# jzhang-dev/FEDRANN

Hardware: AMD Instinct MI355X
Metric: read-pairs/sec (overlap candidates) (higher is better)
Workload: dtype f32 (canonical fp32 results; fp16 MFMA candidate prefilter + exact fp32 re-rank)

## Files before the change

fedrann_amd/_lib.py:

```python
import ctypes
import os

import numpy as np

HERE = os.path.dirname(os.path.abspath(__file__))
LIB_PATH = os.environ.get("FEDRANN_HIP_LIB") or os.path.join(HERE, "libfedrann_hip.so")

SYMBOLS = (
    "fdr_create", "fdr_destroy", "fdr_last_error", "fdr_device_info", "fdr_padded_dim",
    "fdr_projection_load", "fdr_embed", "fdr_knn", "fdr_embed_knn", "fdr_embed_dev",
    "fdr_normalize_dev", "fdr_knn_workspace_bytes", "fdr_knn_dev", "fdr_timing", "fdr_timing_read",
    "fdr_last_uncertified", "fdr_set_knn_mode", "fdr_set_dedup_mode", "fdr_last_unique", "fdr_kmer_output_scan",
    "fdr_kmer_output_load", "fdr_kmer_search", "fdr_kmer_search_indices", "fdr_kmer_count",
    "fdr_kmer_count_fetch", "fdr_set_kmer_count_block", "fdr_last_kmer_count_blocks", "fdr_csr_compact", "fdr_host_register", "fdr_host_unregister",
    "fdr_overlaps_write", "fdr_last_prefilter_launches", "fdr_knn_classes_dev", "fdr_knn_unique_dev",
    "fdr_knn_expand_dev", "fdr_kmer_output_scan_range", "fdr_kmer_output_load_range",
    "fdr_kmer_count_begin", "fdr_kmer_count_add", "fdr_kmer_count_finish", "fdr_reads_scan", "fdr_reads_parse",
    "fdr_kmer_output_append", "fdr_last_query_paths", "fdr_last_knn_trace", "fdr_kmer_count_export_dev",
    "fdr_kmer_count_merge_dev", "fdr_kmer_count_merge", "fdr_set_knn_capture", "fdr_last_candidates",
    "fdr_last_range_sets", "fdr_knn_sparse", "fdr_set_live_chunks", "fdr_knn_sparse_metric",
    "fdr_sparse_index_build", "fdr_sparse_index_search", "fdr_sparse_index_info", "fdr_sparse_index_free",
)
FDR_MAX_K = 128
KERNELS = ("embed_csr", "normalize_rows", "knn_tile", "knn_merge", "knn_prefilter", "knn_rerank",
           "knn_dedup", "kmer_search", "kmer_compact")
FDR_MAX_DIM = 2048
PATH_CERTIFIED, PATH_RANGE, PATH_EXACT, PATH_ZERO, PATH_RANGE_OVERFLOW, PATH_GENERIC, PATH_CLASS_MEMBER = 1, 2, 3, 4, 5, 6, 0x80
TRACE_KINDS = ("none", "exact", "prefilter", "generic", "sparse")
FALLBACKS = ("none", "chunked", "whole")
CAPTURE_CANDIDATES, CAPTURE_RANGE = 1, 2
RANGE_CAP = 1024
METRIC_COSINE, METRIC_JACCARD = 0, 1
SPARSE_METRICS = {"cosine": METRIC_COSINE, "jaccard": METRIC_JACCARD}


class KnnTrace(ctypes.Structure):
    _fields_ = [(n, ctypes.c_int32) for n in ("kind", "dp", "k", "kp")] + \
        [(n, ctypes.c_int64) for n in ("queries", "targets")] + \
        [(n, ctypes.c_int32) for n in (
            "pass_waves", "pass_wps", "pass_units", "pass_list_keys", "pass_pingpong", "pass_launches", "pass_queues",
            "pass_segments", "uncertified", "zero_queries", "range_queries", "range_chunks", "range_pp_chunks",
            "range_w8_chunks", "range_overflow", "exact_fallback", "exact_calls", "exact_queries", "exact_waves",
            "exact_qsets", "generic", "exact_segments", "pass_live", "pass_live_items_2", "pass_live_items_3",
            "pass_live_items_4", "pass_live_items_5", "pass_live_items_6", "pass_live_dense_items")]


class FedrannHipError(RuntimeError):
    pass


_lib = None


def _share_torch_hip_runtime():
    if os.environ.get("FEDRANN_HIP_SYSTEM_RUNTIME") == "1":
        return
    try:
        import importlib.util
        spec = importlib.util.find_spec("torch")
        if spec is None or not spec.submodule_search_locations:
            return
        path = os.path.join(list(spec.submodule_search_locations)[0], "lib", "libamdhip64.so")
        if os.path.exists(path):
            ctypes.CDLL(path, mode=ctypes.RTLD_GLOBAL)
    except (OSError, ImportError, ValueError):
        pass


def load_library():
    global _lib
    if _lib is not None:
        return _lib
    if not os.path.exists(LIB_PATH):
        raise FedrannHipError(
            "%s is missing: build it with `python -m fedrann_amd.build` "
            "(hipcc --offload-arch=gfx950); there is no CPU fallback" % LIB_PATH)
    _share_torch_hip_runtime()
    L = ctypes.CDLL(LIB_PATH)
    i32, i64, vp, sz = ctypes.c_int32, ctypes.c_int64, ctypes.c_void_p, ctypes.c_size_t
    L.fdr_create.argtypes = [ctypes.c_int, ctypes.POINTER(vp)]
    L.fdr_destroy.argtypes = [vp]
    L.fdr_last_error.argtypes = []
    L.fdr_last_error.restype = ctypes.c_char_p
    L.fdr_device_info.argtypes = [vp, ctypes.c_char_p, ctypes.c_int]
    L.fdr_padded_dim.argtypes = [ctypes.c_int]
    L.fdr_projection_load.argtypes = [vp, i64, i32, vp, vp, vp]
    L.fdr_embed.argtypes = [vp, i64, vp, vp, vp]
    L.fdr_knn.argtypes = [vp, vp, i64, i32, i32, vp, vp]
    L.fdr_embed_knn.argtypes = [vp, i64, vp, vp, i32, vp, vp, vp]
    L.fdr_knn_sparse.argtypes = [vp, i64, i64, vp, vp, vp, i32, vp, vp]
    L.fdr_knn_sparse_metric.argtypes = [vp, i32, i64, i64, vp, vp, vp, i32, vp, vp]
    L.fdr_sparse_index_build.argtypes = [vp, i32, i64, i64, vp, vp, vp]
    L.fdr_sparse_index_search.argtypes = [vp, i32, i64, i64, vp, vp]
    L.fdr_sparse_index_info.argtypes = [vp, ctypes.POINTER(i32), ctypes.POINTER(i64), ctypes.POINTER(i64),
                                        ctypes.POINTER(i64), ctypes.POINTER(sz)]
    L.fdr_sparse_index_free.argtypes = [vp]
    L.fdr_embed_dev.argtypes = [vp, i64, vp, vp, vp, vp]
    L.fdr_normalize_dev.argtypes = [vp, vp, i64, i32, vp, vp, vp]
    L.fdr_knn_workspace_bytes.argtypes = [vp, i64, i64, i32, i32]
    L.fdr_knn_workspace_bytes.restype = sz
    L.fdr_knn_dev.argtypes = [vp, vp, vp, i64, vp, vp, i64, i64, i32, i32, vp, vp, vp, sz, vp]
    L.fdr_knn_classes_dev.argtypes = [vp, vp, vp, i64, i32, i32, i64, vp, sz, vp, ctypes.POINTER(i32)]
    L.fdr_knn_unique_dev.argtypes = [vp, i64, i64, vp, vp, vp]
    L.fdr_knn_expand_dev.argtypes = [vp, i64, i64, i64, vp, vp, i64, vp, vp, vp]
    L.fdr_last_uncertified.argtypes = [vp]
    L.fdr_last_query_paths.argtypes = [vp, vp, i64]
    L.fdr_last_knn_trace.argtypes = [vp, ctypes.POINTER(KnnTrace)]
    L.fdr_set_knn_mode.argtypes = [vp, ctypes.c_int]
    L.fdr_set_knn_capture.argtypes = [vp, ctypes.c_int]
    L.fdr_last_candidates.argtypes = [vp, vp, i64, i32, ctypes.POINTER(i32)]
    L.fdr_last_range_sets.argtypes = [vp, i64, vp, vp, vp, vp]
    L.fdr_set_dedup_mode.argtypes = [vp, ctypes.c_int]
    L.fdr_set_live_chunks.argtypes = [vp, ctypes.c_int]
    L.fdr_last_unique.argtypes = [vp, ctypes.POINTER(ctypes.c_int), ctypes.POINTER(ctypes.c_int)]
    L.fdr_last_prefilter_launches.argtypes = [vp, ctypes.POINTER(ctypes.c_int), ctypes.POINTER(ctypes.c_int)]
    p64 = ctypes.POINTER(ctypes.c_int64)
    L.fdr_kmer_output_scan.argtypes = [ctypes.c_char_p, p64, p64, p64]
    L.fdr_kmer_output_load.argtypes = [ctypes.c_char_p, i64, i32, i64, i64, i64, vp, vp, vp, vp]
    L.fdr_kmer_output_scan_range.argtypes = [ctypes.c_char_p, i64, i64, p64, p64, p64]
    L.fdr_kmer_output_load_range.argtypes = [ctypes.c_char_p, i64, i32, i64, i64, i64, i64, i64, vp, vp, vp, vp]
    L.fdr_kmer_output_append.argtypes = [ctypes.c_char_p, i64, vp, vp, vp, vp]
    L.fdr_reads_scan.argtypes = [vp, i64, i32, i32, i32, p64, p64, p64]
    L.fdr_reads_parse.argtypes = [vp, i64, i32, i32, i64, i64, vp, vp, vp]
    L.fdr_csr_compact.argtypes = [vp, i64, vp, vp, vp, vp, i64, i32]
    L.fdr_host_register.argtypes = [vp, vp, sz]
    L.fdr_host_unregister.argtypes = [vp, vp]
    L.fdr_overlaps_write.argtypes = [ctypes.c_char_p, i32, i32, i64, i64, i64, i32, vp, vp, vp, vp, vp, i32, p64]
    L.fdr_kmer_search.argtypes = [vp, vp, vp, i64, vp, i64, i32, vp, p64]
    L.fdr_kmer_search_indices.argtypes = [vp, vp]
    L.fdr_kmer_count.argtypes = [vp, vp, vp, i64, i32, i64, p64]
    L.fdr_kmer_count_fetch.argtypes = [vp, vp, vp]
    L.fdr_kmer_count_begin.argtypes = [vp, i32]
    L.fdr_kmer_count_add.argtypes = [vp, vp, vp, i64]
    L.fdr_kmer_count_finish.argtypes = [vp, i64, p64]
    L.fdr_set_kmer_count_block.argtypes = [vp, ctypes.c_int64]
    L.fdr_last_kmer_count_blocks.argtypes = [vp]
    L.fdr_kmer_count_export_dev.argtypes = [vp, vp, i32, vp, vp, vp, vp]
    L.fdr_kmer_count_merge_dev.argtypes = [vp, i32, vp, vp, vp, i64, p64, vp]
    L.fdr_kmer_count_merge.argtypes = [vp, i32, vp, vp, vp, i64, p64]
    L.fdr_timing.argtypes = [vp, ctypes.c_int]
    L.fdr_timing_read.argtypes = [vp, ctypes.c_int, ctypes.POINTER(ctypes.c_int),
                                  ctypes.POINTER(ctypes.c_float)]
    for name in SYMBOLS:
        fn = getattr(L, name)
        if name not in ("fdr_last_error", "fdr_knn_workspace_bytes"):
            fn.restype = ctypes.c_int
    _lib = L
    return L


def _ptr(a):
    return None if a is None else ctypes.c_void_p(a.ctypes.data)


def _as(a, dtype, name):
    b = np.ascontiguousarray(a, dtype=dtype)
    if b.dtype != np.dtype(dtype):
        raise TypeError("%s must be %s" % (name, np.dtype(dtype)))
    return b


def kmer_output_load(path, n_features, n_threads=0):
    L = load_library()
    bpath = os.fsencode(path)
    R, nnz, nb = ctypes.c_int64(), ctypes.c_int64(), ctypes.c_int64()
    rc = L.fdr_kmer_output_scan(bpath, ctypes.byref(R), ctypes.byref(nnz), ctypes.byref(nb))
    if rc != 0:
        raise FedrannHipError("fdr_kmer_output_scan failed (%d): %s" % (rc, L.fdr_last_error().decode()))
    indptr = np.empty(2 * R.value + 1, dtype=np.int64)
    indices = np.empty(2 * nnz.value, dtype=np.int32)
    name_off = np.empty(R.value + 1, dtype=np.int64)
    names = np.empty(nb.value, dtype=np.uint8)
    rc = L.fdr_kmer_output_load(bpath, int(n_features), int(n_threads), R.value, nnz.value, nb.value,
                                indptr.ctypes.data, indices.ctypes.data, name_off.ctypes.data, names.ctypes.data)
    if rc != 0:
        raise FedrannHipError("fdr_kmer_output_load failed (%d): %s" % (rc, L.fdr_last_error().decode()))
    return indptr, indices, name_off, names


def kmer_output_records(path):
    import struct
    with open(path, "rb") as f:
        head = f.read(16)
    if len(head) < 16:
        raise ValueError("incomplete file header")
    magic, version, _, total = struct.unpack("<4sB3sQ", head)
    if magic != b"KMER":
        raise ValueError("invalid file format (bad magic)")
    if version != 1:
        raise ValueError("unsupported version: %d" % version)
    return int(total)


def kmer_output_load_range(path, n_features, rec_lo, rec_hi, n_threads=0, with_names=True):
    L = load_library()
    bpath = os.fsencode(path)
    R, nnz, nb = ctypes.c_int64(), ctypes.c_int64(), ctypes.c_int64()
    total = kmer_output_records(path)
    lo = max(0, min(int(rec_lo), total))
    hi = total if rec_hi is None else max(lo, min(int(rec_hi), total))
    rc = L.fdr_kmer_output_scan_range(bpath, lo, hi, ctypes.byref(R), ctypes.byref(nnz), ctypes.byref(nb))
    if rc != 0:
        raise FedrannHipError("fdr_kmer_output_scan_range failed (%d): %s" % (rc, L.fdr_last_error().decode()))
    indptr = np.empty(2 * (hi - lo) + 1, dtype=np.int64)
    indices = np.empty(2 * nnz.value, dtype=np.int32)
    name_off = np.empty(R.value + 1, dtype=np.int64) if with_names else None
    names = np.empty(nb.value, dtype=np.uint8) if with_names else None
    rc = L.fdr_kmer_output_load_range(bpath, int(n_features), int(n_threads), R.value, lo, hi, nnz.value, nb.value,
                                      indptr.ctypes.data, indices.ctypes.data,
                                      name_off.ctypes.data if with_names else None,
                                      names.ctypes.data if with_names and names.size else None)
    if rc != 0:
        raise FedrannHipError("fdr_kmer_output_load_range failed (%d): %s" % (rc, L.fdr_last_error().decode()))
    return R.value, indptr, indices, name_off, names


def reads_parse(buf, n, is_fastq, fastq_ids_as_fasta, eof, seq_buf=None):
    L = load_library()
    used, R, nb = ctypes.c_int64(), ctypes.c_int64(), ctypes.c_int64()
    base = buf.ctypes.data if n else None
    rc = L.fdr_reads_scan(base, int(n), int(bool(is_fastq)), int(bool(fastq_ids_as_fasta)), int(bool(eof)),
                          ctypes.byref(used), ctypes.byref(R), ctypes.byref(nb))
    if rc != 0:
        raise FedrannHipError("fdr_reads_scan failed (%d): %s" % (rc, L.fdr_last_error().decode()))
    seqs = np.empty(nb.value, dtype=np.uint8) if seq_buf is None else seq_buf[:nb.value]
    off = np.empty(R.value + 1, dtype=np.int64)
    span = np.empty(2 * R.value, dtype=np.int64)
    rc = L.fdr_reads_parse(base, used.value, int(bool(is_fastq)), int(bool(fastq_ids_as_fasta)), R.value, nb.value,
                           seqs.ctypes.data if nb.value else None, off.ctypes.data, span.ctypes.data if R.value else None)
    if rc != 0:
        raise FedrannHipError("fdr_reads_parse failed (%d): %s" % (rc, L.fdr_last_error().decode()))
    view = memoryview(buf)
    sp = span.tolist()
    ids = [bytes(view[sp[2 * r]:sp[2 * r + 1]]) for r in range(R.value)]
    return used.value, ids, seqs, off


def reads_consumed(buf, n, is_fastq, fastq_ids_as_fasta, eof):
    L = load_library()
    used, R, nb = ctypes.c_int64(), ctypes.c_int64(), ctypes.c_int64()
    rc = L.fdr_reads_scan(buf.ctypes.data if n else None, int(n), int(bool(is_fastq)), int(bool(fastq_ids_as_fasta)),
                          int(bool(eof)), ctypes.byref(used), ctypes.byref(R), ctypes.byref(nb))
    if rc != 0:
        raise FedrannHipError("fdr_reads_scan failed (%d): %s" % (rc, L.fdr_last_error().decode()))
    return used.value


def kmer_output_append(path, ids, indptr, indices):
    L = load_library()
    name_off, names = pack_names(ids)
    indptr = np.ascontiguousarray(indptr, dtype=np.int64)
    indices = np.ascontiguousarray(indices, dtype=np.int32)
    if indptr.size != len(ids) + 1:
        raise ValueError("indptr must have one entry per record + 1")
    rc = L.fdr_kmer_output_append(os.fsencode(path), len(ids), _ptr(name_off), _ptr(names) if names.size else None,
                                  _ptr(indptr), _ptr(indices) if indices.size else None)
    if rc != 0:
        msg = L.fdr_last_error().decode()
        if "non-ASCII" in msg or "bytes long" in msg:
            raise ValueError(msg)
        raise FedrannHipError("fdr_kmer_output_append failed (%d): %s" % (rc, msg))


def pack_names(read_names):
    enc = [n if isinstance(n, bytes) else str(n).encode("utf-8") for n in read_names]
    off = np.zeros(len(enc) + 1, dtype=np.int64)
    if enc:
        np.cumsum([len(b) for b in enc], out=off[1:])
    return off, np.frombuffer(b"".join(enc), dtype=np.uint8)


def overlaps_write(path, idx, dist, name_off, names, strands, row0=0, append=False, header=True, n_threads=0):
    L = load_library()
    idx = _as(idx, np.int32, "idx")
    dist = _as(dist, np.float32, "dist")
    if idx.ndim != 2 or dist.shape != idx.shape:
        raise ValueError("idx and dist must be [rows, k] arrays of the same shape")
    name_off = _as(name_off, np.int64, "name_off")
    names = np.ascontiguousarray(names, dtype=np.uint8)
    if strands is None:
        n_total = 2 * (name_off.size - 1)
    else:
        strands = np.ascontiguousarray(strands, dtype=np.uint8)
        n_total = name_off.size - 1
        if strands.size != n_total:
            raise ValueError("strands must have one entry per row")
    lines = ctypes.c_int64()
    rc = L.fdr_overlaps_write(os.fsencode(path), 1 if append else 0, 1 if header else 0, n_total, int(row0),
                              idx.shape[0], idx.shape[1], _ptr(idx), _ptr(dist), _ptr(name_off),
                              names.ctypes.data if names.size else None, _ptr(strands) if strands is not None else None,
                              int(n_threads),
                              ctypes.byref(lines))
    if rc != 0:
        raise FedrannHipError("fdr_overlaps_write failed (%d): %s" % (rc, L.fdr_last_error().decode()))
    return int(lines.value)


def sparse_metric_code(metric):
    if not isinstance(metric, str) or metric not in SPARSE_METRICS:
        raise ValueError("metric must be 'cosine' or 'jaccard', got %r" % (metric,))
    return SPARSE_METRICS[metric]


def check_sparse_rows(indptr, indices, values, n_features, k):
    return _check_sparse(indptr, indices, values, n_features, k)


def check_sparse_csr(indptr, indices, values, n_features):
    n, _, F = _check_sparse(indptr, indices, values, n_features, None)
    return n, F


def check_sparse_search(n, k, lo=0, hi=None):
    for name, v in (("k", k), ("lo", lo), ("hi", hi)):
        if isinstance(v, bool) or not (isinstance(v, (int, np.integer)) or (name == "hi" and v is None)):
            raise ValueError("%s must be an integer, got %r" % (name, v))
    k, lo, hi = int(k), int(lo), int(n if hi is None else hi)
    if not 1 <= k <= FDR_MAX_K or k > n:
        raise ValueError("need 1 <= k <= min(%d, n = %d), got k = %d" % (FDR_MAX_K, n, k))
    if not 0 <= lo <= hi <= n:
        raise ValueError("need 0 <= lo <= hi <= n = %d, got [%d, %d)" % (n, lo, hi))
    return k, lo, hi


def _check_sparse(indptr, indices, values, n_features, k):
    for name, a, dt in (("indptr", indptr, np.int64), ("indices", indices, np.int32), ("values", values, np.float32)):
        if a is None and name == "values":
            continue
        if not isinstance(a, np.ndarray) or a.dtype != dt:
            raise TypeError("%s must be a numpy %s array" % (name, np.dtype(dt)))
        if a.ndim != 1 or not a.flags.c_contiguous:
            raise ValueError("%s must be a C-contiguous 1-D array" % name)
    if indptr.size < 1 or indptr[0] != 0 or indptr[-1] != indices.size or np.any(np.diff(indptr) < 0):
        raise ValueError("indptr is not a CSR row pointer of the indices")
    if values is not None and values.size != indices.size:
        raise ValueError("values and indices differ in length")
    n, k, F = indptr.size - 1, None if k is None else int(k), int(n_features)
    if not 1 <= F <= np.iinfo(np.int32).max:
        raise ValueError("n_features must be in [1, 2^31)")
    if k is None:
        if n < 1:
            raise ValueError("need at least one row")
    elif not 1 <= k <= FDR_MAX_K or k > n:
        raise ValueError("need 1 <= k <= min(%d, n = %d), got k = %d" % (FDR_MAX_K, n, k))
    if indices.size:
        if int(indices.min()) < 0 or int(indices.max()) >= F:
            raise ValueError("a feature index is outside [0, %d)" % F)
        ascending = np.diff(indices) > 0
        starts = indptr[1:-1]
        ascending[starts[(starts > 0) & (starts < indices.size)] - 1] = True
        if not np.all(ascending):
            raise ValueError("feature indices must be strictly ascending inside each row (sorted, no duplicates)")
    if values is not None and not np.all(np.isfinite(values)):
        raise ValueError("values must be finite")
    return n, k, F


class Context:

    def __init__(self, device=0):
        self._L = load_library()
        h = ctypes.c_void_p()
        rc = self._L.fdr_create(int(device), ctypes.byref(h))
        if rc != 0:
            raise FedrannHipError("fdr_create(%d) failed (%d): %s" % (device, rc, self._err()))
        self._h = h
        self.device = int(device)
        self.n_features = 0
        self.d = 0
        self._sparse_gen = 0

    def _err(self):
        return self._L.fdr_last_error().decode("utf-8", "replace")

    def _check(self, rc, what):
        if rc != 0:
            raise FedrannHipError("%s failed (%d): %s" % (what, rc, self._err()))

    def close(self):
        if getattr(self, "_h", None):
            self._L.fdr_destroy(self._h)
            self._h = None

    def __del__(self):
        try:
            self.close()
        except Exception:
            pass

    def __enter__(self):
        return self

    def __exit__(self, *a):
        self.close()

    def device_info(self):
        buf = ctypes.create_string_buffer(256)
        self._check(self._L.fdr_device_info(self._h, buf, 256), "fdr_device_info")
        name, arch, cus, mem = buf.value.decode().split("|")
        return {"name": name, "arch": arch, "cus": int(cus), "hbm_bytes": int(mem)}

    def padded_dim(self, d):
        dp = self._L.fdr_padded_dim(int(d))
        if dp < 0:
            raise FedrannHipError("embedding dimension %d unsupported (1..%d)" % (d, FDR_MAX_DIM))
        return dp

    def set_knn_mode(self, mode):
        code = {"auto": 0, "exact": 1, "prefilter": 2}[mode]
        self._check(self._L.fdr_set_knn_mode(self._h, code), "fdr_set_knn_mode")

    def set_dedup_mode(self, mode):
        code = {"auto": 0, "off": 1, "on": 2, "force": 3}[mode]
        self._check(self._L.fdr_set_dedup_mode(self._h, code), "fdr_set_dedup_mode")

    def set_live_chunks(self, mode):
        code = {"auto": 0, "off": 1, "force": 2}[mode]
        self._check(self._L.fdr_set_live_chunks(self._h, code), "fdr_set_live_chunks")

    def kmer_search(self, seqs, seq_off, lib_codes, k):
        seqs = np.ascontiguousarray(seqs, dtype=np.uint8)
        seq_off = np.ascontiguousarray(seq_off, dtype=np.int64)
        lib_codes = np.ascontiguousarray(lib_codes, dtype=np.uint64)
        R = seq_off.size - 1
        if R < 0 or (R >= 0 and seq_off.size and int(seq_off[-1]) != seqs.size):
            raise ValueError("seq_off does not describe seqs")
        indptr = np.empty(R + 1, dtype=np.int64)
        nnz = ctypes.c_int64()
        self._check(self._L.fdr_kmer_search(self._h, seqs.ctypes.data, seq_off.ctypes.data, R,
                                            lib_codes.ctypes.data, lib_codes.size, int(k), indptr.ctypes.data,
                                            ctypes.byref(nnz)), "fdr_kmer_search")
        indices = np.empty(nnz.value, dtype=np.int32)
        self._check(self._L.fdr_kmer_search_indices(self._h, indices.ctypes.data), "fdr_kmer_search_indices")
        return indptr, indices

    def kmer_count(self, seqs, seq_off, k, min_count=1):
        seqs = np.ascontiguousarray(seqs, dtype=np.uint8)
        seq_off = np.ascontiguousarray(seq_off, dtype=np.int64)
        n = ctypes.c_int64()
        self._check(self._L.fdr_kmer_count(self._h, seqs.ctypes.data, seq_off.ctypes.data, seq_off.size - 1, int(k),
                                           int(min_count), ctypes.byref(n)), "fdr_kmer_count")
        codes = np.empty(n.value, dtype=np.uint64)
        counts = np.empty(n.value, dtype=np.uint64)
        self._check(self._L.fdr_kmer_count_fetch(self._h, codes.ctypes.data, counts.ctypes.data), "fdr_kmer_count_fetch")
        return codes, counts

    def kmer_count_begin(self, k):
        self._check(self._L.fdr_kmer_count_begin(self._h, int(k)), "fdr_kmer_count_begin")

    def kmer_count_add(self, seqs, seq_off):
        seqs = np.ascontiguousarray(seqs, dtype=np.uint8)
        seq_off = np.ascontiguousarray(seq_off, dtype=np.int64)
        self._check(self._L.fdr_kmer_count_add(self._h, seqs.ctypes.data, seq_off.ctypes.data, seq_off.size - 1),
                    "fdr_kmer_count_add")

    def kmer_count_finish(self, min_count=1):
        n = ctypes.c_int64()
        self._check(self._L.fdr_kmer_count_finish(self._h, int(min_count), ctypes.byref(n)), "fdr_kmer_count_finish")
        codes = np.empty(n.value, dtype=np.uint64)
        counts = np.empty(n.value, dtype=np.uint64)
        self._check(self._L.fdr_kmer_count_fetch(self._h, codes.ctypes.data, counts.ctypes.data), "fdr_kmer_count_fetch")
        return codes, counts

    def set_kmer_count_block(self, chars):
        self._check(self._L.fdr_set_kmer_count_block(self._h, int(chars)), "fdr_set_kmer_count_block")

    def kmer_count_export_dev(self, d_splitters, n_parts, d_codes_out=None, d_counts_out=None, stream=None):
        part_off = np.empty(int(n_parts) + 1, dtype=np.int64)
        self._check(self._L.fdr_kmer_count_export_dev(self._h, d_splitters or None, int(n_parts), d_codes_out or None,
                                                      d_counts_out or None, part_off.ctypes.data, stream or None),
                    "fdr_kmer_count_export_dev")
        return part_off

    def kmer_count_merge_dev(self, run_off, d_codes, d_counts, min_count=1, stream=None):
        run_off = np.ascontiguousarray(run_off, dtype=np.int64)
        n = ctypes.c_int64()
        self._check(self._L.fdr_kmer_count_merge_dev(self._h, run_off.size - 1, run_off.ctypes.data, d_codes or None,
                                                     d_counts or None, int(min_count), ctypes.byref(n), stream or None),
                    "fdr_kmer_count_merge_dev")
        return self._kmer_count_fetch(n.value)

    def kmer_count_merge(self, run_off, codes, counts, min_count=1):
        run_off = np.ascontiguousarray(run_off, dtype=np.int64)
        codes = np.ascontiguousarray(codes, dtype=np.uint64)
        counts = np.ascontiguousarray(counts, dtype=np.uint64)
        if codes.size != counts.size or (run_off.size and codes.size < int(run_off[-1])):
            raise ValueError("run_off does not describe codes / counts")
        n = ctypes.c_int64()
        self._check(self._L.fdr_kmer_count_merge(self._h, run_off.size - 1, run_off.ctypes.data, codes.ctypes.data,
                                                 counts.ctypes.data, int(min_count), ctypes.byref(n)),
                    "fdr_kmer_count_merge")
        return self._kmer_count_fetch(n.value)

    def _kmer_count_fetch(self, n):
        codes = np.empty(n, dtype=np.uint64)
        counts = np.empty(n, dtype=np.uint64)
        self._check(self._L.fdr_kmer_count_fetch(self._h, codes.ctypes.data, counts.ctypes.data), "fdr_kmer_count_fetch")
        return codes, counts

    def last_kmer_count_blocks(self):
        return int(self._L.fdr_last_kmer_count_blocks(self._h))

    def last_unique(self):
        a, b = ctypes.c_int(), ctypes.c_int()
        self._check(self._L.fdr_last_unique(self._h, ctypes.byref(a), ctypes.byref(b)), "fdr_last_unique")
        return int(a.value), int(b.value)

    def last_prefilter_launches(self):
        a, b = ctypes.c_int(), ctypes.c_int()
        self._check(self._L.fdr_last_prefilter_launches(self._h, ctypes.byref(a), ctypes.byref(b)),
                    "fdr_last_prefilter_launches")
        return int(a.value), int(b.value)

    def last_uncertified(self):
        return int(self._L.fdr_last_uncertified(self._h))

    def last_query_paths(self, n_queries):
        out = np.empty(int(n_queries), dtype=np.uint8)
        self._check(self._L.fdr_last_query_paths(self._h, _ptr(out), int(n_queries)), "fdr_last_query_paths")
        return out

    def last_knn_trace(self):
        t = KnnTrace()
        self._check(self._L.fdr_last_knn_trace(self._h, ctypes.byref(t)), "fdr_last_knn_trace")
        out = {name: int(getattr(t, name)) for name, _ in KnnTrace._fields_}
        out["kind"] = TRACE_KINDS[out["kind"]]
        out["exact_fallback"] = FALLBACKS[out["exact_fallback"]]
        return out

    def set_knn_capture(self, what):
        self._check(self._L.fdr_set_knn_capture(self._h, int(what)), "fdr_set_knn_capture")

    def last_candidates(self, n_queries, kp):
        keys = np.empty((int(n_queries), int(kp)), dtype=np.uint64)
        qbits = ctypes.c_int32(0)
        self._check(self._L.fdr_last_candidates(self._h, _ptr(keys), int(n_queries), int(kp), ctypes.byref(qbits)),
                    "fdr_last_candidates")
        return keys, int(qbits.value)

    def last_range_sets(self, n_range):
        n = int(n_range)
        q, th, cnt = np.empty(n, np.int32), np.empty(n, np.float32), np.empty(n, np.int32)
        rows = np.empty((n, RANGE_CAP), np.int32)
        self._check(self._L.fdr_last_range_sets(self._h, n, _ptr(q), _ptr(th), _ptr(cnt), _ptr(rows)),
                    "fdr_last_range_sets")
        return q, th, cnt, rows

    def timing(self, enable):
        self._check(self._L.fdr_timing(self._h, 1 if enable else 0), "fdr_timing")

    def timing_read(self, which):
        n, ms = ctypes.c_int(), ctypes.c_float()
        self._check(self._L.fdr_timing_read(self._h, int(which), ctypes.byref(n), ctypes.byref(ms)),
                    "fdr_timing_read")
        return int(n.value), float(ms.value)

    def projection_load(self, p_indptr, p_cols, p_vals, n_features, d):
        p_indptr = _as(p_indptr, np.int64, "p_indptr")
        p_cols = _as(p_cols, np.int32, "p_cols")
        p_vals = _as(p_vals, np.float32, "p_vals")
        if p_indptr.shape != (int(n_features) + 1,):
            raise ValueError("p_indptr must have n_features + 1 entries")
        self._check(self._L.fdr_projection_load(self._h, int(n_features), int(d), _ptr(p_indptr),
                                                _ptr(p_cols), _ptr(p_vals)), "fdr_projection_load")
        self.n_features, self.d = int(n_features), int(d)

    def csr_compact(self, a_indptr, a_indices, n_threads=0):
        a_indptr = _as(a_indptr, np.int64, "a_indptr")
        a_indices = _as(a_indices, np.int32, "a_indices")
        n = a_indptr.shape[0] - 1
        out_ip = np.empty(n + 1, dtype=np.int64)
        out_ix = np.empty(max(int(a_indices.size), 1), dtype=np.int32)
        self._check(self._L.fdr_csr_compact(self._h, n, _ptr(a_indptr), _ptr(a_indices), _ptr(out_ip),
                                            _ptr(out_ix), int(out_ix.size), int(n_threads)), "fdr_csr_compact")
        return out_ip, np.ascontiguousarray(out_ix[:int(out_ip[-1])])

    def host_register(self, *arrays):
        for a in arrays:
            if a is not None and a.nbytes:
                self._check(self._L.fdr_host_register(self._h, a.ctypes.data, a.nbytes), "fdr_host_register")

    def host_unregister(self, *arrays):
        for a in arrays:
            if a is not None and a.nbytes:
                self._check(self._L.fdr_host_unregister(self._h, a.ctypes.data), "fdr_host_unregister")

    def embed(self, a_indptr, a_indices):
        a_indptr = _as(a_indptr, np.int64, "a_indptr")
        a_indices = _as(a_indices, np.int32, "a_indices")
        n = a_indptr.shape[0] - 1
        E = np.empty((n, self.d), dtype=np.float32)
        self._check(self._L.fdr_embed(self._h, n, _ptr(a_indptr), _ptr(a_indices), _ptr(E)),
                    "fdr_embed")
        return E

    def knn(self, E, k):
        E = _as(E, np.float32, "E")
        if E.ndim != 2:
            raise ValueError("E must be 2-D")
        n, d = E.shape
        idx = np.empty((n, k), dtype=np.int32)
        dist = np.empty((n, k), dtype=np.float32)
        self._check(self._L.fdr_knn(self._h, _ptr(E), n, d, int(k), _ptr(idx), _ptr(dist)),
                    "fdr_knn")
        return idx, dist

    def knn_sparse(self, indptr, indices, values, n_features, k, metric="cosine"):
        code = sparse_metric_code(metric)
        n, k, F = check_sparse_rows(indptr, indices, values, n_features, k)
        self._sparse_gen += 1
        idx = np.empty((n, k), dtype=np.int32)
        dist = np.empty((n, k), dtype=np.float32)
        if code == METRIC_COSINE:
            self._check(self._L.fdr_knn_sparse(self._h, n, F, _ptr(indptr), _ptr(indices), _ptr(values), k,
                                               _ptr(idx), _ptr(dist)), "fdr_knn_sparse")
        else:
            self._check(self._L.fdr_knn_sparse_metric(self._h, code, n, F, _ptr(indptr), _ptr(indices),
                                                      _ptr(values), k, _ptr(idx), _ptr(dist)),
                        "fdr_knn_sparse_metric")
        return idx, dist

    def sparse_index(self, indptr, indices, values, n_features, metric="cosine"):
        code = sparse_metric_code(metric)
        n, F = check_sparse_csr(indptr, indices, values, n_features)
        self._sparse_gen += 1
        self._check(self._L.fdr_sparse_index_build(self._h, code, n, F, _ptr(indptr), _ptr(indices), _ptr(values)),
                    "fdr_sparse_index_build")
        return SparseIndex(self, n, metric, self._sparse_gen)

    def embed_knn(self, a_indptr, a_indices, k, return_embedding=False, out=None):
        a_indptr = _as(a_indptr, np.int64, "a_indptr")
        a_indices = _as(a_indices, np.int32, "a_indices")
        n = a_indptr.shape[0] - 1
        if out is None:
            idx = np.empty((n, k), dtype=np.int32)
            dist = np.empty((n, k), dtype=np.float32)
        else:
            idx, dist = out
            if (idx.shape, dist.shape) != ((n, k), (n, k)) or idx.dtype != np.int32 or dist.dtype != np.float32 \
                    or not (idx.flags.c_contiguous and dist.flags.c_contiguous):
                raise ValueError("out must be C-contiguous (int32 [n,k], float32 [n,k])")
        E = np.empty((n, self.d), dtype=np.float32) if return_embedding else None
        self._check(self._L.fdr_embed_knn(self._h, n, _ptr(a_indptr), _ptr(a_indices), int(k),
                                          _ptr(idx), _ptr(dist), _ptr(E)), "fdr_embed_knn")
        return (idx, dist, E) if return_embedding else (idx, dist)

    def embed_dev(self, n_rows, d_indptr, d_indices, d_E, stream=0):
        self._check(self._L.fdr_embed_dev(self._h, int(n_rows), d_indptr, d_indices, d_E,
                                          stream or None), "fdr_embed_dev")

    def normalize_dev(self, d_E, n_rows, d, d_Ehat, d_zero, stream=0):
        self._check(self._L.fdr_normalize_dev(self._h, d_E, int(n_rows), int(d), d_Ehat, d_zero,
                                              stream or None), "fdr_normalize_dev")

    def knn_workspace_bytes(self, nq, nt, d, k):
        return int(self._L.fdr_knn_workspace_bytes(self._h, int(nq), int(nt), int(d), int(k)))

    def knn_dev(self, d_Qhat, d_qzero, nq, d_That, d_tzero, nt, t_base, d, k, d_idx, d_dist,
                d_ws, ws_bytes, stream=0):
        self._check(self._L.fdr_knn_dev(self._h, d_Qhat, d_qzero, int(nq), d_That, d_tzero,
                                        int(nt), int(t_base), int(d), int(k), d_idx, d_dist, d_ws,
                                        int(ws_bytes), stream or None), "fdr_knn_dev")


    def knn_classes_dev(self, d_That, d_tzero, nt, d, k, nq_max, d_ws, ws_bytes, stream=0):
        nu = ctypes.c_int32()
        self._check(self._L.fdr_knn_classes_dev(self._h, d_That, d_tzero, int(nt), int(d), int(k), int(nq_max), d_ws,
                                                int(ws_bytes), stream or None, ctypes.byref(nu)), "fdr_knn_classes_dev")
        return int(nu.value)

    def knn_unique_dev(self, u_lo, u_hi, d_idx_u, d_dist_u, stream=0):
        self._check(self._L.fdr_knn_unique_dev(self._h, int(u_lo), int(u_hi), d_idx_u, d_dist_u, stream or None),
                    "fdr_knn_unique_dev")

    def knn_expand_dev(self, q0, nq, t_base, d_idx_u_all, d_dist_u_all, d_idx, d_dist, stream=0, u_row_stride=0):
        self._check(self._L.fdr_knn_expand_dev(self._h, int(q0), int(nq), int(t_base), d_idx_u_all, d_dist_u_all,
                                               int(u_row_stride), d_idx, d_dist, stream or None), "fdr_knn_expand_dev")


class SparseIndex:

    def __init__(self, ctx, n, metric, gen):
        self._ctx, self.n, self.metric, self._gen = ctx, int(n), metric, gen
        self._open = True

    def _live(self, what):
        if not self._open:
            raise FedrannHipError("%s: the sparse index is closed" % what)
        if not getattr(self._ctx, "_h", None):
            raise FedrannHipError("%s: the context of the sparse index is closed" % what)
        if self._ctx._sparse_gen != self._gen:
            raise FedrannHipError("%s: the context has built another sparse index since this one" % what)

    def search(self, k, lo=0, hi=None, out=None):
        k, lo, hi = check_sparse_search(self.n, k, lo, hi)
        nq = hi - lo
        if out is None:
            idx = np.empty((nq, k), dtype=np.int32)
            dist = np.empty((nq, k), dtype=np.float32)
        else:
            idx, dist = out
            if (idx.shape, dist.shape) != ((nq, k), (nq, k)) or idx.dtype != np.int32 or dist.dtype != np.float32 \
                    or not (idx.flags.c_contiguous and dist.flags.c_contiguous):
                raise ValueError("out must be C-contiguous (int32 [hi - lo, k], float32 [hi - lo, k])")
        self._live("SparseIndex.search")
        c = self._ctx
        c._check(c._L.fdr_sparse_index_search(c._h, k, lo, hi, _ptr(idx), _ptr(dist)), "fdr_sparse_index_search")
        return idx, dist

    def info(self):
        self._live("SparseIndex.info")
        c = self._ctx
        m, n, p, z = ctypes.c_int32(), ctypes.c_int64(), ctypes.c_int64(), ctypes.c_int64()
        b = ctypes.c_size_t()
        c._check(c._L.fdr_sparse_index_info(c._h, ctypes.byref(m), ctypes.byref(n), ctypes.byref(p), ctypes.byref(z),
                                            ctypes.byref(b)), "fdr_sparse_index_info")
        name = [s for s, v in SPARSE_METRICS.items() if v == m.value][0]
        return {"metric": name, "n": int(n.value), "postings": int(p.value), "zero_rows": int(z.value),
                "device_bytes": int(b.value)}

    def close(self):
        c = self._ctx
        if self._open and getattr(c, "_h", None) and c._sparse_gen == self._gen:
            c._check(c._L.fdr_sparse_index_free(c._h), "fdr_sparse_index_free")
        self._open = False

    def __enter__(self):
        return self

    def __exit__(self, *a):
        self.close()


_default_ctx = None


def default_context():
    global _default_ctx
    if _default_ctx is None:
        dev = int(os.environ.get("FEDRANN_DEVICE", os.environ.get("LOCAL_RANK", "0")))
        _default_ctx = Context(dev)
    return _default_ctx
```

fedrann_amd/csrc/fedrann_hip.hip:

```cpp
#include <hip/hip_runtime.h>
#include <rocprim/device/device_radix_sort.hpp>
#include <rocprim/device/device_scan.hpp>
#include <rocprim/device/device_run_length_encode.hpp>
#include <rocprim/device/device_merge.hpp>
#include <rocprim/device/device_reduce_by_key.hpp>

#include <algorithm>
#include <array>
#include <atomic>
#include <cmath>
#include <condition_variable>
#include <cstdarg>
#include <cstdint>
#include <cstdio>
#include <cstdlib>
#include <cstring>
#include <functional>
#include <limits>
#include <mutex>
#include <new>
#include <string>
#include <thread>
#include <type_traits>
#include <utility>
#include <vector>

#include "../../include/fedrann_hip.h"

typedef float f32x4 __attribute__((ext_vector_type(4)));
typedef float f32x16 __attribute__((ext_vector_type(16)));

#include "host_common.inc"

#define HIP_TRY(expr)                                                                          \
    do {                                                                                       \
        hipError_t e_ = (expr);                                                                \
        if (e_ != hipSuccess)                                                                  \
            return fail(e_ == hipErrorOutOfMemory ? FDR_E_NOMEM : FDR_E_HIP, "%s failed: %s",  \
                        #expr, hipGetErrorString(e_));                                         \
    } while (0)

template <int DP>
__global__ __launch_bounds__(256) void embed_csr_kernel(
    long long n_rows, const long long *__restrict__ a_indptr, const int *__restrict__ a_indices,
    long long n_features, const uint2 *__restrict__ ftab, const uint4 *__restrict__ rowinfo,
    const uint2 *__restrict__ ent, int d, float *__restrict__ E) {
    constexpr int NACC = DP / 64;
    static_assert(DP <= 512, "d > 512: embed_csr_wide_kernel");
    constexpr int GR = 8;
    constexpr int NB = 4;
    constexpr int RPW = 2;
    const int lane = threadIdx.x & 63;
    const long long wave0 = (long long)blockIdx.x * (blockDim.x >> 6) + (threadIdx.x >> 6);
    const long long nwaves = (long long)gridDim.x * (blockDim.x >> 6);
    auto apply = [&](float (&acc)[NACC], const uint4 &inf, const bool h) __attribute__((always_inline)) {
        u64 m = __ballot(h);
        while (m) {
            const int src = __builtin_ctzll(m);
            m &= m - 1;
            int q = __builtin_amdgcn_readlane((int)inf.x, src);
            const int ee = q + __builtin_amdgcn_readlane((int)inf.y, src);
            unsigned c = (unsigned)__builtin_amdgcn_readlane((int)inf.z, src);
            float v = __int_as_float(__builtin_amdgcn_readlane((int)inf.w, src));
            while (true) {
#pragma unroll
                for (int i = 0; i < NACC; ++i)
                    if (c == (unsigned)(lane + 64 * i)) acc[i] += v;
                if (++q >= ee) break;
                const uint2 en = ent[q];
                c = en.x;
                v = __uint_as_float(en.y);
            }
        }
    };
    auto store_row = [&](const long long row, const float (&acc)[NACC]) __attribute__((always_inline)) {
        float *out = E + row * (long long)d;
#pragma unroll
        for (int i = 0; i < NACC; ++i)
            if (lane + 64 * i < d) out[lane + 64 * i] = acc[i];
    };
    for (long long row0 = wave0 * GR; row0 < n_rows; row0 += nwaves * GR) {
        long long beg[GR], len_max = 0;
        int len[GR];
#pragma unroll
        for (int r = 0; r < GR; ++r) {
            const long long row = row0 + r < n_rows ? row0 + r : n_rows - 1;
            beg[r] = a_indptr[row];
            const long long l = row0 + r < n_rows ? a_indptr[row + 1] - beg[r] : 0;
            len[r] = (int)(l < 64 ? l : 64);
            len_max = l > len_max ? l : len_max;
        }
        if (len_max <= 64) {
            int f[GR];
            uint2 w[GR];
            uint4 info[GR];
            bool hit[GR];
#pragma unroll
            for (int r = 0; r < GR; ++r) f[r] = lane < len[r] ? a_indices[beg[r] + lane] : -1;
#pragma unroll
            for (int r = 0; r < GR; ++r) {
                w[r] = make_uint2(0u, 0u);
                if (f[r] >= 0 && (long long)f[r] < n_features) w[r] = ftab[f[r] >> 5];
            }
#pragma unroll
            for (int r = 0; r < GR; ++r) {
                const unsigned bit = 1u << (f[r] & 31);
                hit[r] = (w[r].x & bit) != 0u;
                info[r] = make_uint4(0u, 0u, 0u, 0u);
                if (hit[r]) info[r] = rowinfo[w[r].y + __popc(w[r].x & (bit - 1u))];
            }
#pragma unroll
            for (int r = 0; r < GR; ++r) {
                if (row0 + r >= n_rows) continue;
                float acc[NACC];
#pragma unroll
                for (int i = 0; i < NACC; ++i) acc[i] = 0.0f;
                apply(acc, info[r], hit[r]);
                store_row(row0 + r, acc);
            }
            continue;
        }
        for (int p0 = 0; p0 < GR && row0 + p0 < n_rows; p0 += RPW) {
            const long long prow0 = row0 + p0;
            long long pbeg[RPW], pend[RPW];
            int f[RPW][NB];
            uint2 w[RPW][NB];
            uint4 info[RPW][NB];
            bool hit[RPW][NB];
#pragma unroll
            for (int r = 0; r < RPW; ++r) {
                const long long row = prow0 + r < n_rows ? prow0 + r : n_rows - 1;
                pbeg[r] = a_indptr[row];
                pend[r] = prow0 + r < n_rows ? a_indptr[row + 1] : pbeg[r];
            }
#pragma unroll
            for (int r = 0; r < RPW; ++r)
#pragma unroll
                for (int u = 0; u < NB; ++u) {
                    const long long pos = pbeg[r] + 64 * u + lane;
                    f[r][u] = pos < pend[r] ? a_indices[pos] : -1;
                }
#pragma unroll
            for (int r = 0; r < RPW; ++r)
#pragma unroll
                for (int u = 0; u < NB; ++u) {
                    w[r][u] = make_uint2(0u, 0u);
                    if (f[r][u] >= 0 && (long long)f[r][u] < n_features) w[r][u] = ftab[f[r][u] >> 5];
                }
#pragma unroll
            for (int r = 0; r < RPW; ++r)
#pragma unroll
                for (int u = 0; u < NB; ++u) {
                    const unsigned bit = 1u << (f[r][u] & 31);
                    hit[r][u] = (w[r][u].x & bit) != 0u;
                    info[r][u] = make_uint4(0u, 0u, 0u, 0u);
                    if (hit[r][u]) info[r][u] = rowinfo[w[r][u].y + __popc(w[r][u].x & (bit - 1u))];
                }
#pragma unroll
            for (int r = 0; r < RPW; ++r) {
                if (prow0 + r >= n_rows) continue;
                float acc[NACC];
#pragma unroll
                for (int i = 0; i < NACC; ++i) acc[i] = 0.0f;
#pragma unroll
                for (int u = 0; u < NB; ++u) apply(acc, info[r][u], hit[r][u]);
                for (long long base = pbeg[r] + 64 * NB; base < pend[r]; base += 64 * NB) {
                    int f2[NB];
                    uint2 w2[NB];
#pragma unroll
                    for (int u = 0; u < NB; ++u) {
                        const long long pos = base + 64 * u + lane;
                        f2[u] = pos < pend[r] ? a_indices[pos] : -1;
                    }
#pragma unroll
                    for (int u = 0; u < NB; ++u) {
                        w2[u] = make_uint2(0u, 0u);
                        if (f2[u] >= 0 && (long long)f2[u] < n_features) w2[u] = ftab[f2[u] >> 5];
                    }
#pragma unroll
                    for (int u = 0; u < NB; ++u) {
                        const unsigned bit = 1u << (f2[u] & 31);
                        const bool h2 = (w2[u].x & bit) != 0u;
                        uint4 i2 = make_uint4(0u, 0u, 0u, 0u);
                        if (h2) i2 = rowinfo[w2[u].y + __popc(w2[u].x & (bit - 1u))];
                        apply(acc, i2, h2);
                    }
                }
                store_row(prow0 + r, acc);
            }
        }
    }
}

template <int DP>
__global__ __launch_bounds__(256) void embed_csr_wide_kernel(
    long long n_rows, const long long *__restrict__ a_indptr, const int *__restrict__ a_indices,
    long long n_features, const uint2 *__restrict__ ftab, const uint4 *__restrict__ rowinfo,
    const uint2 *__restrict__ ent, int d, float *__restrict__ E) {
    constexpr int NACC = DP / 64;
    constexpr int NB = 4;
    constexpr int RPW = 2;
    const int lane = threadIdx.x & 63;
    const long long wave0 = (long long)blockIdx.x * (blockDim.x >> 6) + (threadIdx.x >> 6);
    const long long nwaves = (long long)gridDim.x * (blockDim.x >> 6);
    for (long long row0 = wave0 * RPW; row0 < n_rows; row0 += nwaves * RPW) {
        long long beg[RPW], end[RPW];
        int f[RPW][NB];
        uint2 w[RPW][NB];
        uint4 info[RPW][NB];
        bool hit[RPW][NB];
#pragma unroll
        for (int r = 0; r < RPW; ++r) {
            const long long row = row0 + r < n_rows ? row0 + r : n_rows - 1;
            beg[r] = a_indptr[row];
            end[r] = row0 + r < n_rows ? a_indptr[row + 1] : beg[r];
        }
#pragma unroll
        for (int r = 0; r < RPW; ++r)
#pragma unroll
            for (int u = 0; u < NB; ++u) {
                const long long pos = beg[r] + 64 * u + lane;
                f[r][u] = pos < end[r] ? a_indices[pos] : -1;
            }
#pragma unroll
        for (int r = 0; r < RPW; ++r)
#pragma unroll
            for (int u = 0; u < NB; ++u) {
                w[r][u] = make_uint2(0u, 0u);
                if (f[r][u] >= 0 && (long long)f[r][u] < n_features) w[r][u] = ftab[f[r][u] >> 5];
            }
#pragma unroll
        for (int r = 0; r < RPW; ++r)
#pragma unroll
            for (int u = 0; u < NB; ++u) {
                const unsigned bit = 1u << (f[r][u] & 31);
                hit[r][u] = (w[r][u].x & bit) != 0u;
                info[r][u] = make_uint4(0u, 0u, 0u, 0u);
                if (hit[r][u]) info[r][u] = rowinfo[w[r][u].y + __popc(w[r][u].x & (bit - 1u))];
            }
#pragma unroll
        for (int r = 0; r < RPW; ++r) {
            if (row0 + r >= n_rows) break;
            float acc[NACC];
#pragma unroll
            for (int i = 0; i < NACC; ++i) acc[i] = 0.0f;
            auto apply = [&](const uint4 &inf, const bool h) {
                u64 m = __ballot(h);
                while (m) {
                    const int src = __builtin_ctzll(m);
                    m &= m - 1;
                    int q = __builtin_amdgcn_readlane((int)inf.x, src);
                    const int ee = q + __builtin_amdgcn_readlane((int)inf.y, src);
                    unsigned c = (unsigned)__builtin_amdgcn_readlane((int)inf.z, src);
                    float v = __int_as_float(__builtin_amdgcn_readlane((int)inf.w, src));
                    while (true) {
#pragma unroll
                        for (int i = 0; i < NACC; ++i)
                            if (c == (unsigned)(lane + 64 * i)) acc[i] += v;
                        if (++q >= ee) break;
                        const uint2 en = ent[q];
                        c = en.x;
                        v = __uint_as_float(en.y);
                    }
                }
            };
#pragma unroll
            for (int u = 0; u < NB; ++u) apply(info[r][u], hit[r][u]);
            for (long long base = beg[r] + 64 * NB; base < end[r]; base += 64 * NB) {
                int f2[NB];
                uint2 w2[NB];
#pragma unroll
                for (int u = 0; u < NB; ++u) {
                    const long long pos = base + 64 * u + lane;
                    f2[u] = pos < end[r] ? a_indices[pos] : -1;
                }
#pragma unroll
                for (int u = 0; u < NB; ++u) {
                    w2[u] = make_uint2(0u, 0u);
                    if (f2[u] >= 0 && (long long)f2[u] < n_features) w2[u] = ftab[f2[u] >> 5];
                }
#pragma unroll
                for (int u = 0; u < NB; ++u) {
                    const unsigned bit = 1u << (f2[u] & 31);
                    const bool h2 = (w2[u].x & bit) != 0u;
                    uint4 i2 = make_uint4(0u, 0u, 0u, 0u);
                    if (h2) i2 = rowinfo[w2[u].y + __popc(w2[u].x & (bit - 1u))];
                    apply(i2, h2);
                }
            }
            float *out = E + (row0 + r) * (long long)d;
#pragma unroll
            for (int i = 0; i < NACC; ++i)
                if (lane + 64 * i < d) out[lane + 64 * i] = acc[i];
        }
    }
}

template <int DP, int RB, bool VEC>
__global__ __launch_bounds__(256) void normalize_rows_kernel(const float *__restrict__ E,
                                                             long long n_rows, int d,
                                                             float *__restrict__ Ehat,
                                                             unsigned char *__restrict__ zero) {
    __shared__ float tile[RB][DP + 1];
    const int tid = threadIdx.x;
    const long long row0 = (long long)blockIdx.x * RB;
    const int nr = (int)min((long long)RB, n_rows - row0);
    const float *src = E + row0 * (long long)d;
    if (d < DP || nr < RB) {
        for (int i = tid; i < RB * DP; i += 256) tile[i / DP][i % DP] = 0.0f;
        __syncthreads();
    }
    const int total = nr * d;
    if constexpr (VEC) {
        const f32x4 *src4 = reinterpret_cast<const f32x4 *>(src);
        for (int i4 = tid; i4 < total / 4; i4 += 256) {
            const f32x4 v = src4[i4];
            const int i = 4 * i4, r = i / d, c = i - r * d;
            tile[r][c] = v[0];
            tile[r][c + 1] = v[1];
            tile[r][c + 2] = v[2];
            tile[r][c + 3] = v[3];
        }
    } else {
        for (int i = tid; i < total; i += 256) tile[i / d][i % d] = src[i];
    }
    __syncthreads();
    if (tid < RB) {
        float n = 0.0f;
#pragma unroll 8
        for (int k = 0; k < DP; ++k) {
            const float x = tile[tid][k];
            n = __builtin_fmaf(x, x, n);
        }
        float ri = 0.0f;
        if (n > 0.0f) ri = (float)(1.0 / sqrt((double)n));
#pragma unroll 8
        for (int k = 0; k < DP; ++k) tile[tid][k] = tile[tid][k] * ri;
        if (tid < nr) zero[row0 + tid] = n > 0.0f ? 0 : 1;
    }
    __syncthreads();
    float *dst = Ehat + row0 * (long long)DP;
    if constexpr (VEC) {
        f32x4 *dst4 = reinterpret_cast<f32x4 *>(dst);
        for (int i4 = tid; i4 < nr * DP / 4; i4 += 256) {
            const int i = 4 * i4, r = i / DP, p = i % DP;
            const int g = p >> 3, hh = (p >> 2) & 1;
            const float *t = &tile[r][8 * g + hh];
            dst4[i4] = f32x4{t[0], t[2], t[4], t[6]};
        }
    } else {
        for (int i = tid; i < nr * DP; i += 256) {
            const int r = i / DP, p = i % DP;
            const int g = p >> 3, hh = (p >> 2) & 1, s = p & 3;
            dst[i] = tile[r][8 * g + 2 * s + hh];
        }
    }
}

#include "knn_plan.inc"
#include "knn_workspace.inc"
#include "projection_tables.inc"
#include "csr_compact.inc"
#include "host_upload.inc"
#include "knn_exact.inc"
#include "knn_exact_wide.inc"
#include "knn_prefilter.inc"
#include "knn_prefilter_pp.inc"
#include "knn_order.inc"
#include "knn_prefilter_live.inc"
#include "dedup_classes.inc"
#include "knn_generic.inc"

struct DevBuf {
    void *p = nullptr;
    size_t cap = 0;
    int reserve(size_t bytes) {
        if (bytes <= cap) return FDR_OK;
        if (p) (void)hipFree(p);
        p = nullptr;
        cap = 0;
        hipError_t e = hipMalloc(&p, bytes ? bytes : 1);
        if (e != hipSuccess) {
            p = nullptr;
            return fail(FDR_E_NOMEM, "hipMalloc(%zu bytes) failed: %s", bytes, hipGetErrorString(e));
        }
        cap = bytes;
        return FDR_OK;
    }
    void release() {
        if (p) (void)hipFree(p);
        p = nullptr;
        cap = 0;
    }
    DevBuf() = default;
    DevBuf(const DevBuf &) = delete;
    DevBuf &operator=(const DevBuf &) = delete;
    ~DevBuf() { release(); }
};

template <class T>
struct DevArray {
    DevBuf buf;
    int reserve(size_t count) { return buf.reserve(count * sizeof(T)); }
    T *ptr() const { return static_cast<T *>(buf.p); }
    void release() { buf.release(); }
    size_t bytes() const { return buf.cap; }
};
template <class... A>
static void release_all(A &...arrays) {
    (arrays.release(), ...);
}

template <class... F>
static int rocprim_reserve(DevArray<char> &tmp, const F &...calls) {
    size_t need = 1;
    hipError_t e = hipSuccess;
    auto ask = [&](const auto &call) {
        size_t bytes = 0;
        if (e == hipSuccess) e = call(nullptr, bytes);
        need = std::max(need, bytes);
    };
    (ask(calls), ...);
    if (e != hipSuccess) return fail(FDR_E_HIP, "rocprim temporary storage size query failed: %s", hipGetErrorString(e));
    return tmp.reserve(need);
}
template <class F>
static int rocprim_run(DevArray<char> &tmp, const char *what, const F &call) {
    if (int rc = rocprim_reserve(tmp, call)) return rc;
    size_t bytes = tmp.bytes();
    const hipError_t e = call(tmp.ptr(), bytes);
    if (e != hipSuccess)
        return fail(e == hipErrorOutOfMemory ? FDR_E_NOMEM : FDR_E_HIP, "%s failed: %s", what, hipGetErrorString(e));
    return FDR_OK;
}

struct PinnedBuf {
    void *p = nullptr;
    size_t cap = 0;
    int reserve(size_t bytes) {
        if (bytes <= cap) return FDR_OK;
        if (p) (void)hipHostFree(p);
        p = nullptr;
        cap = 0;
        hipError_t e = hipHostMalloc(&p, bytes ? bytes : 1, hipHostMallocDefault);
        if (e != hipSuccess) {
            p = nullptr;
            return fail(FDR_E_NOMEM, "hipHostMalloc(%zu bytes) failed: %s", bytes, hipGetErrorString(e));
        }
        cap = bytes;
        return FDR_OK;
    }
    PinnedBuf() = default;
    PinnedBuf(const PinnedBuf &) = delete;
    PinnedBuf &operator=(const PinnedBuf &) = delete;
    ~PinnedBuf() {
        if (p) (void)hipHostFree(p);
    }
};

struct KnnCallRecord {
    struct {
        int flagged = 0;
        int launches = 0, queues = 0;
    } pass;
    int unique_targets = 0, unique_queries = 0;
    struct {
        const uint8_t *dev = nullptr;
        int64_t n = 0;
        uint8_t all = FDR_PATH_NONE;
        hipStream_t stream = nullptr;
    } paths;
    fdr_knn_trace trace = {};
};

struct KnnArgs {
    const float *Qhat;
    const uint8_t *qzero;
    int64_t nq;
    const float *That;
    const uint8_t *tzero;
    int64_t nt, t_base;
    int d, k;
    int32_t *idx;
    float *dist;
    void *ws;
    size_t ws_bytes;
    hipStream_t st;
};


struct KmerSearchScratch {
    DevArray<unsigned char> seq;
    DevArray<long long> off;
    DevArray<u64> lib_codes;
    DevArray<u64> keys;
    DevArray<unsigned> vals;
    DevArray<u64> bloom;
    DevArray<unsigned long long> counter;
    DevArray<u64> pairs, sorted;
    DevArray<int> flag, scan;
    DevArray<int> indices, rows;
    DevArray<long long> indptr;
    DevArray<char> tmp;
    long long nnz = 0;
    void release() {
        release_all(seq, off, lib_codes, keys, vals, bloom, counter, pairs, sorted, flag, scan, indices, rows, indptr, tmp);
        nnz = 0;
    }
};

struct KmerCountScratch {
    DevArray<unsigned char> seq;
    DevArray<long long> off;
    DevArray<u64> codes;
    DevArray<u64> sorted;
    DevArray<unsigned> run_len;
    DevArray<unsigned> n_runs;
    DevArray<u64> run_counts;
    DevArray<u64> acc_codes[2], acc_counts[2];
    DevArray<u64> merged_codes, merged_counts;
    DevArray<unsigned long long> n_table;
    DevArray<int> keep, keep_scan;
    DevArray<u64> kept_counts;
    DevArray<long long> run_off, samp_pre;
    DevArray<u64> samples, bounds;
    DevArray<long long> slices;
    DevArray<long long> part_off;
    DevArray<char> tmp;
    int k = 0;
    int acc = 0;
    long long na = 0;
    long long n = 0;
    int64_t block_chars = 0;
    int blocks = 0;
    void release() {
        release_all(seq, off, codes, sorted, run_len, n_runs, run_counts, acc_codes[0], acc_codes[1], acc_counts[0],
                    acc_counts[1], merged_codes, merged_counts, n_table, keep, keep_scan, kept_counts, run_off, samp_pre,
                    samples, bounds, slices, part_off, tmp);
        k = acc = 0;
        na = n = 0;
    }
};

struct SparseIndex {
    DevArray<long long> indptr;
    DevArray<int> indices;
    DevArray<float> values;
    DevArray<float> xhat;
    DevArray<int> asize;
    DevArray<unsigned char> zero;
    DevArray<u64> keys, sorted_keys;
    DevArray<unsigned> pos, sorted_pos;
    DevArray<int> efeat;
    DevArray<float> pval;
    DevArray<long long> runptr;
    DevArray<int> heavy;
    DevArray<u64> cnt;
    DevArray<char> tmp;
    struct Built {
        bool valid = false;
        int metric = 0;
        long long n = 0, kept = 0, nzero = 0;
    } built;
    int *run_flags() const { return reinterpret_cast<int *>(keys.ptr()); }
    int *run_numbers(long long kept) const { return run_flags() + kept; }
    int *posting_rows() const { return reinterpret_cast<int *>(pos.ptr()); }
    static constexpr size_t cnt_words = 8 + FDR_MAX_K;
    int *zidx() const { return reinterpret_cast<int *>(cnt.ptr() + 8); }
    float *zdist() const { return reinterpret_cast<float *>(zidx() + FDR_MAX_K); }
    template <class F>
    auto each(F f) {
        return f(indptr, indices, values, xhat, asize, zero, keys, sorted_keys, pos, sorted_pos, efeat, pval, runptr,
                 heavy, cnt, tmp);
    }
    size_t bytes() {
        return each([](auto &...a) { return (a.bytes() + ...); });
    }
    void release() {
        each([](auto &...a) { release_all(a...); });
        built = {};
    }
};

struct fdr_ctx {
    int device = 0;
    int num_cus = 256;
    hipStream_t stream = nullptr;
    hipStream_t aux_stream[3] = {nullptr, nullptr, nullptr};
    hipEvent_t aux_ev[4] = {nullptr, nullptr, nullptr, nullptr};
    hipDeviceProp_t prop;
    long long n_features = 0;
    int d = 0;
    long long p_nnz = 0, p_rows = 0;
    DevBuf ftab, crow, ent;
    std::vector<uint32_t> h_bits;
    DevBuf a_indptr, a_indices, E, Ehat, zero, idx, dist, ws;
    DevBuf c_indptr, c_indices;
    PinnedBuf stage_ids, stage_ptr;
    hipEvent_t up_ev[3] = {nullptr, nullptr, nullptr};
    hup::WorkerPool up_pool;
    KmerSearchScratch ks;
    KmerCountScratch kc;
    SparseIndex sp;
    int knn_mode = FDR_MODE_AUTO;
    int dedup_mode = FDR_DEDUP_AUTO;
    int live_mode = FDR_LIVE_AUTO;
    std::vector<unsigned> live_host;
    KnnCallRecord last;
    struct {
        int what = 0;
        bool cand_valid = false, range_valid = false;
        int64_t nq = 0, n_range = 0;
        int kp = 0, qbits = 0;
        DevBuf cand, rq, rtheta, rcnt, rrows;
        hipStream_t stream = nullptr;
    } cap;
    struct {
        bool valid = false;
        const float *That = nullptr;
        const uint8_t *tzero = nullptr;
        int64_t nt = 0, nq_max = 0;
        int d = 0, k = 0, nu = 0;
        void *ws = nullptr;
        size_t ws_bytes = 0;
    } cls;
    bool timing = false;
    std::vector<hipEvent_t> ev_pool[FDR_NUM_KERNELS];
    size_t ev_used[FDR_NUM_KERNELS] = {};
};

static void knn_call_begin(fdr_ctx *ctx) {
    ctx->last.trace = fdr_knn_trace{};
    ctx->last.paths = {};
    ctx->cap.cand_valid = ctx->cap.range_valid = false;
    ctx->cap.nq = ctx->cap.n_range = 0;
}

static void knn_call_header(fdr_ctx *ctx, int kind, int dp, int k, int64_t nq, int64_t nt) {
    ctx->last.trace.kind = kind;
    ctx->last.trace.dp = dp;
    ctx->last.trace.k = k;
    ctx->last.trace.queries = nq;
    ctx->last.trace.targets = nt;
}
static void knn_call_whole(fdr_ctx *ctx, uint8_t path, int kind, int dp, int k, int64_t nq, int64_t nt) {
    knn_call_header(ctx, kind, dp, k, nq, nt);
    ctx->last.paths = {nullptr, nq, path, nullptr};
    ctx->last.pass = {};
}

static int timing_begin(fdr_ctx *ctx, int kind, hipStream_t st) {
    if (!ctx->timing) return FDR_OK;
    std::vector<hipEvent_t> &pool = ctx->ev_pool[kind];
    if (ctx->ev_used[kind] + 2 > pool.size()) {
        hipEvent_t a, b;
        HIP_TRY(hipEventCreate(&a));
        HIP_TRY(hipEventCreate(&b));
        pool.push_back(a);
        pool.push_back(b);
    }
    HIP_TRY(hipEventRecord(pool[ctx->ev_used[kind]], st));
    return FDR_OK;
}

static int timing_end(fdr_ctx *ctx, int kind, hipStream_t st) {
    if (!ctx->timing) return FDR_OK;
    HIP_TRY(hipEventRecord(ctx->ev_pool[kind][ctx->ev_used[kind] + 1], st));
    ctx->ev_used[kind] += 2;
    return FDR_OK;
}

static int use_device(fdr_ctx *ctx) {
    if (!ctx) return fail(FDR_E_ARG, "null context");
    HIP_TRY(hipSetDevice(ctx->device));
    return FDR_OK;
}

FDR_EXPORT const char *fdr_last_error(void) { return g_err; }

FDR_EXPORT int fdr_padded_dim(int d) { return padded_dim(d); }

FDR_EXPORT int fdr_create(int device_id, fdr_ctx **out) {
    if (!out) return fail(FDR_E_ARG, "fdr_create: out is null");
    *out = nullptr;
    int n = 0;
    HIP_TRY(hipGetDeviceCount(&n));
    if (n <= 0) return fail(FDR_E_HIP, "no HIP device visible: the MI355X path cannot run");
    if (device_id < 0 || device_id >= n)
        return fail(FDR_E_ARG, "device %d out of range (have %d)", device_id, n);
    fdr_ctx *c = new (std::nothrow) fdr_ctx();
    if (!c) return fail(FDR_E_NOMEM, "out of host memory");
    c->device = device_id;
    hipError_t e = hipSetDevice(device_id);
    if (e == hipSuccess) e = hipGetDeviceProperties(&c->prop, device_id);
    if (e == hipSuccess) e = hipStreamCreateWithFlags(&c->stream, hipStreamNonBlocking);
    if (e != hipSuccess) {
        delete c;
        return fail(FDR_E_HIP, "fdr_create: device %d: %s", device_id, hipGetErrorString(e));
    }
    c->num_cus = c->prop.multiProcessorCount > 0 ? c->prop.multiProcessorCount : 256;
    if (const char *m = getenv("FDR_KNN_MODE")) {
        if (strcmp(m, "exact") == 0) c->knn_mode = FDR_MODE_EXACT;
        else if (strcmp(m, "prefilter") == 0) c->knn_mode = FDR_MODE_PREFILTER;
    }
    *out = c;
    return FDR_OK;
}

FDR_EXPORT int fdr_destroy(fdr_ctx *ctx) {
    if (!ctx) return FDR_OK;
    (void)hipSetDevice(ctx->device);
    (void)hipStreamSynchronize(ctx->stream);
    ctx->up_pool.stop();
    for (hipEvent_t e : ctx->up_ev)
        if (e) (void)hipEventDestroy(e);
    for (int i = 0; i < FDR_NUM_KERNELS; ++i)
        for (hipEvent_t e : ctx->ev_pool[i]) (void)hipEventDestroy(e);
    (void)hipStreamDestroy(ctx->stream);
    for (hipStream_t a : ctx->aux_stream)
        if (a) {
            (void)hipStreamSynchronize(a);
            (void)hipStreamDestroy(a);
        }
    for (hipEvent_t e : ctx->aux_ev)
        if (e) (void)hipEventDestroy(e);
    delete ctx;
    return FDR_OK;
}

FDR_EXPORT int fdr_device_info(fdr_ctx *ctx, char *buf, int buflen) {
    if (!ctx || !buf || buflen <= 0) return fail(FDR_E_ARG, "fdr_device_info: bad argument");
    snprintf(buf, (size_t)buflen, "%s|%s|%d|%zu", ctx->prop.name, ctx->prop.gcnArchName,
             ctx->prop.multiProcessorCount, (size_t)ctx->prop.totalGlobalMem);
    return FDR_OK;
}

FDR_EXPORT int fdr_last_uncertified(fdr_ctx *ctx) { return ctx ? ctx->last.pass.flagged : 0; }

FDR_EXPORT int fdr_last_query_paths(fdr_ctx *ctx, uint8_t *paths, int64_t n_queries) {
    int rc = use_device(ctx);
    if (rc) return rc;
    if (!paths || n_queries <= 0) return fail(FDR_E_ARG, "last_query_paths: bad argument");
    const auto &rec = ctx->last.paths;
    if (rec.n != n_queries)
        return fail(FDR_E_STATE, "last_query_paths: the last k-NN call recorded codes for %lld query rows, not %lld",
                    (long long)rec.n, (long long)n_queries);
    if (!rec.dev) {
        memset(paths, rec.all, (size_t)n_queries);
        return FDR_OK;
    }
    HIP_TRY(hipMemcpyAsync(paths, rec.dev, (size_t)n_queries, hipMemcpyDeviceToHost, rec.stream));
    HIP_TRY(hipStreamSynchronize(rec.stream));
    return FDR_OK;
}

FDR_EXPORT int fdr_last_unique(fdr_ctx *ctx, int *unique_targets, int *unique_queries) {
    if (!ctx || !unique_targets || !unique_queries) return fail(FDR_E_ARG, "bad argument");
    *unique_targets = ctx->last.unique_targets;
    *unique_queries = ctx->last.unique_queries;
    return FDR_OK;
}

FDR_EXPORT int fdr_last_prefilter_launches(fdr_ctx *ctx, int *launches, int *queues) {
    if (!ctx || !launches || !queues) return fail(FDR_E_ARG, "bad argument");
    *launches = ctx->last.pass.launches;
    *queues = ctx->last.pass.queues;
    return FDR_OK;
}

FDR_EXPORT int fdr_last_knn_trace(fdr_ctx *ctx, fdr_knn_trace *out) {
    if (!ctx || !out) return fail(FDR_E_ARG, "bad argument");
    *out = ctx->last.trace;
    return FDR_OK;
}

FDR_EXPORT int fdr_set_knn_capture(fdr_ctx *ctx, int what) {
    if (!ctx || what < 0 || what > (FDR_CAPTURE_CANDIDATES | FDR_CAPTURE_RANGE)) return fail(FDR_E_ARG, "bad capture flags");
    ctx->cap.what = what;
    return FDR_OK;
}

FDR_EXPORT int fdr_last_candidates(fdr_ctx *ctx, uint64_t *keys, int64_t n_queries, int32_t kp, int32_t *qbits_out) {
    int rc = use_device(ctx);
    if (rc) return rc;
    if (!keys || n_queries <= 0 || kp <= 0) return fail(FDR_E_ARG, "last_candidates: bad argument");
    if (!ctx->cap.cand_valid) return fail(FDR_E_STATE, "last_candidates: the last k-NN call captured no candidates");
    if (ctx->cap.nq != n_queries || ctx->cap.kp != kp)
        return fail(FDR_E_STATE, "last_candidates: the last k-NN call captured %lld x %d keys, not %lld x %d",
                    (long long)ctx->cap.nq, ctx->cap.kp, (long long)n_queries, kp);
    HIP_TRY(hipMemcpyAsync(keys, ctx->cap.cand.p, (size_t)n_queries * kp * 8, hipMemcpyDeviceToHost, ctx->cap.stream));
    HIP_TRY(hipStreamSynchronize(ctx->cap.stream));
    if (qbits_out) *qbits_out = ctx->cap.qbits;
    return FDR_OK;
}

FDR_EXPORT int fdr_last_range_sets(fdr_ctx *ctx, int64_t n_range, int32_t *queries, float *theta, int32_t *counts,
                                   int32_t *rows) {
    int rc = use_device(ctx);
    if (rc) return rc;
    if (!queries || !theta || !counts || !rows || n_range <= 0) return fail(FDR_E_ARG, "last_range_sets: bad argument");
    if (!ctx->cap.range_valid) return fail(FDR_E_STATE, "last_range_sets: the last k-NN call captured no range pass");
    if (ctx->cap.n_range != n_range)
        return fail(FDR_E_STATE, "last_range_sets: the last k-NN call captured %lld range queries, not %lld",
                    (long long)ctx->cap.n_range, (long long)n_range);
    const hipStream_t st = ctx->cap.stream;
    HIP_TRY(hipMemcpyAsync(queries, ctx->cap.rq.p, (size_t)n_range * 4, hipMemcpyDeviceToHost, st));
    HIP_TRY(hipMemcpyAsync(theta, ctx->cap.rtheta.p, (size_t)n_range * 4, hipMemcpyDeviceToHost, st));
    HIP_TRY(hipMemcpyAsync(counts, ctx->cap.rcnt.p, (size_t)n_range * 4, hipMemcpyDeviceToHost, st));
    HIP_TRY(hipMemcpyAsync(rows, ctx->cap.rrows.p, (size_t)n_range * RANGE_CAP * 4, hipMemcpyDeviceToHost, st));
    HIP_TRY(hipStreamSynchronize(st));
    for (int64_t i = 0; i < n_range; ++i)
        for (int m = std::max(0, std::min(counts[i], RANGE_CAP)); m < RANGE_CAP; ++m) rows[i * RANGE_CAP + m] = -1;
    return FDR_OK;
}

FDR_EXPORT int fdr_set_knn_mode(fdr_ctx *ctx, int mode) {
    if (!ctx || mode < FDR_MODE_AUTO || mode > FDR_MODE_PREFILTER) return fail(FDR_E_ARG, "bad k-NN mode");
    ctx->knn_mode = mode;
    return FDR_OK;
}

FDR_EXPORT int fdr_set_dedup_mode(fdr_ctx *ctx, int mode) {
    if (!ctx || mode < FDR_DEDUP_AUTO || mode > FDR_DEDUP_FORCE) return fail(FDR_E_ARG, "bad duplicate-row mode");
    ctx->dedup_mode = mode;
    return FDR_OK;
}

FDR_EXPORT int fdr_set_live_chunks(fdr_ctx *ctx, int mode) {
    if (!ctx || mode < FDR_LIVE_AUTO || mode > FDR_LIVE_FORCE) return fail(FDR_E_ARG, "bad live-chunk mode");
    ctx->live_mode = mode;
    return FDR_OK;
}

FDR_EXPORT int fdr_timing(fdr_ctx *ctx, int enable) {
    if (!ctx) return fail(FDR_E_ARG, "null context");
    ctx->timing = enable != 0;
    for (int i = 0; i < FDR_NUM_KERNELS; ++i) ctx->ev_used[i] = 0;
    return FDR_OK;
}

FDR_EXPORT int fdr_timing_read(fdr_ctx *ctx, int which, int *count_out, float *total_ms_out) {
    int rc = use_device(ctx);
    if (rc) return rc;
    if (which < 0 || which >= FDR_NUM_KERNELS || !count_out || !total_ms_out)
        return fail(FDR_E_ARG, "fdr_timing_read: bad argument");
    float total = 0.f;
    const size_t used = ctx->ev_used[which];
    for (size_t i = 0; i + 1 < used; i += 2) {
        float ms = 0.f;
        HIP_TRY(hipEventSynchronize(ctx->ev_pool[which][i + 1]));
        HIP_TRY(hipEventElapsedTime(&ms, ctx->ev_pool[which][i], ctx->ev_pool[which][i + 1]));
        total += ms;
    }
    *count_out = (int)(used / 2);
    *total_ms_out = total;
    ctx->ev_used[which] = 0;
    return FDR_OK;
}

FDR_EXPORT int fdr_projection_load(fdr_ctx *ctx, int64_t n_features, int32_t d,
                                   const int64_t *p_indptr, const int32_t *p_cols,
                                   const float *p_vals) {
    int rc = use_device(ctx);
    if (rc) return rc;
    ProjectionTables T;
    if ((rc = build_projection_tables(n_features, d, p_indptr, p_cols, p_vals, T))) return rc;
    const std::vector<PU2> &ftab = T.ftab, &ent = T.ent;
    const std::vector<PU4> &crow = T.rowinfo;
    const int64_t nnz = p_indptr[n_features];
    const unsigned rows = T.rows;
    static_assert(sizeof(PU2) == sizeof(uint2) && sizeof(PU4) == sizeof(uint4), "table records = the kernel's uint2 / uint4");
    if ((rc = ctx->ftab.reserve(ftab.size() * sizeof(uint2)))) return rc;
    if ((rc = ctx->crow.reserve(crow.size() * sizeof(uint4)))) return rc;
    if ((rc = ctx->ent.reserve(ent.size() * sizeof(uint2)))) return rc;
    HIP_TRY(hipMemcpyAsync(ctx->ftab.p, ftab.data(), ftab.size() * sizeof(uint2), hipMemcpyHostToDevice, ctx->stream));
    HIP_TRY(hipMemcpyAsync(ctx->crow.p, crow.data(), crow.size() * sizeof(uint4), hipMemcpyHostToDevice, ctx->stream));
    HIP_TRY(hipMemcpyAsync(ctx->ent.p, ent.data(), ent.size() * sizeof(uint2), hipMemcpyHostToDevice, ctx->stream));
    HIP_TRY(hipStreamSynchronize(ctx->stream));
    ctx->n_features = n_features;
    ctx->d = d;
    ctx->p_nnz = nnz;
    ctx->p_rows = rows;
    ctx->h_bits.resize(ftab.size());
    for (size_t w = 0; w < ftab.size(); ++w) ctx->h_bits[w] = ftab[w].x;
    return FDR_OK;
}

FDR_EXPORT int fdr_csr_compact(fdr_ctx *ctx, int64_t n_rows, const int64_t *a_indptr, const int32_t *a_indices,
                               int64_t *out_indptr, int32_t *out_indices, int64_t out_capacity, int32_t n_threads) {
    if (!ctx) return fail(FDR_E_ARG, "null context");
    if (ctx->n_features <= 0) return fail(FDR_E_STATE, "csr_compact: no projection loaded");
    return csrc::compact(ctx->h_bits, ctx->n_features, n_rows, a_indptr, a_indices, out_indptr, out_indices,
                         out_capacity, n_threads);
}

FDR_EXPORT int fdr_host_register(fdr_ctx *ctx, void *ptr, size_t bytes) {
    int rc = use_device(ctx);
    if (rc) return rc;
    if (!ptr || bytes == 0) return fail(FDR_E_ARG, "host_register: empty buffer");
    HIP_TRY(hipHostRegister(ptr, bytes, hipHostRegisterDefault));
    return FDR_OK;
}

FDR_EXPORT int fdr_host_unregister(fdr_ctx *ctx, void *ptr) {
    int rc = use_device(ctx);
    if (rc) return rc;
    if (!ptr) return fail(FDR_E_ARG, "host_unregister: null pointer");
    HIP_TRY(hipHostUnregister(ptr));
    return FDR_OK;
}

static int launch_embed(fdr_ctx *ctx, int64_t n_rows, const int64_t *d_indptr,
                        const int32_t *d_indices, float *d_E, hipStream_t st) {
    if (ctx->n_features <= 0) return fail(FDR_E_STATE, "embed: no projection loaded");
    if (n_rows < 0) return fail(FDR_E_ARG, "embed: n_rows < 0");
    if (n_rows == 0) return FDR_OK;
    const int dp = fdr_padded_dim(ctx->d);
    const long long blocks_needed = (n_rows + 7) / 8;
    const int grid = (int)std::min<long long>(blocks_needed, (long long)ctx->num_cus * 8 * 4);
    int trc = timing_begin(ctx, FDR_KERNEL_EMBED, st);
    if (trc) return trc;
#define FDR_LAUNCH_EMBED(DP_)                                                                   \
    hipLaunchKernelGGL(FDR_EMBED_KERNEL<DP_>, dim3(grid), dim3(256), 0, st, (long long)n_rows,  \
                       (const long long *)d_indptr, d_indices, ctx->n_features,                 \
                       (const uint2 *)ctx->ftab.p, (const uint4 *)ctx->crow.p,                  \
                       (const uint2 *)ctx->ent.p, ctx->d, d_E)
#define FDR_EMBED_KERNEL embed_csr_kernel
    if (dp == 128)
        FDR_LAUNCH_EMBED(128);
    else if (dp == 256)
        FDR_LAUNCH_EMBED(256);
    else if (dp == 512)
        FDR_LAUNCH_EMBED(512);
#undef FDR_EMBED_KERNEL
#define FDR_EMBED_KERNEL embed_csr_wide_kernel
    else if (dp == 1024)
        FDR_LAUNCH_EMBED(1024);
    else
        FDR_LAUNCH_EMBED(2048);
#undef FDR_EMBED_KERNEL
#undef FDR_LAUNCH_EMBED
    HIP_TRY(hipGetLastError());
    return timing_end(ctx, FDR_KERNEL_EMBED, st);
}

static int launch_normalize(fdr_ctx *ctx, const float *d_E, int64_t n_rows, int d, float *d_Ehat,
                            uint8_t *d_zero, hipStream_t st) {
    const int dp = fdr_padded_dim(d);
    if (dp < 0) return fail(FDR_E_ARG, "normalize: dimension %d unsupported (1..%d)", d, FDR_MAX_DIM);
    if (n_rows < 0) return fail(FDR_E_ARG, "normalize: n_rows < 0");
    if (n_rows == 0) return FDR_OK;
    const int rb = dp == 128 ? 64 : dp == 256 ? 32 : dp == 512 ? 16 : dp == 1024 ? 8 : 4;
    const long long grid = (n_rows + rb - 1) / rb;
    if (grid > 0x7fffffffll) return fail(FDR_E_ARG, "normalize: too many rows");
    int trc = timing_begin(ctx, FDR_KERNEL_NORMALIZE, st);
    if (trc) return trc;
    const bool vec = d % 4 == 0 && (reinterpret_cast<uintptr_t>(d_E) & 15) == 0 && (reinterpret_cast<uintptr_t>(d_Ehat) & 15) == 0;
#define FDR_LAUNCH_NORM(DP_, RB_)                                                                                  \
    do {                                                                                                            \
        if (vec)                                                                                                    \
            hipLaunchKernelGGL((normalize_rows_kernel<DP_, RB_, true>), dim3((unsigned)grid), dim3(256), 0, st, d_E, \
                               (long long)n_rows, d, d_Ehat, d_zero);                                              \
        else                                                                                                        \
            hipLaunchKernelGGL((normalize_rows_kernel<DP_, RB_, false>), dim3((unsigned)grid), dim3(256), 0, st,    \
                               d_E, (long long)n_rows, d, d_Ehat, d_zero);                                         \
    } while (0)
    if (dp == 128) FDR_LAUNCH_NORM(128, 64);
    else if (dp == 256) FDR_LAUNCH_NORM(256, 32);
    else if (dp == 512) FDR_LAUNCH_NORM(512, 16);
    else if (dp == 1024) FDR_LAUNCH_NORM(1024, 8);
    else FDR_LAUNCH_NORM(2048, 4);
#undef FDR_LAUNCH_NORM
    HIP_TRY(hipGetLastError());
    return timing_end(ctx, FDR_KERNEL_NORMALIZE, st);
}

static size_t order_sort_tmp_bytes(size_t rows) {
    size_t t = 0;
    (void)rocprim::radix_sort_pairs(nullptr, t, (u64 *)nullptr, (u64 *)nullptr, (int *)nullptr, (int *)nullptr, rows, 0, 40,
                                    (hipStream_t) nullptr);
    return t;
}
static size_t class_tables_tmp_bytes(size_t rows) {
    size_t t_sort = 0, t_scan = 0;
    (void)rocprim::radix_sort_pairs(nullptr, t_sort, (u64 *)nullptr, (u64 *)nullptr, (int *)nullptr, (int *)nullptr, rows, 0,
                                    64, (hipStream_t) nullptr);
    (void)rocprim::inclusive_scan(nullptr, t_scan, (int *)nullptr, (int *)nullptr, rows, rocprim::plus<int>(),
                                  (hipStream_t) nullptr);
    return std::max(t_sort, t_scan);
}
static WsEnv ws_env(const fdr_ctx *ctx) {
    return {ctx->num_cus, ctx->knn_mode, ctx->dedup_mode, order_sort_tmp_bytes, class_tables_tmp_bytes, ctx->live_mode};
}

FDR_EXPORT size_t fdr_knn_workspace_bytes(fdr_ctx *ctx, int64_t nq, int64_t nt, int32_t d,
                                          int32_t k) {
    if (!ctx || nq <= 0 || nt <= 0 || k <= 0 || k > FDR_MAX_K || fdr_padded_dim(d) < 0) return 0;
    return knn_workspace_bytes(ws_env(ctx), nq, nt, d, k);
}

#ifndef FDR_SHAPE_MASK
#define FDR_SHAPE_MASK (~0ull)
#endif
#ifndef FDR_LH_MASK
#define FDR_LH_MASK 48
#endif
typedef void (*TileKernel)(const float *, const unsigned char *, int, const float *, const unsigned *, int, int, SegBounds,
                           int, int, u64 *, unsigned *, int, int, int FDR_DBG_PARAM);
typedef void (*PassKernel)(const _Float16 *, int, const _Float16 *, int, int, SegBounds, int, int, u64 *, unsigned *, int,
                           int, int, OrderArgs FDR_DBG_PARAM);
typedef void (*RangeKernel)(const _Float16 *, const float *, int, const _Float16 *, int, int, SegBounds, int *, int *);
static_assert(kShapes[FDR_R128].tps == RANGE_STAGES && kShapes[FDR_R256].tps == RANGE_STAGES &&
              kShapes[FDR_R512].tps == RANGE_STAGES, "the range kernel's ring");

template <int S>
static constexpr bool shape_compiled() {
    constexpr KnnShape e = kShapes[S];
#ifdef FDR_DEV
    constexpr bool built = true;
#else
    constexpr bool built = e.release;
#endif
    constexpr bool pass = e.family == FDR_FAM_PREFILTER || e.family == FDR_FAM_PINGPONG;
    return built && (!pass || (((unsigned long long)(FDR_SHAPE_MASK) >> S) & 1));
}
template <int S>
static constexpr TileKernel tile_kernel() {
    constexpr KnnShape e = kShapes[S];
    if constexpr (e.family == FDR_FAM_TILE && shape_compiled<S>()) return knn_tile_kernel<e.dp, e.nq, e.nw, e.wps>;
    else if constexpr (e.family == FDR_FAM_TILE_SPLIT && shape_compiled<S>()) return knn_tile_split_kernel<e.dp>;
    else return nullptr;
}
template <int S, int LH>
static constexpr PassKernel pass_kernel() {
    constexpr KnnShape e = kShapes[S];
    if constexpr (!shape_compiled<S>() || !(e.lists & LH & FDR_LH_MASK)) return nullptr;
    else if constexpr (e.family == FDR_FAM_PREFILTER)
        return knn_prefilter_kernel<e.dp, e.nq, e.nw, e.wps, e.units(), LH, e.paired && LH == 16>;
    else if constexpr (e.family == FDR_FAM_PINGPONG) return knn_prefilter_pp_kernel<e.dp, e.units(), LH>;
    else return nullptr;
}
template <int S>
static constexpr RangeKernel range_kernel() {
    constexpr KnnShape e = kShapes[S];
    if constexpr (!shape_compiled<S>()) return nullptr;
    else if constexpr (e.family == FDR_FAM_RANGE) return knn_range_kernel<e.dp, e.nw, e.dp == 128 ? e.wps : 2>;
    else if constexpr (e.family == FDR_FAM_RANGE_PP) return knn_range_pp_kernel<e.dp, e.units()>;
    else return nullptr;
}
template <size_t... S>
struct KnnKernelTable {
    static constexpr TileKernel tile[] = {tile_kernel<S>()...};
    static constexpr PassKernel pass[][2] = {{pass_kernel<S, 16>(), pass_kernel<S, 32>()}...};
    static constexpr RangeKernel range[] = {range_kernel<S>()...};
};
template <size_t... S>
static KnnKernelTable<S...> knn_kernel_table(std::index_sequence<S...>);
typedef decltype(knn_kernel_table(std::make_index_sequence<FDR_NUM_SHAPES>())) KnnKernels;

static int no_kernel(int shape) {
    return fail(FDR_E_STATE, "this development build was compiled without the kernel shape this call needs (kShapes[%d])",
                shape);
}

#include "knn_debug.inc"

struct Rounds { int launches = 0, queues = 0; };
template <class Launch>
static int launch_rounds(fdr_ctx *ctx, const KnnPlan &p, const std::vector<long long> &items, int max_queues, int kind,
                         bool span_each, hipStream_t st, Rounds &r, Launch launch) {
    const int dealt = p.cohort > 0 ? std::max(1, std::min(p.queues, max_queues)) : 1;
    const std::vector<RoundLaunch> sched = round_schedule(items, p.cohort > 0 ? p.cohort : 0, dealt);
    const int nqueues = sched.size() > 1 ? dealt : 1;
    hipStream_t qs[4] = {st, st, st, st};
    if (nqueues > 1) {
        if (!ctx->aux_ev[0]) {
            for (hipStream_t &a : ctx->aux_stream) HIP_TRY(hipStreamCreateWithFlags(&a, hipStreamNonBlocking));
            for (hipEvent_t &e : ctx->aux_ev) HIP_TRY(hipEventCreateWithFlags(&e, hipEventDisableTiming));
        }
        for (int q = 1; q < nqueues; ++q) qs[q] = ctx->aux_stream[q - 1];
    }
    const bool one_span = nqueues > 1 || !span_each;
    int trc;
    if (one_span && (trc = timing_begin(ctx, kind, st))) return trc;
    if (nqueues > 1) {
        HIP_TRY(hipEventRecord(ctx->aux_ev[0], st));
        for (int q = 1; q < nqueues; ++q) HIP_TRY(hipStreamWaitEvent(qs[q], ctx->aux_ev[0], 0));
    }
    for (const RoundLaunch &l : sched) {
        const hipStream_t ls = qs[l.queue];
        if (!one_span && (trc = timing_begin(ctx, kind, ls))) return trc;
        launch(ls, (unsigned)l.grid, l.base, l.group);
        if (!one_span && (trc = timing_end(ctx, kind, ls))) return trc;
    }
    HIP_TRY(hipGetLastError());
    r.launches = (int)sched.size();
    r.queues = nqueues;
    for (int q = 1; q < nqueues; ++q) {
        HIP_TRY(hipEventRecord(ctx->aux_ev[q], qs[q]));
        HIP_TRY(hipStreamWaitEvent(st, ctx->aux_ev[q], 0));
    }
    return one_span ? timing_end(ctx, kind, st) : FDR_OK;
}

static int check_knn_args(fdr_ctx *, const KnnArgs &a) {
    const int dp = fdr_padded_dim(a.d);
    if (dp < 0) return fail(FDR_E_ARG, "knn: dimension %d unsupported (1..%d)", a.d, FDR_MAX_DIM);
    if (a.k < 1 || a.k > FDR_MAX_K) return fail(FDR_E_ARG, "knn: k=%d, d=%d outside the MFMA kernels' shapes", a.k, a.d);
    if (a.nq < 0 || a.nt < a.k) return fail(FDR_E_ARG, "knn: need n_targets (%lld) >= k (%d)", (long long)a.nt, a.k);
    if (a.nt + a.t_base > 0x7fffffffll || a.nq > 0x7fffffffll) return fail(FDR_E_ARG, "knn: row numbers exceed int32");
    if (a.nq == 0) return FDR_OK;
    const bool need_ws = knn_route(dp, a.k, a.nt) != FDR_ROUTE_GENERIC;
    if (!a.Qhat || !a.qzero || !a.That || !a.tzero || !a.idx || !a.dist || (need_ws && !a.ws))
        return fail(FDR_E_ARG, "knn: null device pointer");
    return FDR_OK;
}
static_assert(FDR_MAX_K == FDR_EXACT_MAX_K, "every k the generic kernel takes, the exact MFMA pass takes from 8192 targets");

static int launch_knn_exact(fdr_ctx *ctx, const KnnArgs &a) {
    if (a.nq == 0) return FDR_OK;
    const hipStream_t st = a.st;
    const int k = a.k;
    const KnnPlan p = knn_plan(ctx->num_cus, a.nq, a.nt, a.d, k);
    if (a.ws_bytes < p.total_bytes) return fail(FDR_E_ARG, "knn: workspace %zu < required %zu bytes", a.ws_bytes, p.total_bytes);
    const TileKernel kern = KnnKernels::tile[p.shape];
    if (!kern) return no_kernel(p.shape);
    const PlanRegions R = plan_regions(a.ws, p);
    hipLaunchKernelGGL(pack_zero_bits_kernel, dim3((unsigned)((a.nt + 255) / 256)), dim3(256), 0, st,
                       a.tzero, (int)a.nt, R.bits, R.shared, p.nq_pad);
    HIP_TRY(hipGetLastError());
    const KnnShape &sh = kShapes[p.shape];
    const size_t lds = knn_lds_bytes(sh, k);
    if (lds > 160 * 1024) return fail(FDR_E_ARG, "knn: k=%d, d=%d needs %zu B of LDS (> 160 KiB)", k, a.d, lds);
    ctx->last.trace.exact_calls++;
    ctx->last.trace.exact_queries += (int32_t)a.nq;
    ctx->last.trace.exact_waves = sh.nw;
    ctx->last.trace.exact_qsets = sh.nq;
    ctx->last.trace.exact_segments = p.nseg;
    [[maybe_unused]] const int dbg = dev_knobs().debug;
    const int qcap = knn_qcap(sh, k);
    HIP_TRY(hipFuncSetAttribute(reinterpret_cast<const void *>(kern), hipFuncAttributeMaxDynamicSharedMemorySize, (int)lds));
    Rounds r;
    int trc = launch_rounds(ctx, p, {(long long)p.nqb * p.nseg}, 2, FDR_KERNEL_KNN_TILE, false, st, r,
                            [&](hipStream_t s, unsigned grid, int base, int) {
        hipLaunchKernelGGL(kern, dim3(grid), dim3(64 * sh.nw), lds, s, a.Qhat, a.qzero, (int)a.nq, a.That, R.bits, (int)a.nt,
                           (int)a.t_base, p.segs, k, p.nq_pad, R.partial, R.shared, qcap, base, p.nqb FDR_DBG_ARG(dbg));
    });
    if (trc) return trc;
    if ((trc = dump_debug_counters(st, "tile", p, "update calls, rounds, flushes, flush iterations, rescans, -"))) return trc;
    if ((trc = timing_begin(ctx, FDR_KERNEL_KNN_MERGE, st))) return trc;
    hipLaunchKernelGGL(k <= FDR_FAST_MAX_K ? knn_merge_kernel : knn_merge_wide_kernel, dim3((unsigned)((a.nq + 3) / 4)),
                       dim3(256), 0, st, (const u64 *)R.partial, p.nseg, (int)a.nq, p.nq_pad, k, a.idx, a.dist);
    HIP_TRY(hipGetLastError());
    return timing_end(ctx, FDR_KERNEL_KNN_MERGE, st);
}

struct PrefilterCounts { int exact, zero, range; };
struct PrefilterCall {
    fdr_ctx *ctx;
    KnnArgs a;
    bool self;
    int dp;
    PrefilterWs L;
    int shape;
    KnnPlan p;
    PassKernel kern;
    PlanRegions R;
    int ib;
    const _Float16 *p1_q, *p1_t;
    OrderArgs ord;
    const KnnShape &sh() const { return kShapes[shape]; }
    size_t lds() const { return knn_lds_bytes(sh(), L.kp); }
    _Float16 *hq() const { return self ? L.ht : L.hq; }
    int setup(), pass_dense(Rounds &r), pass_live(Rounds &r);
    int certify(PrefilterCounts &n), range(PrefilterCounts &n), exact_rest(const PrefilterCounts &n);
};

int PrefilterCall::setup() {
    const hipStream_t st = a.st;
    const int64_t nq = a.nq, nt = a.nt;
    int trc = timing_begin(ctx, FDR_KERNEL_KNN_RERANK, st);
    if (trc) return trc;
    hipLaunchKernelGGL(to_half_kernel, dim3((unsigned)((nt * (dp / 8) + 255) / 256)), dim3(256), 0, st, a.That,
                       (long long)nt * (dp / 8), L.ht);
    if (!self)
        hipLaunchKernelGGL(to_half_kernel, dim3((unsigned)((nq * (dp / 8) + 255) / 256)), dim3(256), 0, st, a.Qhat,
                           (long long)nq * (dp / 8), L.hq);
    hipLaunchKernelGGL(pack_zero_bits_kernel, dim3((unsigned)((nt + 255) / 256)), dim3(256), 0, st,
                       a.tzero, (int)nt, R.bits, R.shared, p.nq_pad);
    HIP_TRY(hipGetLastError());
    ord = {nullptr, nullptr};
    p1_q = hq();
    p1_t = L.ht;
    if (L.ordered) {
        _Float16 *const ho_t = L.ho_t, *const ho_q = self ? L.ho_t : L.ho_q;
        auto order = [&](const float *X, int64_t n, int *perm, _Float16 *out) -> int {
            hipLaunchKernelGGL(row_chunk_keys_kernel, dim3((unsigned)(((size_t)n * 16 + 255) / 256)), dim3(256), 0, st, X,
                               (int)n, dp, L.okeys, L.ovals);
            size_t tb = L.otmp_bytes;
            HIP_TRY(rocprim::radix_sort_pairs(L.otmp, tb, L.okeys, L.okeys_s, L.ovals, perm, (size_t)n, 0, 40, st));
            const long long groups = (long long)n * (dp / 8);
            hipLaunchKernelGGL(to_half_ordered_kernel, dim3((unsigned)((groups + 255) / 256)), dim3(256), 0, st, X,
                               (const int *)perm, groups, dp / 8, out);
            HIP_TRY(hipGetLastError());
            return FDR_OK;
        };
        int orc;
        if ((orc = order(a.That, nt, L.perm_t, ho_t))) return orc;
        if (!self && (orc = order(a.Qhat, nq, L.perm_q, ho_q))) return orc;
        ord.perm_t = L.perm_t;
        p1_t = ho_t;
        ord.perm_q = self ? L.perm_t : L.perm_q;
        p1_q = ho_q;
        if (L.live) {
            const long long bgroups = (long long)((nt + 31) / 32 + 4) * 32 * 16;
            hipLaunchKernelGGL(to_half_blocked_kernel, dim3((unsigned)((bgroups + 255) / 256)), dim3(256), 0, st, a.That,
                               (const int *)L.perm_t, (int)nt, bgroups, L.hb_t);
            hipLaunchKernelGGL(live_block_masks_kernel, dim3((unsigned)((nq + 255) / 256)), dim3(64), 0, st,
                               (const u64 *)L.okeys_s, (int)nq, L.live_masks);
            HIP_TRY(hipGetLastError());
        }
    }
    int max_seg = 1;
    for (int i = 0; i < p.nseg; ++i) max_seg = std::max(max_seg, p.segs.b[i + 1] - p.segs.b[i]);
    ib = prefilter_index_bits(max_seg);
    if (ib > FDR_PREFILTER_MAX_IB) return fail(FDR_E_ARG, "knn prefilter: segment of %d rows", max_seg);
    if ((trc = timing_end(ctx, FDR_KERNEL_KNN_RERANK, st))) return trc;
    if (lds() > 32768)
        HIP_TRY(hipFuncSetAttribute(reinterpret_cast<const void *>(kern), hipFuncAttributeMaxDynamicSharedMemorySize, (int)lds()));
    return FDR_OK;
}

int PrefilterCall::pass_dense(Rounds &r) {
    return launch_rounds(ctx, p, {(long long)p.nqb * p.nseg}, 4, FDR_KERNEL_KNN_PREFILTER, true, a.st, r,
                         [&](hipStream_t s, unsigned grid, int base, int) {
        hipLaunchKernelGGL(kern, dim3(grid), dim3(64 * sh().nw), lds(), s, p1_q, (int)a.nq, p1_t, (int)a.nt, (int)a.t_base,
                           p.segs, L.kp, p.nq_pad, R.partial, R.shared, ib, base, p.nqb, ord FDR_DBG_ARG(dev_knobs().debug));
    });
}

int PrefilterCall::pass_live(Rounds &r) {
    const hipStream_t st = a.st;
    const int nqb = p.nqb, kp = L.kp;
    fdr_knn_trace &tr = ctx->last.trace;
    std::vector<unsigned> &masks = ctx->live_host;
    masks.resize((size_t)nqb);
    HIP_TRY(hipMemcpyAsync(masks.data(), L.live_masks, (size_t)nqb * 4, hipMemcpyDeviceToHost, st));
    HIP_TRY(hipStreamSynchronize(st));
    const LivePlan lp = live_plan(masks.data(), nqb, p.nseg, ctx->live_mode == FDR_LIVE_FORCE ? 0 : p.cohort);
    HIP_TRY(hipMemcpyAsync(L.live_ids, lp.ids.data(), (size_t)nqb * 4, hipMemcpyHostToDevice, st));
    HIP_TRY(hipMemcpyAsync(L.live_order, lp.order.data(), (size_t)nqb * 4, hipMemcpyHostToDevice, st));
    HIP_TRY(hipStreamSynchronize(st));
    tr.pass_live = 1;
    int dense_nq = 0;
    std::vector<long long> items;
    for (const LiveGroup &g : lp.groups) {
        items.push_back((long long)g.count * p.nseg);
        if (g.nl != FDR_LIVE_DENSE) {
            tr.pass_live_items[g.nl - FDR_LIVE_MIN_NL] = g.count * p.nseg;
            continue;
        }
        tr.pass_live_dense_items = g.count * p.nseg;
        const int last = lp.order[(size_t)(g.first + g.count - 1)];
        dense_nq = (g.count - 1) * 256 + (int)std::min<int64_t>(256, a.nq - (int64_t)last * 256);
        hipLaunchKernelGGL(live_gather_dense_kernel, dim3((unsigned)g.count), dim3(256), 0, st, p1_q, ord.perm_q,
                           (const unsigned *)R.shared, (int)a.nq, (const int *)(L.live_order + g.first), L.live_hq,
                           L.live_perm, L.live_tau);
    }
    for (int nl = FDR_LIVE_MIN_NL; nl <= FDR_LIVE_MAX_NL; ++nl)
        if (live_lds_bytes(nl) > 32768)
            HIP_TRY(hipFuncSetAttribute(reinterpret_cast<const void *>(kLiveKernels[nl - FDR_LIVE_MIN_NL]),
                                        hipFuncAttributeMaxDynamicSharedMemorySize, (int)live_lds_bytes(nl)));
    return launch_rounds(ctx, p, items, 4, FDR_KERNEL_KNN_PREFILTER, false, st, r,
                         [&](hipStream_t s, unsigned grid, int base, int group) {
        const LiveGroup &g = lp.groups[(size_t)group];
        if (g.nl == FDR_LIVE_DENSE)
            hipLaunchKernelGGL(kern, dim3(grid), dim3(64 * sh().nw), lds(), s, (const _Float16 *)L.live_hq, dense_nq, p1_t,
                               (int)a.nt, (int)a.t_base, p.segs, kp, p.nq_pad, R.partial, L.live_tau, ib, base, g.count,
                               OrderArgs{ord.perm_t, (const int *)L.live_perm} FDR_DBG_ARG(dev_knobs().debug));
        else
            hipLaunchKernelGGL(kLiveKernels[g.nl - FDR_LIVE_MIN_NL], dim3(grid), dim3(512), live_lds_bytes(g.nl), s,
                               p1_q, (int)a.nq, (const _Float16 *)L.hb_t, (int)a.nt, (int)a.t_base, p.segs, kp, p.nq_pad,
                               R.partial, R.shared, ib, base, g.count, (const int *)(L.live_order + g.first),
                               (const unsigned *)L.live_ids, ord);
    });
}

int PrefilterCall::certify(PrefilterCounts &n) {
    const hipStream_t st = a.st;
    const int kp = L.kp, k = a.k;
    const int64_t nq = a.nq;
    int trc;
    if ((trc = timing_begin(ctx, FDR_KERNEL_KNN_RERANK, st))) return trc;
    const int64_t mq = p.nseg * kp <= 64 ? 4 * MERGE_QPW : 4;
    hipLaunchKernelGGL(knn_merge_keys_kernel, dim3((unsigned)((nq + mq - 1) / mq)), dim3(256), 0, st,
                       (const u64 *)R.partial, p.nseg, (int)nq, p.nq_pad, kp, L.cand);
    HIP_TRY(hipGetLastError());
    if (ctx->cap.what & FDR_CAPTURE_CANDIDATES) {
        if ((trc = ctx->cap.cand.reserve((size_t)nq * kp * 8))) return trc;
        HIP_TRY(hipMemcpyAsync(ctx->cap.cand.p, L.cand, (size_t)nq * kp * 8, hipMemcpyDeviceToDevice, st));
        ctx->cap.nq = nq;
        ctx->cap.kp = kp;
        ctx->cap.qbits = std::min(20, 32 - ib);
        ctx->cap.stream = st;
        ctx->cap.cand_valid = true;
    }
    HIP_TRY(hipMemsetAsync(L.counter, 0, 16, st));
    const float margin = 2.0f * prefilter_eps(ib) + 4.0e-7f;
    HIP_TRY(hipFuncSetAttribute(reinterpret_cast<const void *>(knn_rerank_kernel),
                                hipFuncAttributeMaxDynamicSharedMemorySize, RERANK_LDS_BYTES));
    hipLaunchKernelGGL(knn_rerank_kernel, dim3((unsigned)((nq + 3) / 4)), dim3(256), RERANK_LDS_BYTES, st,
                       (const u64 *)L.cand, kp, k, a.Qhat, a.qzero, a.That, (int)nq, dp, (int)a.t_base, margin,
                       a.idx, a.dist, L.counter, L.flagged, L.rlist, L.theta, L.path);
    hipLaunchKernelGGL(zero_answer_kernel, dim3(1), dim3(1024), 0, st, (const unsigned *)R.bits, (int)a.nt,
                       (int)a.t_base, k, L.zidx, L.zdist);
    hipLaunchKernelGGL(scatter_zero_answer_kernel, dim3((unsigned)(((int64_t)nq * k + 255) / 256)),
                       dim3(256), 0, st, (const int *)L.zidx, (const float *)L.zdist,
                       (const int *)L.flagged, (int)nq, (const int *)L.counter, k, a.idx, a.dist);
    HIP_TRY(hipGetLastError());
    if ((trc = timing_end(ctx, FDR_KERNEL_KNN_RERANK, st))) return trc;
    n = {0, 0, 0};
    HIP_TRY(hipMemcpyAsync(&n, L.counter, 12, hipMemcpyDeviceToHost, st));
    HIP_TRY(hipStreamSynchronize(st));
    ctx->last.pass.flagged = n.exact + n.range;
    ctx->last.trace.uncertified = n.exact;
    ctx->last.trace.zero_queries = n.zero;
    ctx->last.trace.range_queries = n.range;
    return FDR_OK;
}

int PrefilterCall::range(PrefilterCounts &n) {
    const hipStream_t st = a.st;
    const int rcount = n.range;
    fdr_knn_trace &tr = ctx->last.trace;
    int trc;
    if ((trc = timing_begin(ctx, FDR_KERNEL_KNN_RERANK, st))) return trc;
    const bool rcap = ctx->cap.what & FDR_CAPTURE_RANGE;
    if (rcap) {
        if ((trc = ctx->cap.rq.reserve((size_t)rcount * 4)) || (trc = ctx->cap.rtheta.reserve((size_t)rcount * 4)) ||
            (trc = ctx->cap.rcnt.reserve((size_t)rcount * 4)) || (trc = ctx->cap.rrows.reserve((size_t)rcount * RANGE_CAP * 4)))
            return trc;
        ctx->cap.stream = st;
    }
    for (int first = 0; first < rcount; first += L.rchunk) {
        const int cq = std::min(L.rchunk, rcount - first);
        hipLaunchKernelGGL(gather_half_queries_kernel, dim3((unsigned)cq), dim3(256), 0, st, (const _Float16 *)hq(),
                           (const float *)L.theta, (const int *)L.rlist, first, cq, dp, L.hqc, L.thetac, L.cnt);
        HIP_TRY(hipGetLastError());
        const int rs = range_shape(dp, cq, rcount);
        const KnnShape &rsh = kShapes[rs];
        const RangeKernel rk = KnnKernels::range[rs];
        if (!rk) return no_kernel(rs);
        const KnnPlan rp = knn_plan(ctx->num_cus, cq, a.nt, a.d, 1, rs);
        const size_t rlds = knn_lds_bytes(rsh, 1) + (size_t)RANGE_LANE_BUF * 64 * rsh.nw * 4;
        if (rsh.family == FDR_FAM_RANGE_PP)
            HIP_TRY(hipFuncSetAttribute(reinterpret_cast<const void *>(rk), hipFuncAttributeMaxDynamicSharedMemorySize, (int)rlds));
        hipLaunchKernelGGL(rk, dim3((unsigned)rp.nqb, (unsigned)rp.nseg), dim3(64 * rsh.nw), rlds, st, (const _Float16 *)L.hqc,
                           (const float *)L.thetac, cq, (const _Float16 *)L.ht, (int)a.nt, (int)a.t_base, rp.segs, L.cnt, L.rcand);
        HIP_TRY(hipGetLastError());
        tr.range_chunks++;
        tr.range_pp_chunks += rsh.family == FDR_FAM_RANGE_PP;
        tr.range_w8_chunks += rs == FDR_R128_W8;
        if (rcap) {
            auto keep = [&](const DevBuf &to, const void *from, size_t row_bytes) {
                return hipMemcpyAsync(static_cast<char *>(to.p) + first * row_bytes, from, cq * row_bytes, hipMemcpyDeviceToDevice, st);
            };
            HIP_TRY(keep(ctx->cap.rq, L.rlist + first, 4));
            HIP_TRY(keep(ctx->cap.rtheta, L.thetac, 4));
            HIP_TRY(keep(ctx->cap.rcnt, L.cnt, 4));
            HIP_TRY(keep(ctx->cap.rrows, L.rcand, (size_t)RANGE_CAP * 4));
        }
        hipLaunchKernelGGL(knn_rerank_long_kernel, dim3((unsigned)((cq + 3) / 4)), dim3(256), 0, st,
                           (const int *)(L.rlist + first), cq, (const int *)L.cnt, (const int *)L.rcand, a.k,
                           a.Qhat, a.That, dp, (int)a.t_base, a.idx, a.dist, L.counter, L.flagged, L.path);
        HIP_TRY(hipGetLastError());
    }
    if (rcap) {
        ctx->cap.n_range = rcount;
        ctx->cap.range_valid = true;
    }
    if ((trc = timing_end(ctx, FDR_KERNEL_KNN_RERANK, st))) return trc;
    int count = 0;
    HIP_TRY(hipMemcpyAsync(&count, L.counter, 4, hipMemcpyDeviceToHost, st));
    HIP_TRY(hipStreamSynchronize(st));
    tr.range_overflow = count - n.exact;
    n.exact = count;
    return FDR_OK;
}

int PrefilterCall::exact_rest(const PrefilterCounts &n) {
    const hipStream_t st = a.st;
    KnnArgs e = a;
    e.ws_bytes = L.knn_bytes;
    if ((int64_t)n.exact * 2 > a.nq - n.zero) {
        ctx->last.trace.exact_fallback = FDR_FALLBACK_WHOLE;
        ctx->last.paths = {nullptr, a.nq, FDR_PATH_EXACT, nullptr};
        return launch_knn_exact(ctx, e);
    }
    ctx->last.trace.exact_fallback = FDR_FALLBACK_CHUNKED;
    e.Qhat = L.qc;
    e.qzero = L.qzc;
    e.idx = L.idxc;
    e.dist = L.distc;
    for (int first = 0; first < n.exact; first += L.chunk) {
        const int cq = std::min(L.chunk, n.exact - first);
        hipLaunchKernelGGL(gather_queries_kernel, dim3((unsigned)cq), dim3(256), 0, st, a.Qhat, a.qzero,
                           (const int *)L.flagged, first, cq, dp, L.qc, L.qzc);
        HIP_TRY(hipGetLastError());
        e.nq = cq;
        int rc = launch_knn_exact(ctx, e);
        if (rc) return rc;
        hipLaunchKernelGGL(scatter_results_kernel, dim3((unsigned)(((int64_t)cq * a.k + 255) / 256)), dim3(256), 0, st,
                           (const int *)L.idxc, (const float *)L.distc, (const int *)L.flagged, first, cq, a.k, a.idx, a.dist);
        HIP_TRY(hipGetLastError());
    }
    return FDR_OK;
}

static int launch_knn_prefilter(fdr_ctx *ctx, const KnnArgs &a) {
    PrefilterCall c = {ctx, a};
    c.self = a.Qhat == a.That && a.qzero == a.tzero && a.nq == a.nt;
    c.dp = fdr_padded_dim(a.d);
    c.L = prefilter_ws(ws_env(ctx), a.ws, a.nq, a.nt, a.d, a.k);
    if (a.ws_bytes < c.L.total) return fail(FDR_E_ARG, "knn: workspace %zu < required %zu bytes", a.ws_bytes, c.L.total);
    const int kp = c.L.kp;
    knn_call_header(ctx, FDR_TRACE_PREFILTER, c.dp, a.k, a.nq, a.nt);
    ctx->last.paths = {c.L.path, a.nq, FDR_PATH_NONE, a.st};

    c.shape = prefilter_shape_live(ctx->live_mode, c.dp, kp, a.nq, ctx->num_cus, a.nt);
    c.p = knn_plan(ctx->num_cus, a.nq, a.nt, a.d, kp, c.shape);
    fdr_knn_trace &tr = ctx->last.trace;
    tr.kp = kp;
    tr.pass_waves = c.sh().nw;
    tr.pass_wps = c.sh().wps;
    tr.pass_units = c.sh().tps;
    tr.pass_list_keys = kp <= 32 ? 16 : 32;
    tr.pass_pingpong = c.sh().family == FDR_FAM_PINGPONG;
    tr.pass_segments = c.p.nseg;
    c.kern = KnnKernels::pass[c.shape][kp > 32];
    if (!c.kern) return no_kernel(c.shape);
    c.R = plan_regions(c.L.knn, c.p);
    int rc;
    if ((rc = c.setup())) return rc;
    Rounds r;
    rc = c.L.live ? c.pass_live(r) : c.pass_dense(r);
    ctx->last.pass.launches = r.launches;
    ctx->last.pass.queues = r.queues;
    tr.pass_launches = r.launches;
    tr.pass_queues = r.queues;
    if (rc) return rc;
#ifdef FDR_STAMPS
    if ((rc = dump_stamps(a.st, c.sh().nw))) return rc;
#endif
    if ((rc = dump_debug_counters(a.st, "prefilter", c.p, "wave-tiles, cold, groups, rounds, second rounds, candidates"))) return rc;
    PrefilterCounts n;
    if ((rc = c.certify(n))) return rc;
    if (n.range > 0 && (rc = c.range(n))) return rc;
    if (n.exact <= 0) return FDR_OK;
    return c.exact_rest(n);
}

static int launch_knn_mode(fdr_ctx *ctx, const KnnArgs &a) {
    const int dp = fdr_padded_dim(a.d);
    if (knn_route(dp, a.k, a.nt) == FDR_ROUTE_FAST && a.nq > 0 && knn_prefilter_wanted(ctx->knn_mode, a.nt, a.k)) {
        const int rc = launch_knn_prefilter(ctx, a);
        if (rc) ctx->cap.cand_valid = ctx->cap.range_valid = false;
        return rc;
    }
    knn_call_whole(ctx, FDR_PATH_EXACT, FDR_TRACE_EXACT, dp, a.k, a.nq, a.nt);
    return launch_knn_exact(ctx, a);
}

static int queue_class_tables(const DedupWs &W, const float *d_That, int n, int dp, hipStream_t st) {
    const unsigned g1 = (unsigned)((n + 255) / 256);
    size_t tb = W.tmp_bytes;
    HIP_TRY(rocprim::radix_sort_pairs(W.tmp, tb, W.hash, W.hash_s, W.idx, W.idx_s, (size_t)n, 0, 64, st));
    hipLaunchKernelGGL(mark_class_starts_kernel, dim3(g1), dim3(256), 0, st, d_That, n, dp, (const u64 *)W.hash_s,
                       (const int *)W.idx_s, W.flag);
    tb = W.tmp_bytes;
    HIP_TRY(rocprim::inclusive_scan(W.tmp, tb, W.flag, W.cid, (size_t)n, rocprim::plus<int>(), st));
    hipLaunchKernelGGL(class_tables_kernel, dim3(g1), dim3(256), 0, st, n, (const int *)W.flag, (const int *)W.cid,
                       (const int *)W.idx_s, W.cls, W.cstart, W.isrep);
    tb = W.tmp_bytes;
    HIP_TRY(rocprim::inclusive_scan(W.tmp, tb, W.isrep, W.upos, (size_t)n, rocprim::plus<int>(), st));
    hipLaunchKernelGGL(unique_tables_kernel, dim3(g1), dim3(256), 0, st, n, (const int *)W.isrep, (const int *)W.upos,
                       (const int *)W.cls, (const int *)W.cstart, W.uofc, W.cofu, W.rep_m);
    HIP_TRY(hipGetLastError());
    return FDR_OK;
}

static int launch_expand(const DedupWs &W, int64_t q0, int64_t nq, int k, int64_t t_base, const int *uqpos,
                         const int32_t *idx_u, const float *dist_u, int64_t u_stride, int32_t *d_idx, float *d_dist,
                         const uint8_t *upath, uint8_t path_all, uint8_t *rowpath, hipStream_t st) {
    const int xw = (size_t)4 * k * k * 8 <= 32768 ? 4 : (size_t)2 * k * k * 8 <= 32768 ? 2 : 1;
    const int xq = xw * (64 / k) * EXPAND_UNROLL;
    hipLaunchKernelGGL(expand_classes_kernel, dim3((unsigned)((nq + xq - 1) / xq)), dim3(64 * xw), (size_t)xw * k * k * 8,
                       st, (int)q0, (int)nq, k, 64 / k, (int)t_base, (const int *)W.cls, (const int *)W.uofc, uqpos,
                       (const int *)idx_u, dist_u, (const int *)W.idx_s, (const int4 *)W.rep_m, d_idx, d_dist,
                       (int)u_stride, upath, path_all, rowpath);
    HIP_TRY(hipGetLastError());
    return FDR_OK;
}

static int launch_knn(fdr_ctx *ctx, const KnnArgs &a) {
    int rc = check_knn_args(ctx, a);
    if (rc) return rc;
    const float *const d_Qhat = a.Qhat, *const d_That = a.That;
    const int64_t nq = a.nq, nt = a.nt;
    const int d = a.d, k = a.k;
    const hipStream_t st = a.st;
    const int dp = fdr_padded_dim(d);
    const int route = knn_route(dp, k, nt);
    if (route == FDR_ROUTE_GENERIC) {
        if (nq == 0) return FDR_OK;
        ctx->last.unique_targets = (int)nt;
        ctx->last.unique_queries = (int)nq;
        knn_call_whole(ctx, FDR_PATH_GENERIC, FDR_TRACE_GENERIC, dp, k, nq, nt);
        ctx->last.trace.generic = 1;
        int trc = timing_begin(ctx, FDR_KERNEL_KNN_TILE, st);
        if (trc) return trc;
        hipLaunchKernelGGL(knn_generic_kernel, dim3((unsigned)((nq + GEN_QPB - 1) / GEN_QPB)), dim3(256),
                           (size_t)GEN_QPB * dp * 4, st, d_Qhat, a.qzero, (int)nq, d_That, a.tzero, (int)nt, (int)a.t_base, dp, k,
                           a.idx, a.dist);
        HIP_TRY(hipGetLastError());
        return timing_end(ctx, FDR_KERNEL_KNN_TILE, st);
    }
    auto plain = [&](size_t bytes) {
        ctx->last.unique_targets = (int)nt;
        ctx->last.unique_queries = (int)nq;
        KnnArgs b = a;
        b.ws_bytes = bytes;
        return launch_knn_mode(ctx, b);
    };
    const bool q_in_t = nq > 0 && d_Qhat >= d_That && d_Qhat + (size_t)nq * dp <= d_That + (size_t)nt * dp &&
                        ((d_Qhat - d_That) % dp) == 0;
    if (!(route == FDR_ROUTE_FAST && q_in_t && knn_dedup_wanted(ctx->dedup_mode, nq, nt))) return plain(a.ws_bytes);
    const WsEnv env = ws_env(ctx);
    const DedupWs W = dedup_ws(env, a.ws, nq, nt, d, k);
    if (a.ws_bytes < W.total) return fail(FDR_E_ARG, "knn: workspace %zu < required %zu bytes", a.ws_bytes, W.total);
    const int n = (int)nt;
    const int q0 = (int)((d_Qhat - d_That) / dp);
    const unsigned g16 = (unsigned)(((size_t)n * 16 + 255) / 256), g1 = (unsigned)((n + 255) / 256);

    int trc = timing_begin(ctx, FDR_KERNEL_KNN_DEDUP, st);
    if (trc) return trc;
    hipLaunchKernelGGL(hash_rows_kernel, dim3(g16), dim3(256), 0, st, d_That, n, dp, W.hash, W.idx);
    HIP_TRY(hipGetLastError());
    if (ctx->dedup_mode != FDR_DEDUP_FORCE && W.probe_slots) {
        HIP_TRY(hipMemsetAsync(W.probe_table, 0, (size_t)W.probe_slots * 8 + 4, st));
        hipLaunchKernelGGL(dedup_probe_kernel, dim3(g1), dim3(256), 0, st, (const u64 *)W.hash, n, W.probe_table,
                           W.probe_slots - 1, W.probe_count);
        HIP_TRY(hipGetLastError());
        int dups = 0;
        HIP_TRY(hipMemcpyAsync(&dups, W.probe_count, 4, hipMemcpyDeviceToHost, st));
        HIP_TRY(hipStreamSynchronize(st));
        if ((double)dups < 0.05 * (double)n) {
            if ((trc = timing_end(ctx, FDR_KERNEL_KNN_DEDUP, st))) return trc;
            return plain(W.inner_bytes);
        }
    }
    if ((rc = queue_class_tables(W, d_That, n, dp, st))) return rc;
    HIP_TRY(hipMemsetAsync(W.uqflag, 0, (size_t)n * 4, st));
    hipLaunchKernelGGL(mark_query_classes_kernel, dim3((unsigned)((nq + 255) / 256)), dim3(256), 0, st, q0,
                       (int)nq, (const int *)W.cls, (const int *)W.uofc, W.uqflag);
    size_t tb = W.tmp_bytes;
    HIP_TRY(rocprim::inclusive_scan(W.tmp, tb, W.uqflag, W.uqpos, (size_t)n, rocprim::plus<int>(), st));
    HIP_TRY(hipGetLastError());
    int nu = 0, nuq = 0;
    HIP_TRY(hipMemcpyAsync(&nu, W.cid + (n - 1), 4, hipMemcpyDeviceToHost, st));
    HIP_TRY(hipMemcpyAsync(&nuq, W.uqpos + (n - 1), 4, hipMemcpyDeviceToHost, st));
    HIP_TRY(hipStreamSynchronize(st));
    if (!dedup_worth(nu, nuq, nt, nq, k, ctx->dedup_mode) || knn_mode_workspace_bytes(env, nuq, nu, d, k) > W.inner_bytes) {
        if ((trc = timing_end(ctx, FDR_KERNEL_KNN_DEDUP, st))) return trc;
        return plain(W.inner_bytes);
    }
    ctx->last.unique_targets = nu;
    ctx->last.unique_queries = nuq;
    hipLaunchKernelGGL(gather_unique_rows_kernel, dim3(g16), dim3(256), 0, st, d_That, a.tzero, n, dp,
                       (const int *)W.isrep, (const int *)W.upos, W.U, W.uzero);
    if (nuq != nu)
        hipLaunchKernelGGL(gather_unique_queries_kernel, dim3((unsigned)(((size_t)nu * 16 + 255) / 256)), dim3(256),
                           0, st, (const float *)W.U, (const unsigned char *)W.uzero, nu, dp, (const int *)W.uqflag,
                           (const int *)W.uqpos, W.Uq, W.uqz);
    HIP_TRY(hipGetLastError());
    if ((trc = timing_end(ctx, FDR_KERNEL_KNN_DEDUP, st))) return trc;
    const bool all_q = nuq == nu;
    KnnArgs u = a;
    u.Qhat = all_q ? W.U : W.Uq;
    u.qzero = all_q ? W.uzero : W.uqz;
    u.nq = nuq;
    u.That = W.U;
    u.tzero = W.uzero;
    u.nt = nu;
    u.t_base = 0;
    u.idx = W.idx_u;
    u.dist = W.dist_u;
    u.ws_bytes = W.inner_bytes;
    if ((rc = launch_knn_mode(ctx, u))) return rc;
    if ((trc = timing_begin(ctx, FDR_KERNEL_KNN_DEDUP, st))) return trc;
    const auto &inner = ctx->last.paths;
    if ((rc = launch_expand(W, q0, nq, k, a.t_base, W.uqpos, W.idx_u, W.dist_u, k, a.idx, a.dist,
                            inner.n == nuq ? inner.dev : nullptr, inner.all, W.rowpath, st)))
        return rc;
    ctx->last.paths = {W.rowpath, nq, FDR_PATH_NONE, st};
    return timing_end(ctx, FDR_KERNEL_KNN_DEDUP, st);
}

FDR_EXPORT int fdr_knn_classes_dev(fdr_ctx *ctx, const float *d_That, const uint8_t *d_tzero, int64_t nt, int32_t d,
                                   int32_t k, int64_t nq_max, void *d_ws, size_t ws_bytes, void *stream,
                                   int32_t *n_unique_out) {
    int rc = use_device(ctx);
    if (rc) return rc;
    knn_call_begin(ctx);
    hipStream_t st = (hipStream_t)stream;
    ctx->cls.valid = false;
    if (!n_unique_out) return fail(FDR_E_ARG, "knn_classes: n_unique_out is null");
    *n_unique_out = 0;
    const int dp = fdr_padded_dim(d);
    if (dp < 0 || k < 1 || k > FDR_MAX_K || nt < k || nq_max <= 0 || nq_max > nt || !d_That || !d_tzero || !d_ws ||
        nt > 0x7fffffffll)
        return fail(FDR_E_ARG, "knn_classes: bad argument");
    if (knn_route(dp, k, nt) != FDR_ROUTE_FAST) return FDR_OK;
    if (!knn_dedup_wanted(ctx->dedup_mode, nq_max, nt)) return FDR_OK;
    const DedupWs W = dedup_ws(ws_env(ctx), d_ws, nq_max, nt, d, k);
    if (ws_bytes < W.total) return fail(FDR_E_ARG, "knn_classes: workspace %zu < required %zu bytes", ws_bytes, W.total);
    const int n = (int)nt;
    const unsigned g16 = (unsigned)(((size_t)n * 16 + 255) / 256);
    int trc = timing_begin(ctx, FDR_KERNEL_KNN_DEDUP, st);
    if (trc) return trc;
    hipLaunchKernelGGL(hash_rows_kernel, dim3(g16), dim3(256), 0, st, d_That, n, dp, W.hash, W.idx);
    HIP_TRY(hipGetLastError());
    if ((rc = queue_class_tables(W, d_That, n, dp, st))) return rc;
    int nu = 0;
    HIP_TRY(hipMemcpyAsync(&nu, W.cid + (n - 1), 4, hipMemcpyDeviceToHost, st));
    HIP_TRY(hipStreamSynchronize(st));
    if (!dedup_worth(nu, nu, nt, nt, k, ctx->dedup_mode)) return timing_end(ctx, FDR_KERNEL_KNN_DEDUP, st);
    hipLaunchKernelGGL(gather_unique_rows_kernel, dim3(g16), dim3(256), 0, st, d_That, d_tzero, n, dp,
                       (const int *)W.isrep, (const int *)W.upos, W.U, W.uzero);
    HIP_TRY(hipGetLastError());
    if ((trc = timing_end(ctx, FDR_KERNEL_KNN_DEDUP, st))) return trc;
    ctx->cls.valid = true;
    ctx->cls.That = d_That;
    ctx->cls.tzero = d_tzero;
    ctx->cls.nt = nt;
    ctx->cls.nq_max = nq_max;
    ctx->cls.d = d;
    ctx->cls.k = k;
    ctx->cls.nu = nu;
    ctx->cls.ws = d_ws;
    ctx->cls.ws_bytes = ws_bytes;
    ctx->last.unique_targets = nu;
    *n_unique_out = nu;
    return FDR_OK;
}

static DedupWs classes_ws(const fdr_ctx *ctx) {
    return dedup_ws(ws_env(ctx), ctx->cls.ws, ctx->cls.nq_max, ctx->cls.nt, ctx->cls.d, ctx->cls.k);
}

FDR_EXPORT int fdr_knn_unique_dev(fdr_ctx *ctx, int64_t u_lo, int64_t u_hi, int32_t *d_idx_u, float *d_dist_u,
                                  void *stream) {
    int rc = use_device(ctx);
    if (rc) return rc;
    knn_call_begin(ctx);
    if (!ctx->cls.valid) return fail(FDR_E_STATE, "knn_unique: no classes (call fdr_knn_classes_dev first)");
    if (u_lo < 0 || u_hi < u_lo || u_hi > ctx->cls.nu || u_hi - u_lo > ctx->cls.nq_max)
        return fail(FDR_E_ARG, "knn_unique: bad range [%lld, %lld) of %d unique rows (at most %lld per call)",
                    (long long)u_lo, (long long)u_hi, ctx->cls.nu, (long long)ctx->cls.nq_max);
    if (u_hi == u_lo) return FDR_OK;
    if (!d_idx_u || !d_dist_u) return fail(FDR_E_ARG, "knn_unique: null output");
    const int dp = fdr_padded_dim(ctx->cls.d);
    const DedupWs W = classes_ws(ctx);
    ctx->last.unique_queries = (int)(u_hi - u_lo);
    rc = launch_knn_mode(ctx, KnnArgs{W.U + (size_t)u_lo * dp, W.uzero + u_lo, u_hi - u_lo, W.U, W.uzero, ctx->cls.nu, 0,
                                      ctx->cls.d, ctx->cls.k, d_idx_u, d_dist_u, ctx->cls.ws, W.inner_bytes,
                                      (hipStream_t)stream});
    ctx->last.paths = {};
    return rc;
}

FDR_EXPORT int fdr_knn_expand_dev(fdr_ctx *ctx, int64_t q0, int64_t nq, int64_t t_base, const int32_t *d_idx_u_all,
                                  const float *d_dist_u_all, int64_t u_row_stride, int32_t *d_idx, float *d_dist,
                                  void *stream) {
    int rc = use_device(ctx);
    if (rc) return rc;
    knn_call_begin(ctx);
    if (!ctx->cls.valid) return fail(FDR_E_STATE, "knn_expand: no classes (call fdr_knn_classes_dev first)");
    if (q0 < 0 || nq < 0 || q0 + nq > ctx->cls.nt) return fail(FDR_E_ARG, "knn_expand: bad row range");
    if (nq == 0) return FDR_OK;
    if (!d_idx_u_all || !d_dist_u_all || !d_idx || !d_dist) return fail(FDR_E_ARG, "knn_expand: null pointer");
    hipStream_t st = (hipStream_t)stream;
    const int k = ctx->cls.k;
    if (u_row_stride == 0) u_row_stride = k;
    if (u_row_stride < k || u_row_stride > 0x7fffffffll) return fail(FDR_E_ARG, "knn_expand: bad row stride");
    int trc = timing_begin(ctx, FDR_KERNEL_KNN_DEDUP, st);
    if (trc) return trc;
    if ((rc = launch_expand(classes_ws(ctx), q0, nq, k, t_base, nullptr, d_idx_u_all, d_dist_u_all, u_row_stride, d_idx,
                            d_dist, nullptr, 0, nullptr, st)))
        return rc;
    return timing_end(ctx, FDR_KERNEL_KNN_DEDUP, st);
}

FDR_EXPORT int fdr_embed_dev(fdr_ctx *ctx, int64_t n_rows, const int64_t *d_indptr,
                             const int32_t *d_indices, float *d_E, void *stream) {
    int rc = use_device(ctx);
    if (rc) return rc;
    if (n_rows > 0 && (!d_indptr || !d_E)) return fail(FDR_E_ARG, "embed: null device pointer");
    return launch_embed(ctx, n_rows, d_indptr, d_indices, d_E, (hipStream_t)stream);
}

FDR_EXPORT int fdr_normalize_dev(fdr_ctx *ctx, const float *d_E, int64_t n_rows, int32_t d,
                                 float *d_Ehat, uint8_t *d_zero, void *stream) {
    int rc = use_device(ctx);
    if (rc) return rc;
    if (n_rows > 0 && (!d_E || !d_Ehat || !d_zero)) return fail(FDR_E_ARG, "normalize: null device pointer");
    return launch_normalize(ctx, d_E, n_rows, d, d_Ehat, d_zero, (hipStream_t)stream);
}

FDR_EXPORT int fdr_knn_dev(fdr_ctx *ctx, const float *d_Qhat, const uint8_t *d_qzero, int64_t nq,
                           const float *d_That, const uint8_t *d_tzero, int64_t nt, int64_t t_base,
                           int32_t d, int32_t k, int32_t *d_idx, float *d_dist, void *d_workspace,
                           size_t workspace_bytes, void *stream) {
    int rc = use_device(ctx);
    if (rc) return rc;
    knn_call_begin(ctx);
    if (d_workspace == ctx->cls.ws) ctx->cls.valid = false;
    return launch_knn(ctx, KnnArgs{d_Qhat, d_qzero, nq, d_That, d_tzero, nt, t_base, d, k, d_idx, d_dist, d_workspace,
                                   workspace_bytes, (hipStream_t)stream});
}

static int check_csr(int64_t n_rows, const int64_t *a_indptr, const int32_t *a_indices) {
    if (n_rows < 0 || !a_indptr) return fail(FDR_E_ARG, "embed: bad CSR (n_rows=%lld)", (long long)n_rows);
    if (a_indptr[0] != 0 || a_indptr[n_rows] < 0) return fail(FDR_E_ARG, "embed: bad indptr");
    if (a_indptr[n_rows] > 0 && !a_indices) return fail(FDR_E_ARG, "embed: indices is null");
    return FDR_OK;
}

static int upload_csr(fdr_ctx *ctx, int64_t n_rows, const int64_t *a_indptr,
                      const int32_t *a_indices) {
    int rc;
    const int64_t nnz = a_indptr[n_rows];
    if ((rc = ctx->a_indptr.reserve((size_t)(n_rows + 1) * 8))) return rc;
    if ((rc = ctx->a_indices.reserve((size_t)std::max<int64_t>(nnz, 1) * 4))) return rc;
    HIP_TRY(hipMemcpyAsync(ctx->a_indptr.p, a_indptr, (size_t)(n_rows + 1) * 8, hipMemcpyHostToDevice, ctx->stream));
    if (nnz > 0)
        HIP_TRY(hipMemcpyAsync(ctx->a_indices.p, a_indices, (size_t)nnz * 4, hipMemcpyHostToDevice, ctx->stream));
    return FDR_OK;
}

struct UploadLink {
    fdr_ctx *ctx;
    int64_t n_rows;
    const int64_t *a_indptr;
    const int32_t *a_indices;
    float *d_E;
    int64_t stage_cap;
    int send_raw(int64_t r0, int64_t r1, int slot) {
        hipStream_t st = ctx->stream;
        const int64_t o = a_indptr[r0], len = a_indptr[r1] - o;
        if (len > 0)
            HIP_TRY(hipMemcpyAsync((int32_t *)ctx->a_indices.p + o, a_indices + o, (size_t)len * 4, hipMemcpyHostToDevice, st));
        int erc = launch_embed(ctx, r1 - r0, (const int64_t *)ctx->a_indptr.p + r0, (const int32_t *)ctx->a_indices.p,
                               d_E + (size_t)r0 * ctx->d, st);
        if (erc) return erc;
        if (slot >= 0) HIP_TRY(hipEventRecord(ctx->up_ev[slot], st));
        return FDR_OK;
    }
    int wait_slot(int slot) {
        HIP_TRY(hipEventSynchronize(ctx->up_ev[slot]));
        return FDR_OK;
    }
    int send_staged(int64_t rb, int64_t used) {
        hipStream_t st = ctx->stream;
        const int32_t *stage_ids = (const int32_t *)ctx->stage_ids.p;
        const int64_t *stage_ptr = (const int64_t *)ctx->stage_ptr.p;
        if (used > 0)
            HIP_TRY(hipMemcpyAsync((int32_t *)ctx->c_indices.p + (stage_cap - used), stage_ids + (stage_cap - used),
                                   (size_t)used * 4, hipMemcpyHostToDevice, st));
        HIP_TRY(hipMemcpyAsync((int64_t *)ctx->c_indptr.p + rb, stage_ptr + rb, (size_t)(n_rows - rb + 1) * 8,
                               hipMemcpyHostToDevice, st));
        HIP_TRY(hipEventRecord(ctx->up_ev[2], st));
        return launch_embed(ctx, n_rows - rb, (const int64_t *)ctx->c_indptr.p + rb, (const int32_t *)ctx->c_indices.p,
                            d_E + (size_t)rb * ctx->d, st);
    }
};

static int upload_embed_pipelined(fdr_ctx *ctx, int64_t n_rows, const int64_t *a_indptr, const int32_t *a_indices,
                                  float *d_E) {
    int rc;
    const int64_t nnz = a_indptr[n_rows];
    const hup::Tuning tune;
    if (nnz < tune.min_ids || ctx->h_bits.empty()) {
        if ((rc = upload_csr(ctx, n_rows, a_indptr, a_indices))) return rc;
        return launch_embed(ctx, n_rows, (const int64_t *)ctx->a_indptr.p, (const int32_t *)ctx->a_indices.p, d_E, ctx->stream);
    }
    for (hipEvent_t &e : ctx->up_ev)
        if (!e) HIP_TRY(hipEventCreateWithFlags(&e, hipEventDisableTiming));
    HIP_TRY(hipEventSynchronize(ctx->up_ev[2]));
    const int64_t stage_cap = hup::Tuning::stage_cap(nnz);
    if ((rc = ctx->a_indptr.reserve((size_t)(n_rows + 1) * 8))) return rc;
    if ((rc = ctx->a_indices.reserve((size_t)nnz * 4))) return rc;
    if ((rc = ctx->c_indptr.reserve((size_t)(n_rows + 1) * 8))) return rc;
    if ((rc = ctx->c_indices.reserve((size_t)stage_cap * 4))) return rc;
    if ((rc = ctx->stage_ids.reserve((size_t)stage_cap * 4))) return rc;
    if ((rc = ctx->stage_ptr.reserve((size_t)(n_rows + 1) * 8))) return rc;
    HIP_TRY(hipMemcpyAsync(ctx->a_indptr.p, a_indptr, (size_t)(n_rows + 1) * 8, hipMemcpyHostToDevice, ctx->stream));
    UploadLink link{ctx, n_rows, a_indptr, a_indices, d_E, stage_cap};
    return hup::upload(tune, n_rows, a_indptr, a_indices, ctx->h_bits.data(), (uint64_t)ctx->n_features,
                       (int32_t *)ctx->stage_ids.p, (int64_t *)ctx->stage_ptr.p, stage_cap, ctx->up_pool,
                       hup::Tuning::helpers(host_cpu_budget()), link)
        .rc;
}

FDR_EXPORT int fdr_embed(fdr_ctx *ctx, int64_t n_rows, const int64_t *a_indptr,
                         const int32_t *a_indices, float *E_out) {
    int rc = use_device(ctx);
    if (rc) return rc;
    if ((rc = check_csr(n_rows, a_indptr, a_indices))) return rc;
    if (ctx->n_features <= 0) return fail(FDR_E_STATE, "embed: no projection loaded");
    if (n_rows == 0) return FDR_OK;
    if (!E_out) return fail(FDR_E_ARG, "embed: E_out is null");
    const size_t ebytes = (size_t)n_rows * ctx->d * 4;
    if ((rc = ctx->E.reserve(ebytes))) return rc;
    if ((rc = upload_embed_pipelined(ctx, n_rows, a_indptr, a_indices, (float *)ctx->E.p))) return rc;
    HIP_TRY(hipMemcpyAsync(E_out, ctx->E.p, ebytes, hipMemcpyDeviceToHost, ctx->stream));
    HIP_TRY(hipStreamSynchronize(ctx->stream));
    return FDR_OK;
}

static int knn_from_device_E(fdr_ctx *ctx, const float *d_E, int64_t n, int d, int k,
                             int32_t *idx_out, float *dist_out) {
    int rc;
    const int dp = fdr_padded_dim(d);
    if (dp < 0) return fail(FDR_E_ARG, "knn: dimension %d unsupported (1..%d)", d, FDR_MAX_DIM);
    if (k < 1 || k > FDR_MAX_K) return fail(FDR_E_ARG, "knn: k=%d unsupported (1..%d)", k, FDR_MAX_K);
    if (n < k) return fail(FDR_E_ARG, "knn: need n (%lld) >= k (%d)", (long long)n, k);
    if (!idx_out || !dist_out) return fail(FDR_E_ARG, "knn: null output pointer");
    if ((rc = ctx->Ehat.reserve((size_t)n * dp * 4))) return rc;
    if ((rc = ctx->zero.reserve((size_t)n))) return rc;
    if ((rc = ctx->idx.reserve((size_t)n * k * 4))) return rc;
    if ((rc = ctx->dist.reserve((size_t)n * k * 4))) return rc;
    const size_t wsb = fdr_knn_workspace_bytes(ctx, n, n, d, k);
    if ((rc = ctx->ws.reserve(wsb))) return rc;
    if ((rc = launch_normalize(ctx, d_E, n, d, (float *)ctx->Ehat.p, (uint8_t *)ctx->zero.p, ctx->stream)))
        return rc;
    const float *const Ehat = (const float *)ctx->Ehat.p;
    const uint8_t *const zero = (const uint8_t *)ctx->zero.p;
    const KnnArgs a = {Ehat, zero, n, Ehat, zero, n, 0, d, k, (int32_t *)ctx->idx.p, (float *)ctx->dist.p, ctx->ws.p, wsb, ctx->stream};
    if ((rc = launch_knn(ctx, a))) return rc;
    HIP_TRY(hipMemcpyAsync(idx_out, ctx->idx.p, (size_t)n * k * 4, hipMemcpyDeviceToHost, ctx->stream));
    HIP_TRY(hipMemcpyAsync(dist_out, ctx->dist.p, (size_t)n * k * 4, hipMemcpyDeviceToHost, ctx->stream));
    HIP_TRY(hipStreamSynchronize(ctx->stream));
    return FDR_OK;
}

FDR_EXPORT int fdr_knn(fdr_ctx *ctx, const float *E, int64_t n, int32_t d, int32_t k,
                       int32_t *idx_out, float *dist_out) {
    int rc = use_device(ctx);
    if (rc) return rc;
    knn_call_begin(ctx);
    if (!E || n <= 0) return fail(FDR_E_ARG, "knn: empty input");
    if (fdr_padded_dim(d) < 0) return fail(FDR_E_ARG, "knn: dimension %d unsupported (1..%d)", d, FDR_MAX_DIM);
    if ((rc = ctx->E.reserve((size_t)n * d * 4))) return rc;
    HIP_TRY(hipMemcpyAsync(ctx->E.p, E, (size_t)n * d * 4, hipMemcpyHostToDevice, ctx->stream));
    return knn_from_device_E(ctx, (const float *)ctx->E.p, n, d, k, idx_out, dist_out);
}

FDR_EXPORT int fdr_embed_knn(fdr_ctx *ctx, int64_t n_rows, const int64_t *a_indptr,
                             const int32_t *a_indices, int32_t k, int32_t *idx_out, float *dist_out,
                             float *E_out) {
    int rc = use_device(ctx);
    if (rc) return rc;
    knn_call_begin(ctx);
    if ((rc = check_csr(n_rows, a_indptr, a_indices))) return rc;
    if (ctx->n_features <= 0) return fail(FDR_E_STATE, "embed: no projection loaded");
    if (n_rows <= 0) return fail(FDR_E_ARG, "embed_knn: empty input");
    const size_t ebytes = (size_t)n_rows * ctx->d * 4;
    if ((rc = ctx->E.reserve(ebytes))) return rc;
    if ((rc = upload_embed_pipelined(ctx, n_rows, a_indptr, a_indices, (float *)ctx->E.p))) return rc;
    if (E_out) HIP_TRY(hipMemcpyAsync(E_out, ctx->E.p, ebytes, hipMemcpyDeviceToHost, ctx->stream));
    return knn_from_device_E(ctx, (const float *)ctx->E.p, n_rows, ctx->d, k, idx_out, dist_out);
}

#include "knn_sparse.inc"
#include "kmer_search.inc"
#include "kmer_output_loader.inc"
#include "reads_parser.inc"
#include "overlaps_writer.inc"
```

fedrann_amd/csrc/host_common.inc:

```
#define FDR_EXPORT extern "C" __attribute__((visibility("default")))
typedef unsigned long long u64;

#ifndef FDR_W8_DEFAULT
#define FDR_W8_DEFAULT 1
#endif
struct DevKnobs {
    int extra = 0;
    int w8 = FDR_W8_DEFAULT;
    int d256 = 3;
    int shape = -1;
    int slots = 0;
    double ov = 0.0;
    int nseg = 0;
    int streams = -1;
    int cohort_slots = 0;
    int cohort = 1;
    int cohort_ns = 0;
    int range8 = -1;
    int xrounds = 0;
    int ordered = 0;
    int rangepp = -1;
    int pp = -1;
    int debug = 0;
};
#ifdef FDR_DEV
static DevKnobs dev_knobs() {
    DevKnobs k;
    auto geti = [](const char *name, int &v) { if (const char *e = getenv(name)) v = atoi(e); };
    geti("FDR_KNN_EXTRA", k.extra);
    geti("FDR_KNN_W8", k.w8);
    geti("FDR_KNN_D256", k.d256);
    geti("FDR_KNN_SHAPE", k.shape);
    geti("FDR_KNN_SLOTS", k.slots);
    if (const char *e = getenv("FDR_KNN_OV")) k.ov = atof(e);
    geti("FDR_KNN_NSEG", k.nseg);
    geti("FDR_KNN_STREAMS", k.streams);
    geti("FDR_KNN_COHORT_SLOTS", k.cohort_slots);
    geti("FDR_KNN_COHORT", k.cohort);
    geti("FDR_KNN_COHORT_NS", k.cohort_ns);
    geti("FDR_KNN_RANGE8", k.range8);
    geti("FDR_KNN_XROUNDS", k.xrounds);
    geti("FDR_KNN_ORDERED", k.ordered);
    geti("FDR_KNN_PP", k.pp);
    geti("FDR_KNN_RANGEPP", k.rangepp);
    geti("FDR_KNN_DEBUG", k.debug);
    return k;
}
#else
static constexpr DevKnobs dev_knobs() { return DevKnobs(); }
#endif

static int host_cpu_budget() {
    int n = (int)std::thread::hardware_concurrency();
    if (n < 1) n = 1;
    if (FILE *f = fopen("/sys/fs/cgroup/cpu.max", "r")) {
        char q[32];
        long long period = 0;
        if (fscanf(f, "%31s %lld", q, &period) == 2 && strcmp(q, "max") != 0 && period > 0) {
            const long long quota = atoll(q);
            if (quota > 0) n = (int)std::max<long long>(1, std::min<long long>(n, quota / period));
        }
        fclose(f);
    }
    return n;
}

static thread_local char g_err[512] = "";

static int fail(int code, const char *fmt, ...) {
    va_list ap;
    va_start(ap, fmt);
    vsnprintf(g_err, sizeof(g_err), fmt, ap);
    va_end(ap);
    return code;
}
```

fedrann_amd/csrc/knn_prefilter_live.inc:

```

__global__ __launch_bounds__(64) void live_block_masks_kernel(const u64 *__restrict__ keys_s, int nq,
                                                              unsigned *__restrict__ masks) {
    const int b = blockIdx.x, lane = threadIdx.x;
    unsigned m = 0;
#pragma unroll
    for (int i = 0; i < 4; ++i) {
        const int r = b * 256 + i * 64 + lane;
        if (r < nq) m |= (unsigned)keys_s[r] & 0xffu;
    }
#pragma unroll
    for (int off = 32; off >= 1; off >>= 1) m |= __shfl_xor(m, off);
    if (lane == 0) masks[b] = m;
}

__global__ __launch_bounds__(256) void to_half_blocked_kernel(const float *__restrict__ Ehat,
                                                              const int *__restrict__ perm, int n, long long n_groups,
                                                              _Float16 *__restrict__ out) {
    const long long t = (long long)blockIdx.x * 256 + threadIdx.x;
    if (t >= n_groups) return;
    const long long i = t >> 4;
    const int g = (int)(t & 15);
    f16x8 h;
#pragma unroll
    for (int e = 0; e < 8; ++e) h[e] = (_Float16)0.0f;
    if (i < n) {
        const f32x4 *src = reinterpret_cast<const f32x4 *>(Ehat) + ((size_t)perm[i] * 16 + g) * 2;
        const f32x4 e = src[0], o = src[1];
        h[0] = (_Float16)e.x; h[1] = (_Float16)o.x; h[2] = (_Float16)e.y; h[3] = (_Float16)o.y;
        h[4] = (_Float16)e.z; h[5] = (_Float16)o.z; h[6] = (_Float16)e.w; h[7] = (_Float16)o.w;
    }
    const size_t slot = ((((size_t)(i >> 5) * 8 + (size_t)(g >> 1)) * 32 + (size_t)(i & 31)) << 1) + (size_t)(g & 1);
    reinterpret_cast<f16x8 *>(out)[slot] = h;
}

__global__ __launch_bounds__(256) void live_gather_dense_kernel(const _Float16 *__restrict__ hq, const int *__restrict__ perm_q,
                                                                const unsigned *__restrict__ tau, int nq,
                                                                const int *__restrict__ blocks, _Float16 *__restrict__ out_q,
                                                                int *__restrict__ out_perm, unsigned *__restrict__ out_tau) {
    const int b = blocks[blockIdx.x];
    const int sub = threadIdx.x & 15;
    for (int r = threadIdx.x >> 4; r < 256; r += 16) {
        const int src = b * 256 + r, dst = blockIdx.x * 256 + r;
        if (src >= nq) {
            if (sub == 0) out_tau[dst] = 0x7F800000u;
            continue;
        }
        reinterpret_cast<f16x8 *>(out_q)[(size_t)dst * 16 + sub] = reinterpret_cast<const f16x8 *>(hq)[(size_t)src * 16 + sub];
        if (sub == 0) {
            out_perm[dst] = perm_q[src];
            out_tau[dst] = tau[src];
        }
    }
}

template <int NL>
__global__ __launch_bounds__(512, 4) void knn_prefilter_live_kernel(
    const _Float16 *__restrict__ Qh, int nq, const _Float16 *__restrict__ Tb, int nt, int t_base, SegBounds segs, int K,
    int nq_pad, u64 *__restrict__ partial, unsigned *__restrict__ tau_shared, int ib, int item_base, int nb,
    const int *__restrict__ blocks, const unsigned *__restrict__ live_ids, OrderArgs ord) {
    static_assert(NL >= FDR_LIVE_MIN_NL && NL <= FDR_LIVE_MAX_NL, "instances NL = 2 .. 6");
    extern __shared__ __attribute__((aligned(16))) unsigned char smem[];
    constexpr int DP = 128, NW = 8, U = 4, LH = 16, QW = 32 * NW;
    constexpr int TILE_BYTES = 8 * 1024;
    constexpr int UNIT_BYTES = NL * 1024;
    constexpr int STAGE_BYTES = U * UNIT_BYTES;
    constexpr int NPIECE = U * NL;
    constexpr int PPW = (NPIECE + NW - 1) / NW;
    const int item = item_base + (int)blockIdx.x;
    const int seg = item / nb;
    const int qb = __builtin_amdgcn_readfirstlane(blocks[item - seg * nb]);
    const unsigned ids = __builtin_amdgcn_readfirstlane(live_ids[qb]);

    const int tid = threadIdx.x;
    const int lane = tid & 63;
    const int wave = __builtin_amdgcn_readfirstlane(tid >> 6);
    const int j = lane & 31, h = lane >> 5;
    const int ql0 = wave * 32 + j;
    const int qg0 = qb * QW + ql0;

    f16x8 b[NL];
    {
        const f16x8 *qp = reinterpret_cast<const f16x8 *>(Qh + (size_t)(qg0 < nq ? qg0 : nq - 1) * DP);
#pragma unroll
        for (int s = 0; s < NL; ++s) b[s] = qp[2 * (int)((ids >> (4 * s)) & 7u) + h];
    }
    const int qbits = min(20, 32 - ib);
    const unsigned QM1 = (1u << qbits) - 2u;
    const float qscale = (float)QM1, qinv = 1.0f / qscale;
    const int nlive = (K - h + 1) >> 1, dead = LH - nlive;
    RegList<LH> L;
    unsigned flim;
    int cthr;
#pragma unroll
    for (int e = 0; e < LH; ++e) L.v[e] = e < dead ? 0u : PK_EMPTY;
    L.pmax = PK_EMPTY;
    auto share = [&](RegList<LH> &Ln, unsigned &fl) {
        unsigned *slot = tau_shared + qg0;
        const unsigned tk = max(Ln.v[LH - 1], Ln.pmax);
        const unsigned mine = tk == PK_EMPTY ? 0x7F800000u : (tk >> ib);
        unsigned seen = mine;
        if (h == 0) {
            const unsigned old = mine <= QM1
                                     ? __hip_atomic_fetch_min(slot, mine, __ATOMIC_RELAXED, __HIP_MEMORY_SCOPE_AGENT)
                                     : __hip_atomic_load(slot, __ATOMIC_RELAXED, __HIP_MEMORY_SCOPE_AGENT);
            seen = min(old, mine);
        }
        const unsigned ps = partner32(seen, h);
        fl = min(h ? ps : seen, QM1 + 1);
    };
    auto rethreshold = [&](const RegList<LH> &Ln, unsigned fl) -> int {
        const unsigned tk = max(Ln.v[LH - 1], Ln.pmax);
        const unsigned oq = tk >> ib;
        const unsigned lim = tk == PK_EMPTY ? fl : min(oq - 1u, fl);
        int th = lim >= QM1 ? (int)0x80000000u : __float_as_int(((float)(QM1 - lim) - 0.75f) * qinv) + 1;
        if (tk != PK_EMPTY && oq == 0u) th = 0x7fffffff;
        return th;
    };
    share(L, flim);
    cthr = rethreshold(L, flim);

    const int t_begin = segs.b[seg];
    const int t_end = min(nt, segs.b[seg + 1]);
    const int nunits = (t_end - t_begin + 31) >> 5;
    const int nstages = (nunits + U - 1) / U;

    const char *seg_base = reinterpret_cast<const char *>(Tb) + (size_t)(t_begin >> 5) * TILE_BYTES;
    unsigned poff[PPW];
#pragma unroll
    for (int u = 0; u < PPW; ++u) {
        const int p = min(wave + NW * u, NPIECE - 1);
        const int tl = p / NL, s = p - tl * NL;
        poff[u] = (unsigned)(tl * TILE_BYTES) + ((ids >> (4 * s)) & 7u) * 1024u;
    }
    unsigned soff = (unsigned)((lane & 31) * 32 + (lane >> 5) * 16);
    auto issue_stage = [&](auto par_c) {
        constexpr int par = decltype(par_c)::value;
        unsigned char *dst = smem + par * STAGE_BYTES;
        static_for(std::make_integer_sequence<int, PPW>{}, [&](auto u_c) {
            constexpr int u = decltype(u_c)::value;
            if (NW * (u + 1) <= NPIECE || wave < NPIECE - NW * u)
                __builtin_amdgcn_global_load_lds((const __attribute__((address_space(1))) void *)(seg_base + (soff + poff[u])),
                                                 (__attribute__((address_space(3))) void *)(dst + (wave + NW * u) * 1024),
                                                 16, 0, 0);
        });
        soff += (unsigned)(U * TILE_BYTES);
    };
    if (nstages > 0) issue_stage(std::integral_constant<int, 0>{});
    __syncthreads();

    unsigned q0 = PK_EMPTY, q1 = PK_EMPTY;
    auto flush = [&](RegList<LH> &Ln, unsigned &a0, unsigned &a1) {
        while (__any(a0 != PK_EMPTY)) {
            const unsigned took = reglist_round<LH>(Ln, a0, h);
            if (a0 == took) {
                a0 = a1;
                a1 = PK_EMPTY;
            }
        }
    };
    auto offer = [&](const f32x16 &a, const int (&g)[4], RegList<LH> &Ln, unsigned &a0, unsigned &a1,
                     const unsigned fl, const int th, int lrow, int nvalid) {
#pragma unroll
        for (int q4 = 0; q4 < 4; ++q4) {
            if (!__any(g[q4] >= th)) continue;
#pragma unroll
            for (int r = 4 * q4; r < 4 * q4 + 4; ++r) {
                const int roff = (r & 3) + 8 * (r >> 2);
                const bool pass = __float_as_int(a[r]) >= th && roff + 4 * h < nvalid;
                if (!__any(pass)) continue;
                unsigned cand = PK_EMPTY;
                if (pass) {
                    const float sc = fminf(fmaxf(a[r], 0.0f), 1.0f);
                    const unsigned qd = QM1 - (unsigned)__builtin_rintf(sc * qscale);
                    if (qd <= fl) cand = (qd << ib) | (unsigned)(lrow + roff);
                }
                if (__any(cand != PK_EMPTY && a1 != PK_EMPTY)) flush(Ln, a0, a1);
                a1 = (a0 != PK_EMPTY && a1 == PK_EMPTY) ? cand : a1;
                a0 = a0 == PK_EMPTY ? cand : a0;
            }
        }
    };
    unsigned fa = (unsigned)(size_t)(__attribute__((address_space(3))) const unsigned char *)smem + (unsigned)lane * 16u;
    asm volatile("" : "+v"(fa));

    f32x16 acc, accB;
#pragma unroll
    for (int r = 0; r < 16; ++r) acc[r] = accB[r] = 0.f;

    auto score = [&](const f32x16 &av, int t) __attribute__((always_inline)) {
        int g[4];
#pragma unroll
        for (int q4 = 0; q4 < 4; ++q4)
            g[q4] = max(max(max(__float_as_int(av[4 * q4]), __float_as_int(av[4 * q4 + 1])),
                            __float_as_int(av[4 * q4 + 2])),
                        __float_as_int(av[4 * q4 + 3]));
        const int mx = max(max(max(g[0], g[1]), g[2]), g[3]);
        if (__any(mx >= cthr)) {
            int lrow = t * 32 + 4 * h;
            int nvalid = t_end - (t_begin + t * 32);
            asm volatile("" : "+v"(lrow), "+s"(nvalid));
            offer(av, g, L, q0, q1, flim, cthr, lrow, nvalid);
            cthr = rethreshold(L, flim);
        }
    };
    constexpr int NP = U / 2;
    const bool late = wave >= NW / 2;
#ifdef FDR_STAMPS
    unsigned stamp_acc[6] = {0, 0, 0, 0, 0, 0};
    const bool stamp_on = blockIdx.x == 0;
#endif
    auto stage_body = [&](auto par_c, int it) {
        constexpr int par = decltype(par_c)::value;
        STAMP(ts0);
        if (it + 1 < nstages) issue_stage(std::integral_constant<int, par ^ 1>{});
        STAMP(ts1);
        STAMP_ADD(0, ts0, ts1);
        auto mfma_pair = [&](auto p_c) __attribute__((always_inline)) {
            constexpr int OFF0 = par * STAGE_BYTES + 2 * decltype(p_c)::value * UNIT_BYTES, OFF1 = OFF0 + UNIT_BYTES;
            f16x8 fa0[2], fa1[2];
            lds_read128(fa0[0], fa, std::integral_constant<int, OFF0>{});
            lds_read128(fa1[0], fa, std::integral_constant<int, OFF1>{});
            static_for(std::make_integer_sequence<int, NL>{}, [&](auto s_c) {
                constexpr int s = decltype(s_c)::value;
                if constexpr (s < NL - 1) {
                    lds_read128(fa0[(s + 1) & 1], fa, std::integral_constant<int, OFF0 + (s + 1) * 1024>{});
                    lds_read128(fa1[(s + 1) & 1], fa, std::integral_constant<int, OFF1 + (s + 1) * 1024>{});
                    asm volatile("s_waitcnt lgkmcnt(2)" : "+v"(fa0[s & 1]), "+v"(fa1[s & 1]));
                } else {
                    asm volatile("s_waitcnt lgkmcnt(0)" : "+v"(fa0[s & 1]), "+v"(fa1[s & 1]));
                }
                __builtin_amdgcn_sched_barrier(0);
                acc = __builtin_amdgcn_mfma_f32_32x32x16_f16(fa0[s & 1], b[s], s == 0 ? f32x16{} : acc, 0, 0, 0);
                accB = __builtin_amdgcn_mfma_f32_32x32x16_f16(fa1[s & 1], b[s], s == 0 ? f32x16{} : accB, 0, 0, 0);
                __builtin_amdgcn_sched_barrier(0);
            });
        };
        auto score_pair = [&](const int ts) __attribute__((always_inline)) {
            score(acc, ts);
            if (ts + 1 < nunits) score(accB, ts + 1);
        };
        if (late && it > 0 && U * it - 2 < nunits) score_pair(U * it - 2);
        if (it < nstages) {
            static_for(std::make_integer_sequence<int, NP>{}, [&](auto p_c) {
                constexpr int p = decltype(p_c)::value;
                const int tp = U * it + 2 * p;
                if (tp < nunits) {
                    mfma_pair(p_c);
                    if (!late || p < NP - 1) score_pair(tp);
                }
            });
        }
        STAMP(ts2);
        STAMP_ADD(1, ts1, ts2);
        if ((it & FDR_SHARE_EVERY) == FDR_SHARE_EVERY) {
            flush(L, q0, q1);
            share(L, flim);
            cthr = rethreshold(L, flim);
        }
        STAMP(ts3);
        STAMP_ADD(2, ts2, ts3);
#ifdef FDR_STAMPS
        asm volatile("s_waitcnt vmcnt(0)" ::: "memory");
        STAMP(ts3b);
        STAMP_ADD(3, ts3, ts3b);
        __syncthreads();
        STAMP(ts4);
        STAMP_ADD(4, ts3b, ts4);
        if (stamp_on) stamp_acc[5] += 1;
#else
        __syncthreads();
#endif
    };
    const int niter = nstages + 1;
    for (int it0 = 0; it0 < niter; it0 += 2) {
        stage_body(std::integral_constant<int, 0>{}, it0);
        if (it0 + 1 < niter) stage_body(std::integral_constant<int, 1>{}, it0 + 1);
    }
#ifdef FDR_STAMPS
    if (stamp_on && lane == 0)
        for (int ph = 0; ph < 6; ++ph) atomicAdd(&g_stamps[wave][ph], (unsigned long long)stamp_acc[ph]);
#endif
    const unsigned imask = (1u << ib) - 1u;
    flush(L, q0, q1);
    size_t qrow = (size_t)qb * QW + ql0;
    if (qrow >= (size_t)nq) return;
    qrow = (size_t)ord.perm_q[qrow];
    u64 *out = partial + ((size_t)seg * nq_pad + qrow) * K + (h ? (K + 1) >> 1 : 0);
#pragma unroll
    for (int e = 0; e < LH; ++e) {
        if (e >= dead) {
            const unsigned kv = L.v[e];
            u64 o = KEY_INF;
            if (kv != PK_EMPTY) {
                const int trow = ord.perm_t[t_begin + (int)(kv & imask)];
                o = ((u64)__float_as_uint((float)(kv >> ib) / qscale) << 32) | (unsigned)(t_base + trow);
            }
            out[e - dead] = o;
        }
    }
}

typedef void (*LiveKernel)(const _Float16 *, int, const _Float16 *, int, int, SegBounds, int, int, u64 *, unsigned *, int,
                           int, int, const int *, const unsigned *, OrderArgs);
static constexpr LiveKernel kLiveKernels[FDR_LIVE_MAX_NL - FDR_LIVE_MIN_NL + 1] = {
    knn_prefilter_live_kernel<2>, knn_prefilter_live_kernel<3>, knn_prefilter_live_kernel<4>,
    knn_prefilter_live_kernel<5>, knn_prefilter_live_kernel<6>};
static size_t live_lds_bytes(int nl) { return (size_t)2 * 4 * nl * 1024; }
```

fedrann_amd/csrc/knn_workspace.inc:

```
#ifdef __HIPCC__
typedef _Float16 ws_half;
typedef int4 ws_int4;
#else
typedef uint16_t ws_half;
struct ws_int4 {
    int x, y, z, w;
};
#endif

#define RANGE_CAP 1024
static_assert(RANGE_CAP == FDR_RANGE_CAP, "fdr_last_range_sets's row length (include/fedrann_hip.h)");
#define FDR_DEDUP_PROBE_BELOW (1 << 18)

static size_t align256(size_t x) { return (x + 255) / 256 * 256; }

struct WsRegion {
    size_t off, bytes;
};
struct WsArena {
    char *base;
    std::vector<WsRegion> *log = nullptr;
    size_t at = 0;
    template <class T>
    T *take(size_t count) {
        const size_t off = at;
        at += align256(count * sizeof(T));
        if (log) log->push_back({off, count * sizeof(T)});
        return base ? reinterpret_cast<T *>(base + off) : nullptr;
    }
};
template <class T>
static T *ws_at(T *region, size_t n) { return region ? region + n : nullptr; }

struct PlanRegions {
    unsigned *bits, *shared;
    u64 *partial;
};
static PlanRegions plan_regions(void *base, const KnnPlan &p) {
    char *const b = static_cast<char *>(base);
    return {reinterpret_cast<unsigned *>(b), reinterpret_cast<unsigned *>(b + p.bits_bytes),
            reinterpret_cast<u64 *>(b + p.bits_bytes + p.shared_bytes)};
}

struct WsEnv {
    int num_cus, knn_mode, dedup_mode;
    size_t (*order_sort_tmp)(size_t rows);
    size_t (*class_tables_tmp)(size_t rows);
    int live_mode = FDR_LIVE_AUTO;
};

#define FDR_LIVE_AUTO_ON 1
static int prefilter_shape_live(int live_mode, int dp, int kp, int64_t nq, int num_cus, int64_t nt) {
    if (live_mode == FDR_LIVE_FORCE && dp == 128 && kp <= 32) return FDR_P128_W8U4;
    return prefilter_shape(dp, kp, nq, num_cus, nt);
}
static bool live_chunks_wanted(int live_mode, int shape, const KnnPlan &pp) {
    if (live_mode == FDR_LIVE_OFF || shape != FDR_P128_W8U4) return false;
    return live_mode == FDR_LIVE_FORCE || (FDR_LIVE_AUTO_ON && pp.cohort > 0 && pp.queues == 2);
}

static bool knn_prefilter_wanted(int knn_mode, int64_t nt, int k) {
    if (knn_mode == FDR_MODE_EXACT) return false;
    const int kp = (k + prefilter_extra(k) + 1) & ~1;
    if (!(kp <= FDR_FAST_MAX_K && nt >= kp)) return false;
    if (nt > (int64_t)FDR_MAX_SEG << FDR_PREFILTER_MAX_IB) return false;
    return knn_mode == FDR_MODE_PREFILTER || nt >= 8192;
}

static bool knn_dedup_wanted(int dedup_mode, int64_t nq, int64_t nt) {
    if (dedup_mode != FDR_DEDUP_AUTO) return dedup_mode != FDR_DEDUP_OFF;
    return nt >= 8192 && nq >= 1024;
}

static bool dedup_worth(int nu, int nuq, int64_t nt, int64_t nq, int k, int dedup_mode) {
    if (nu < k) return false;
    return dedup_mode == FDR_DEDUP_FORCE || (double)nu * nuq <= 0.9 * (double)nt * (double)nq;
}

struct PrefilterWs {
    int kp, chunk, rchunk;
    int ordered;
    size_t knn_bytes, otmp_bytes, total;
    char *knn;
    ws_half *ht, *hq;
    u64 *cand;
    int *counter;
    int *zidx;
    float *zdist;
    int *flagged;
    float *qc;
    uint8_t *qzc;
    int32_t *idxc;
    float *distc;
    int *rlist;
    float *theta;
    ws_half *hqc;
    float *thetac;
    int *cnt, *rcand;
    uint8_t *path;
    u64 *okeys, *okeys_s;
    int *ovals, *perm_t, *perm_q;
    ws_half *ho_t, *ho_q;
    char *otmp;
    int live;
    ws_half *hb_t;
    unsigned *live_masks, *live_ids;
    int *live_order;
    ws_half *live_hq;
    int *live_perm;
    unsigned *live_tau;
};

static PrefilterWs prefilter_ws(const WsEnv &env, void *base, int64_t nq, int64_t nt, int d, int k,
                                std::vector<WsRegion> *log = nullptr) {
    PrefilterWs L = {};
    WsArena A{static_cast<char *>(base), log};
    L.kp = (k + prefilter_extra(k) + 1) & ~1;
    L.chunk = (int)std::min<int64_t>(nq, 16384);
    L.rchunk = (int)std::min<int64_t>(nq, 32768);
    const size_t exact_all = knn_plan(env.num_cus, nq, nt, d, k).total_bytes;
    const int dp = padded_dim(d);
    const int pshape = prefilter_shape_live(env.live_mode, dp, L.kp, nq, env.num_cus, nt);
    const KnnPlan pp = knn_plan(env.num_cus, nq, nt, d, L.kp, pshape);
    const size_t pre = std::max(pp.total_bytes, pp.bits_bytes + align256((size_t)(nq + 512) * 4) +
                                                    prefilter_partial_bound(nq, nt, L.kp, pp.qw));
    const size_t chunk_bound = align256((size_t)((nt + 31) / 32) * 4) + align256((size_t)(L.chunk + 128) * 4) +
                               (size_t)FDR_MAX_SEG * (L.chunk + 128) * (size_t)k * 8;
    L.knn_bytes = align256(std::max(exact_all, std::max(pre, chunk_bound)));
    L.knn = A.take<char>(L.knn_bytes);
    L.ht = A.take<ws_half>((size_t)nt * dp);
    L.hq = A.take<ws_half>((size_t)nq * dp);
    L.cand = A.take<u64>((size_t)nq * L.kp);
    L.counter = A.take<int>(256);
    L.zidx = ws_at(L.counter, 64);
    L.zdist = reinterpret_cast<float *>(ws_at(L.counter, 128));
    L.flagged = A.take<int>((size_t)nq);
    L.qc = A.take<float>((size_t)L.chunk * dp);
    L.qzc = A.take<uint8_t>((size_t)L.chunk);
    L.idxc = A.take<int32_t>((size_t)L.chunk * k);
    L.distc = A.take<float>((size_t)L.chunk * k);
    L.rlist = A.take<int>((size_t)nq);
    L.theta = A.take<float>((size_t)nq);
    L.hqc = A.take<ws_half>((size_t)L.rchunk * dp);
    L.thetac = A.take<float>((size_t)L.rchunk);
    L.cnt = A.take<int>((size_t)L.rchunk);
    L.rcand = A.take<int>((size_t)L.rchunk * RANGE_CAP);
    L.path = A.take<uint8_t>((size_t)nq);
    L.live = live_chunks_wanted(env.live_mode, pshape, pp);
    L.ordered = pp.cohort > 0 || dev_knobs().ordered != 0 || L.live;
    if (L.ordered) {
        const size_t nmax = (size_t)std::max(nq, nt);
        L.okeys = A.take<u64>(nmax);
        L.okeys_s = A.take<u64>(nmax);
        L.ovals = A.take<int>(nmax);
        L.perm_t = A.take<int>((size_t)nt);
        L.perm_q = A.take<int>((size_t)nq);
        L.ho_t = A.take<ws_half>((size_t)nt * dp);
        L.ho_q = A.take<ws_half>((size_t)nq * dp);
        L.otmp_bytes = align256(env.order_sort_tmp(nmax));
        L.otmp = A.take<char>(L.otmp_bytes);
    }
    if (L.live) {
        L.hb_t = A.take<ws_half>(((size_t)(nt + 31) / 32 + 4) * 32 * dp);
        const size_t nqb = (size_t)(nq + 255) / 256;
        L.live_masks = A.take<unsigned>(nqb);
        L.live_ids = A.take<unsigned>(nqb);
        L.live_order = A.take<int>(nqb);
        L.live_hq = A.take<ws_half>(nqb * 256 * dp);
        L.live_perm = A.take<int>(nqb * 256);
        L.live_tau = A.take<unsigned>(nqb * 256);
    }
    L.total = A.at;
    return L;
}

static size_t knn_mode_workspace_bytes(const WsEnv &env, int64_t nq, int64_t nt, int d, int k) {
    if (knn_prefilter_wanted(env.knn_mode, nt, k)) return prefilter_ws(env, nullptr, nq, nt, d, k).total;
    return knn_plan(env.num_cus, nq, nt, d, k).total_bytes;
}

struct DedupWs {
    size_t inner_bytes, tmp_bytes, total;
    char *inner;
    u64 *hash, *hash_s;
    ws_int4 *rep_m;
    int *idx, *idx_s, *flag, *cid, *cls, *cstart, *isrep, *upos, *uofc, *cofu, *uqflag, *uqpos;
    float *U;
    unsigned probe_slots;
    u64 *probe_table;
    int *probe_count;
    uint8_t *uzero;
    float *Uq;
    uint8_t *uqz;
    int32_t *idx_u;
    float *dist_u;
    uint8_t *rowpath;
    char *tmp;
};

static DedupWs dedup_ws(const WsEnv &env, void *base, int64_t nq, int64_t nt, int d, int k,
                        std::vector<WsRegion> *log = nullptr) {
    DedupWs L = {};
    WsArena A{static_cast<char *>(base), log};
    const int dp = padded_dim(d);
    const size_t n = (size_t)nt, hash_words = align256(n * 8) / 8;
    L.inner_bytes = align256(knn_mode_workspace_bytes(env, nq, nt, d, k));
    L.inner = A.take<char>(L.inner_bytes);
    L.hash = A.take<u64>(hash_words + n);
    L.hash_s = ws_at(L.hash, hash_words);
    L.rep_m = reinterpret_cast<ws_int4 *>(L.hash);
    L.idx = A.take<int>(n);
    L.idx_s = A.take<int>(n);
    L.flag = A.take<int>(n);
    L.cid = A.take<int>(n);
    L.cls = A.take<int>(n);
    L.cstart = A.take<int>(n + 1);
    L.isrep = A.take<int>(n);
    L.upos = A.take<int>(n);
    L.uofc = A.take<int>(n);
    L.cofu = A.take<int>(n);
    L.uqflag = A.take<int>(n);
    L.uqpos = A.take<int>(n);
    L.U = A.take<float>(n * dp);
    if (nt < FDR_DEDUP_PROBE_BELOW) {
        unsigned tsize = 1024;
        while (tsize < 2u * (unsigned)n) tsize <<= 1;
        if ((size_t)tsize * 8 + 256 <= n * dp * 4) {
            L.probe_slots = tsize;
            L.probe_table = reinterpret_cast<u64 *>(L.U);
            L.probe_count = reinterpret_cast<int *>(ws_at(L.probe_table, tsize));
        }
    }
    L.uzero = A.take<uint8_t>(n);
    L.Uq = A.take<float>((size_t)nq * dp);
    L.uqz = A.take<uint8_t>((size_t)nq);
    L.idx_u = A.take<int32_t>((size_t)nq * k);
    L.dist_u = A.take<float>((size_t)nq * k);
    L.rowpath = A.take<uint8_t>((size_t)nq);
    L.tmp_bytes = align256(env.class_tables_tmp(n));
    L.tmp = A.take<char>(L.tmp_bytes);
    L.total = A.at;
    return L;
}

static size_t knn_workspace_bytes(const WsEnv &env, int64_t nq, int64_t nt, int d, int k) {
    const int route = knn_route(padded_dim(d), k, nt);
    if (route == FDR_ROUTE_GENERIC) return 256;
    if (route == FDR_ROUTE_WIDE) return knn_plan(env.num_cus, nq, nt, d, k).total_bytes;
    if (knn_dedup_wanted(env.dedup_mode, nq, nt)) return dedup_ws(env, nullptr, nq, nt, d, k).total;
    return knn_mode_workspace_bytes(env, nq, nt, d, k);
}
```

include/fedrann_hip.h:

```cpp
#ifndef FEDRANN_HIP_H
#define FEDRANN_HIP_H

#include <stddef.h>
#include <stdint.h>

#ifdef __cplusplus
extern "C" {
#endif

#define FDR_OK 0
#define FDR_E_ARG (-1)
#define FDR_E_HIP (-2)
#define FDR_E_NOMEM (-4)
#define FDR_E_STATE (-5)
#define FDR_E_IO (-6)

#define FDR_MAX_K 128
#define FDR_MAX_DIM 2048

typedef struct fdr_ctx fdr_ctx;

int fdr_create(int device_id, fdr_ctx **out);
int fdr_destroy(fdr_ctx *ctx);
const char *fdr_last_error(void);
int fdr_device_info(fdr_ctx *ctx, char *buf, int buflen);
int fdr_padded_dim(int d);

int fdr_projection_load(fdr_ctx *ctx, int64_t n_features, int32_t d, const int64_t *p_indptr,
                        const int32_t *p_cols, const float *p_vals);

int fdr_csr_compact(fdr_ctx *ctx, int64_t n_rows, const int64_t *a_indptr, const int32_t *a_indices,
                    int64_t *out_indptr, int32_t *out_indices, int64_t out_capacity, int32_t n_threads);

int fdr_host_register(fdr_ctx *ctx, void *ptr, size_t bytes);
int fdr_host_unregister(fdr_ctx *ctx, void *ptr);

int fdr_embed(fdr_ctx *ctx, int64_t n_rows, const int64_t *a_indptr, const int32_t *a_indices,
              float *E_out);

int fdr_knn(fdr_ctx *ctx, const float *E, int64_t n, int32_t d, int32_t k, int32_t *idx_out,
            float *dist_out);

int fdr_embed_knn(fdr_ctx *ctx, int64_t n_rows, const int64_t *a_indptr, const int32_t *a_indices,
                  int32_t k, int32_t *idx_out, float *dist_out, float *E_out);

int fdr_knn_sparse(fdr_ctx *ctx, int64_t n, int64_t n_features, const int64_t *indptr, const int32_t *indices,
                   const float *values, int32_t k, int32_t *idx_out, float *dist_out);

#define FDR_METRIC_COSINE 0
#define FDR_METRIC_JACCARD 1
int fdr_knn_sparse_metric(fdr_ctx *ctx, int32_t metric, int64_t n, int64_t n_features, const int64_t *indptr,
                          const int32_t *indices, const float *values, int32_t k, int32_t *idx_out, float *dist_out);

int fdr_sparse_index_build(fdr_ctx *ctx, int32_t metric, int64_t n, int64_t n_features, const int64_t *indptr,
                           const int32_t *indices, const float *values);
int fdr_sparse_index_search(fdr_ctx *ctx, int32_t k, int64_t q_lo, int64_t q_hi, int32_t *idx_out, float *dist_out);
int fdr_sparse_index_info(fdr_ctx *ctx, int32_t *metric, int64_t *n, int64_t *postings, int64_t *zero_rows,
                          size_t *device_bytes);
int fdr_sparse_index_free(fdr_ctx *ctx);

int fdr_embed_dev(fdr_ctx *ctx, int64_t n_rows, const int64_t *d_indptr, const int32_t *d_indices,
                  float *d_E, void *stream);
int fdr_normalize_dev(fdr_ctx *ctx, const float *d_E, int64_t n_rows, int32_t d, float *d_Ehat,
                      uint8_t *d_zero, void *stream);
size_t fdr_knn_workspace_bytes(fdr_ctx *ctx, int64_t nq, int64_t nt, int32_t d, int32_t k);
int fdr_knn_dev(fdr_ctx *ctx, const float *d_Qhat, const uint8_t *d_qzero, int64_t nq,
                const float *d_That, const uint8_t *d_tzero, int64_t nt, int64_t t_base, int32_t d,
                int32_t k, int32_t *d_idx, float *d_dist, void *d_workspace, size_t workspace_bytes,
                void *stream);
int fdr_knn_classes_dev(fdr_ctx *ctx, const float *d_That, const uint8_t *d_tzero, int64_t nt, int32_t d, int32_t k,
                        int64_t nq_max, void *d_workspace, size_t workspace_bytes, void *stream,
                        int32_t *n_unique_out);
int fdr_knn_unique_dev(fdr_ctx *ctx, int64_t u_lo, int64_t u_hi, int32_t *d_idx_u, float *d_dist_u, void *stream);
int fdr_knn_expand_dev(fdr_ctx *ctx, int64_t q0, int64_t nq, int64_t t_base, const int32_t *d_idx_u_all,
                       const float *d_dist_u_all, int64_t u_row_stride, int32_t *d_idx, float *d_dist, void *stream);

#define FDR_KERNEL_EMBED 0
#define FDR_KERNEL_NORMALIZE 1
#define FDR_KERNEL_KNN_TILE 2
#define FDR_KERNEL_KNN_MERGE 3
#define FDR_KERNEL_KNN_PREFILTER 4
#define FDR_KERNEL_KNN_RERANK 5
#define FDR_KERNEL_KNN_DEDUP 6
#define FDR_KERNEL_KMER_SEARCH 7
#define FDR_KERNEL_KMER_COMPACT 8
#define FDR_NUM_KERNELS 9
int fdr_timing(fdr_ctx *ctx, int enable);
int fdr_timing_read(fdr_ctx *ctx, int which, int *count_out, float *total_ms_out);
#define FDR_MODE_AUTO 0
#define FDR_MODE_EXACT 1
#define FDR_MODE_PREFILTER 2
int fdr_set_knn_mode(fdr_ctx *ctx, int mode);
#define FDR_DEDUP_AUTO 0
#define FDR_DEDUP_OFF 1
#define FDR_DEDUP_ON 2
#define FDR_DEDUP_FORCE 3
int fdr_set_dedup_mode(fdr_ctx *ctx, int mode);
#define FDR_LIVE_AUTO 0
#define FDR_LIVE_OFF 1
#define FDR_LIVE_FORCE 2
int fdr_set_live_chunks(fdr_ctx *ctx, int mode);
int fdr_last_unique(fdr_ctx *ctx, int *unique_targets, int *unique_queries);
int fdr_last_prefilter_launches(fdr_ctx *ctx, int *launches, int *queues);
#define FDR_TRACE_NONE 0
#define FDR_TRACE_EXACT 1
#define FDR_TRACE_PREFILTER 2
#define FDR_TRACE_GENERIC 3
#define FDR_TRACE_SPARSE 4
#define FDR_FALLBACK_NONE 0
#define FDR_FALLBACK_CHUNKED 1
#define FDR_FALLBACK_WHOLE 2
typedef struct fdr_knn_trace {
    int32_t kind;
    int32_t dp, k, kp;
    int64_t queries, targets;
    int32_t pass_waves;
    int32_t pass_wps;
    int32_t pass_units;
    int32_t pass_list_keys;
    int32_t pass_pingpong;
    int32_t pass_launches, pass_queues, pass_segments;
    int32_t uncertified, zero_queries;
    int32_t range_queries;
    int32_t range_chunks;
    int32_t range_pp_chunks;
    int32_t range_w8_chunks;
    int32_t range_overflow;
    int32_t exact_fallback;
    int32_t exact_calls;
    int32_t exact_queries;
    int32_t exact_waves, exact_qsets;
    int32_t generic;
    int32_t exact_segments;
    int32_t pass_live;
    int32_t pass_live_items[5];
    int32_t pass_live_dense_items;
} fdr_knn_trace;
int fdr_last_knn_trace(fdr_ctx *ctx, fdr_knn_trace *out);
int fdr_last_uncertified(fdr_ctx *ctx);
#define FDR_PATH_NONE 0
#define FDR_PATH_CERTIFIED 1
#define FDR_PATH_RANGE 2
#define FDR_PATH_EXACT 3
#define FDR_PATH_ZERO 4
#define FDR_PATH_RANGE_OVERFLOW 5
#define FDR_PATH_GENERIC 6
#define FDR_PATH_CLASS_MEMBER 0x80
int fdr_last_query_paths(fdr_ctx *ctx, uint8_t *paths, int64_t n_queries);
#define FDR_CAPTURE_CANDIDATES 1
#define FDR_CAPTURE_RANGE 2
#define FDR_RANGE_CAP 1024
int fdr_set_knn_capture(fdr_ctx *ctx, int what);
int fdr_last_candidates(fdr_ctx *ctx, uint64_t *keys, int64_t n_queries, int32_t kp, int32_t *qbits_out);
int fdr_last_range_sets(fdr_ctx *ctx, int64_t n_range, int32_t *queries, float *theta, int32_t *counts, int32_t *rows);

int fdr_kmer_search(fdr_ctx *ctx, const uint8_t *seqs, const int64_t *seq_off, int64_t n_reads,
                    const uint64_t *lib_codes, int64_t n_lib, int32_t k, int64_t *indptr_out,
                    int64_t *nnz_out);
int fdr_kmer_search_indices(fdr_ctx *ctx, int32_t *indices_out);

int fdr_kmer_count(fdr_ctx *ctx, const uint8_t *seqs, const int64_t *seq_off, int64_t n_reads, int32_t k,
                   int64_t min_count, int64_t *n_out);
int fdr_kmer_count_fetch(fdr_ctx *ctx, uint64_t *codes_out, uint64_t *counts_out);
int fdr_kmer_count_begin(fdr_ctx *ctx, int32_t k);
int fdr_kmer_count_add(fdr_ctx *ctx, const uint8_t *seqs, const int64_t *seq_off, int64_t n_reads);
int fdr_kmer_count_finish(fdr_ctx *ctx, int64_t min_count, int64_t *n_out);
int fdr_set_kmer_count_block(fdr_ctx *ctx, int64_t chars);
int fdr_last_kmer_count_blocks(fdr_ctx *ctx);
int fdr_kmer_count_export_dev(fdr_ctx *ctx, const uint64_t *d_splitters, int32_t n_parts, uint64_t *d_codes_out,
                              uint64_t *d_counts_out, int64_t *part_off_out, void *stream);
int fdr_kmer_count_merge_dev(fdr_ctx *ctx, int32_t n_runs, const int64_t *run_off, const uint64_t *d_codes,
                             const uint64_t *d_counts, int64_t min_count, int64_t *n_out, void *stream);
int fdr_kmer_count_merge(fdr_ctx *ctx, int32_t n_runs, const int64_t *run_off, const uint64_t *codes,
                         const uint64_t *counts, int64_t min_count, int64_t *n_out);

int fdr_reads_scan(const uint8_t *raw, int64_t n, int32_t is_fastq, int32_t fastq_ids_as_fasta, int32_t eof,
                   int64_t *consumed, int64_t *n_records, int64_t *n_bases);
int fdr_reads_parse(const uint8_t *raw, int64_t consumed, int32_t is_fastq, int32_t fastq_ids_as_fasta,
                    int64_t n_records, int64_t n_bases, uint8_t *seqs, int64_t *seq_off, int64_t *id_span);

int fdr_kmer_output_scan(const char *path, int64_t *n_records, int64_t *nnz, int64_t *name_bytes);
int fdr_kmer_output_load(const char *path, int64_t n_features, int32_t n_threads, int64_t n_records, int64_t nnz,
                         int64_t name_bytes, int64_t *indptr, int32_t *indices, int64_t *name_off, char *names);
int fdr_kmer_output_scan_range(const char *path, int64_t rec_lo, int64_t rec_hi, int64_t *n_records,
                               int64_t *nnz_range, int64_t *name_bytes);
int fdr_kmer_output_load_range(const char *path, int64_t n_features, int32_t n_threads, int64_t n_records,
                               int64_t rec_lo, int64_t rec_hi, int64_t nnz_range, int64_t name_bytes, int64_t *indptr,
                               int32_t *indices, int64_t *name_off, char *names);

int fdr_kmer_output_append(const char *path, int64_t n_records, const int64_t *name_off, const char *names,
                           const int64_t *indptr, const int32_t *indices);

int fdr_overlaps_write(const char *path, int32_t append, int32_t write_header, int64_t n_total, int64_t row0,
                       int64_t n_rows, int32_t k, const int32_t *idx, const float *dist, const int64_t *name_off,
                       const char *names, const uint8_t *strands, int32_t n_threads, int64_t *lines_out);

#ifdef __cplusplus
}
#endif
#endif
```

Measured before the change: 276.4 million.

## Skip target stages whose chunk mask is disjoint from the query block in live-chunk prefilter

Builds a per-segment, per-128-row-stage OR of target chunk masks, then for each of the 256 possible query-block mask values compiles a list of stages that share at least one live chunk. The live prefilter kernel walks only those stages, skipping MFMA work and global-to-LDS loads for stages that cannot contribute. Stage 0 is always kept. This adds two small kernels, extra workspace, a host copy of list lengths and trace and capture plumbing. The pipelined loop now indexes stages indirectly, which adds a readfirstlane load per iteration.

```diff
diff --git a/devtools/live_skip_stats.py b/devtools/live_skip_stats.py
--- /dev/null
+++ b/devtools/live_skip_stats.py
@@ -0,0 +1,74 @@
+import argparse
+import os
+import sys
+import time
+
+import numpy as np
+
+sys.path.insert(0, os.path.dirname(os.path.dirname(os.path.abspath(__file__))))
+sys.path.insert(0, os.path.dirname(os.path.abspath(__file__)))
+from live_chunk_stats import D, NC, chunk_masks, popcount
+from fedrann_amd.precompute import build_precompute_matrix
+from fedrann_amd.synth import synth
+from oracle import oracle as O
+
+DISJOINT = (np.arange(256)[:, None] & np.arange(256)[None, :]) == 0
+
+
+def or_blocks(masks, block):
+    pad = (-masks.size) % block
+    return np.bitwise_or.reduce(np.concatenate([masks, np.zeros(pad, dtype=np.int64)]).reshape(-1, block), axis=1)
+
+
+def unit_masks(masks, unit, segments):
+    tiles = -(-masks.size // 32)
+    cuts = [32 * (tiles * g // segments) for g in range(segments)] + [masks.size]
+    return [or_blocks(masks[b:e], unit) for b, e in zip(cuts, cuts[1:]) if e > b]
+
+
+def block_cost(nl):
+    return np.where(nl > 6, 1.0, 0.23 + 0.09 * np.maximum(nl, 2))
+
+
+def report(masks, unit, segments):
+    bm = or_blocks(masks, 256)
+    nl = popcount(bm)
+    segs = unit_masks(masks, unit, segments)
+    units = sum(u.size for u in segs)
+    hist = sum(np.bincount(u[1:], minlength=256) for u in segs)
+    per_value = (DISJOINT * hist[None, :]).sum(1)
+    skipped = np.where(nl > 6, 0, per_value[bm])
+    cost = block_cost(nl)
+    print("  %3d-row units, %d segment(s): %d blocks x %d units; disjoint pairs %.4f; weighted by 0.23 + 0.09 NL: %.4f"
+          % (unit, segments, bm.size, units, skipped.sum() / (bm.size * units),
+             (cost * skipped).sum() / (cost.sum() * units)))
+    by_nl = ["%d: %.4f (%d)" % (n, skipped[nl == n].sum() / max(1, (nl == n).sum() * units), (nl == n).sum())
+             for n in range(NC + 1)]
+    print("      disjoint share by the block's NL (blocks): " + "  ".join(by_nl))
+
+
+def main():
+    ap = argparse.ArgumentParser(description=__doc__.splitlines()[0])
+    ap.add_argument("--segments", type=int, default=1)
+    ap.add_argument("reads", type=int, nargs="*", default=[100_000, 1_000_000])
+    a = ap.parse_args()
+    for R in a.reads:
+        t0 = time.time()
+        s = synth(R, seed=602)
+        P = build_precompute_matrix(s["counts"], D)
+        E = O.embed(s["indptr"], s["indices"], (P.indptr, P.indices, P.data), s["n_features"], D)
+        del s
+        Eh, _, _ = O.normalize(E)
+        del E
+        v = np.ascontiguousarray(Eh).view(np.dtype((np.void, 4 * D))).ravel()
+        _, first = np.unique(v, return_index=True)
+        first.sort()
+        m = chunk_masks(Eh[first])
+        m = m[np.argsort((popcount(m) << 32) | m, kind="stable")]
+        print("reads %d: %d unique rows, shipped order  (%.0f s)" % (R, first.size, time.time() - t0))
+        for unit in (32, 128):
+            report(m, unit, a.segments)
+
+
+if __name__ == "__main__":
+    main()
diff --git a/fedrann_amd/_lib.py b/fedrann_amd/_lib.py
--- a/fedrann_amd/_lib.py
+++ b/fedrann_amd/_lib.py
@@ -19,6 +19,7 @@
     "fdr_kmer_output_append", "fdr_last_query_paths", "fdr_last_knn_trace", "fdr_kmer_count_export_dev",
     "fdr_kmer_count_merge_dev", "fdr_kmer_count_merge", "fdr_set_knn_capture", "fdr_last_candidates",
     "fdr_last_range_sets", "fdr_knn_sparse", "fdr_set_live_chunks", "fdr_knn_sparse_metric",
+    "fdr_set_live_skip", "fdr_last_live_stage_lists",
     "fdr_sparse_index_build", "fdr_sparse_index_search", "fdr_sparse_index_info", "fdr_sparse_index_free",
 )
 FDR_MAX_K = 128
@@ -28,7 +29,7 @@
 PATH_CERTIFIED, PATH_RANGE, PATH_EXACT, PATH_ZERO, PATH_RANGE_OVERFLOW, PATH_GENERIC, PATH_CLASS_MEMBER = 1, 2, 3, 4, 5, 6, 0x80
 TRACE_KINDS = ("none", "exact", "prefilter", "generic", "sparse")
 FALLBACKS = ("none", "chunked", "whole")
-CAPTURE_CANDIDATES, CAPTURE_RANGE = 1, 2
+CAPTURE_CANDIDATES, CAPTURE_RANGE, CAPTURE_LIVE_LISTS = 1, 2, 4
 RANGE_CAP = 1024
 METRIC_COSINE, METRIC_JACCARD = 0, 1
 SPARSE_METRICS = {"cosine": METRIC_COSINE, "jaccard": METRIC_JACCARD}
@@ -42,7 +43,8 @@
             "pass_segments", "uncertified", "zero_queries", "range_queries", "range_chunks", "range_pp_chunks",
             "range_w8_chunks", "range_overflow", "exact_fallback", "exact_calls", "exact_queries", "exact_waves",
             "exact_qsets", "generic", "exact_segments", "pass_live", "pass_live_items_2", "pass_live_items_3",
-            "pass_live_items_4", "pass_live_items_5", "pass_live_items_6", "pass_live_dense_items")]
+            "pass_live_items_4", "pass_live_items_5", "pass_live_items_6", "pass_live_dense_items", "skip_live")] + \
+        [(n, ctypes.c_int64) for n in ("skip_stages_walked", "skip_stages_skipped")]
 
 
 class FedrannHipError(RuntimeError):
@@ -112,6 +114,8 @@
     L.fdr_last_range_sets.argtypes = [vp, i64, vp, vp, vp, vp]
     L.fdr_set_dedup_mode.argtypes = [vp, ctypes.c_int]
     L.fdr_set_live_chunks.argtypes = [vp, ctypes.c_int]
+    L.fdr_set_live_skip.argtypes = [vp, ctypes.c_int]
+    L.fdr_last_live_stage_lists.argtypes = [vp, i32, ctypes.POINTER(i32), ctypes.POINTER(i32), vp, vp]
     L.fdr_last_unique.argtypes = [vp, ctypes.POINTER(ctypes.c_int), ctypes.POINTER(ctypes.c_int)]
     L.fdr_last_prefilter_launches.argtypes = [vp, ctypes.POINTER(ctypes.c_int), ctypes.POINTER(ctypes.c_int)]
     p64 = ctypes.POINTER(ctypes.c_int64)
@@ -418,6 +422,21 @@
         code = {"auto": 0, "off": 1, "force": 2}[mode]
         self._check(self._L.fdr_set_live_chunks(self._h, code), "fdr_set_live_chunks")
 
+    def set_live_skip(self, mode):
+        code = {"auto": 0, "off": 1}[mode]
+        self._check(self._L.fdr_set_live_skip(self._h, code), "fdr_set_live_skip")
+
+    def last_live_stage_lists(self, segment):
+        first, nst = ctypes.c_int32(), ctypes.c_int32()
+        lens = np.empty(256, dtype=np.int32)
+        self._check(self._L.fdr_last_live_stage_lists(self._h, int(segment), ctypes.byref(first), ctypes.byref(nst),
+                                                      lens.ctypes.data, None), "fdr_last_live_stage_lists")
+        lists = np.empty((256, nst.value), dtype=np.uint16)
+        if nst.value:
+            self._check(self._L.fdr_last_live_stage_lists(self._h, int(segment), None, ctypes.byref(nst), None,
+                                                          lists.ctypes.data), "fdr_last_live_stage_lists")
+        return first.value, lens, lists
+
     def kmer_search(self, seqs, seq_off, lib_codes, k):
         seqs = np.ascontiguousarray(seqs, dtype=np.uint8)
         seq_off = np.ascontiguousarray(seq_off, dtype=np.int64)
diff --git a/fedrann_amd/csrc/fedrann_hip.hip b/fedrann_amd/csrc/fedrann_hip.hip
--- a/fedrann_amd/csrc/fedrann_hip.hip
+++ b/fedrann_amd/csrc/fedrann_hip.hip
@@ -471,6 +471,12 @@
         hipStream_t stream = nullptr;
     } paths;
     fdr_knn_trace trace = {};
+    struct {
+        int nseg = 0;
+        int nt = 0;
+        SegBounds segs;
+        hipStream_t stream = nullptr;
+    } skip;
 };
 
 struct KnnArgs {
@@ -606,6 +612,8 @@
     int dedup_mode = FDR_DEDUP_AUTO;
     int live_mode = FDR_LIVE_AUTO;
     std::vector<unsigned> live_host;
+    int skip_mode = FDR_SKIP_AUTO;
+    std::vector<int> skip_host;
     KnnCallRecord last;
     struct {
         int what = 0;
@@ -613,6 +621,7 @@
         int64_t nq = 0, n_range = 0;
         int kp = 0, qbits = 0;
         DevBuf cand, rq, rtheta, rcnt, rrows;
+        DevBuf lists;
         hipStream_t stream = nullptr;
     } cap;
     struct {
@@ -632,6 +641,7 @@
 static void knn_call_begin(fdr_ctx *ctx) {
     ctx->last.trace = fdr_knn_trace{};
     ctx->last.paths = {};
+    ctx->last.skip.nseg = 0;
     ctx->cap.cand_valid = ctx->cap.range_valid = false;
     ctx->cap.nq = ctx->cap.n_range = 0;
 }
@@ -775,7 +785,7 @@
 }
 
 FDR_EXPORT int fdr_set_knn_capture(fdr_ctx *ctx, int what) {
-    if (!ctx || what < 0 || what > (FDR_CAPTURE_CANDIDATES | FDR_CAPTURE_RANGE)) return fail(FDR_E_ARG, "bad capture flags");
+    if (!ctx || what < 0 || what > (FDR_CAPTURE_CANDIDATES | FDR_CAPTURE_RANGE | FDR_CAPTURE_LIVE_LISTS)) return fail(FDR_E_ARG, "bad capture flags");
     ctx->cap.what = what;
     return FDR_OK;
 }
@@ -829,6 +839,37 @@
 FDR_EXPORT int fdr_set_live_chunks(fdr_ctx *ctx, int mode) {
     if (!ctx || mode < FDR_LIVE_AUTO || mode > FDR_LIVE_FORCE) return fail(FDR_E_ARG, "bad live-chunk mode");
     ctx->live_mode = mode;
+    return FDR_OK;
+}
+
+FDR_EXPORT int fdr_set_live_skip(fdr_ctx *ctx, int mode) {
+    if (!ctx || mode < FDR_SKIP_AUTO || mode > FDR_SKIP_OFF) return fail(FDR_E_ARG, "bad stage-skip mode");
+    ctx->skip_mode = mode;
+    return FDR_OK;
+}
+
+FDR_EXPORT int fdr_last_live_stage_lists(fdr_ctx *ctx, int32_t segment, int32_t *first_row_out, int32_t *nstages_out,
+                                         int32_t *lens, uint16_t *lists) {
+    int rc = use_device(ctx);
+    if (rc) return rc;
+    const auto &rec = ctx->last.skip;
+    if (rec.nseg <= 0)
+        return fail(FDR_E_STATE, "last_live_stage_lists: the last k-NN call captured no live-chunk pass's stage lists");
+    if (segment < 0 || segment >= rec.nseg || !nstages_out)
+        return fail(FDR_E_ARG, "last_live_stage_lists: bad argument (the pass had %d segments)", rec.nseg);
+    const int t_begin = rec.segs.b[segment], t_end = std::min(rec.nt, rec.segs.b[segment + 1]);
+    const int nstages = t_end > t_begin ? (t_end - t_begin + 127) >> 7 : 0;
+    *nstages_out = nstages;
+    if (first_row_out) *first_row_out = t_begin;
+    if (lens) memcpy(lens, ctx->skip_host.data() + (size_t)segment * 256, 256 * sizeof(int));
+    if (!lists || nstages == 0) return FDR_OK;
+    const int stride = live_list_stride(nstages);
+    HIP_TRY(hipMemcpy2DAsync(lists, (size_t)nstages * 2, static_cast<const uint16_t *>(ctx->cap.lists.p) + (size_t)live_stage_row(t_begin, segment) * 256,
+                             (size_t)stride * 2, (size_t)nstages * 2, 256, hipMemcpyDeviceToHost, rec.stream));
+    HIP_TRY(hipStreamSynchronize(rec.stream));
+    for (int v = 0; v < 256; ++v)
+        for (int i = std::max(0, std::min(ctx->skip_host[(size_t)segment * 256 + v], nstages)); i < nstages; ++i)
+            lists[(size_t)v * nstages + i] = 0xffffu;
     return FDR_OK;
 }
 
@@ -1207,6 +1248,18 @@
         };
         int orc;
         if ((orc = order(a.That, nt, L.perm_t, ho_t))) return orc;
+        if (L.live) {
+            int max_stages = 1;
+            for (int i = 0; i < p.nseg; ++i)
+                max_stages = std::max(max_stages, (std::min<int>((int)nt, p.segs.b[i + 1]) - p.segs.b[i] + 127) >> 7);
+            hipLaunchKernelGGL(live_stage_masks_kernel, dim3((unsigned)max_stages, (unsigned)p.nseg), dim3(64), 0, st,
+                               (const u64 *)L.okeys_s, (int)nt, p.segs, L.live_smask);
+            const int all = !(FDR_SKIP_AUTO_ON && ctx->skip_mode == FDR_SKIP_AUTO);
+            hipLaunchKernelGGL(live_stage_lists_kernel, dim3(256, (unsigned)p.nseg), dim3(64), 0, st,
+                               (const uint8_t *)L.live_smask, (int)nt, p.segs, all, L.live_lists, L.live_lens);
+            HIP_TRY(hipGetLastError());
+            ctx->last.trace.skip_live = !all;
+        }
         if (!self && (orc = order(a.Qhat, nq, L.perm_q, ho_q))) return orc;
         ord.perm_t = L.perm_t;
         p1_t = ho_t;
@@ -1246,7 +1299,20 @@
     std::vector<unsigned> &masks = ctx->live_host;
     masks.resize((size_t)nqb);
     HIP_TRY(hipMemcpyAsync(masks.data(), L.live_masks, (size_t)nqb * 4, hipMemcpyDeviceToHost, st));
+    std::vector<int> &lens = ctx->skip_host;
+    lens.resize((size_t)p.nseg * 256);
+    HIP_TRY(hipMemcpyAsync(lens.data(), L.live_lens, (size_t)p.nseg * 256 * 4, hipMemcpyDeviceToHost, st));
     HIP_TRY(hipStreamSynchronize(st));
+    if (ctx->cap.what & FDR_CAPTURE_LIVE_LISTS) {
+        const size_t bytes = live_stage_rows(a.nt) * 256 * sizeof(uint16_t);
+        int crc = ctx->cap.lists.reserve(bytes);
+        if (crc) return crc;
+        HIP_TRY(hipMemcpyAsync(ctx->cap.lists.p, L.live_lists, bytes, hipMemcpyDeviceToDevice, st));
+        ctx->last.skip.nseg = p.nseg;
+        ctx->last.skip.nt = (int)a.nt;
+        ctx->last.skip.segs = p.segs;
+        ctx->last.skip.stream = st;
+    }
     const LivePlan lp = live_plan(masks.data(), nqb, p.nseg, ctx->live_mode == FDR_LIVE_FORCE ? 0 : p.cohort);
     HIP_TRY(hipMemcpyAsync(L.live_ids, lp.ids.data(), (size_t)nqb * 4, hipMemcpyHostToDevice, st));
     HIP_TRY(hipMemcpyAsync(L.live_order, lp.order.data(), (size_t)nqb * 4, hipMemcpyHostToDevice, st));
@@ -1258,6 +1324,15 @@
         items.push_back((long long)g.count * p.nseg);
         if (g.nl != FDR_LIVE_DENSE) {
             tr.pass_live_items[g.nl - FDR_LIVE_MIN_NL] = g.count * p.nseg;
+            for (int sg = 0; sg < p.nseg; ++sg) {
+                const int len = std::min<int>((int)a.nt, p.segs.b[sg + 1]) - p.segs.b[sg];
+                const int64_t nst = len > 0 ? (len + 127) >> 7 : 0;
+                int64_t walked = 0;
+                for (int i = 0; i < g.count; ++i)
+                    walked += std::min<int64_t>(nst, lens[(size_t)sg * 256 + (masks[(size_t)lp.order[(size_t)(g.first + i)]] & 0xffu)]);
+                tr.skip_stages_walked += walked;
+                tr.skip_stages_skipped += nst * g.count - walked;
+            }
             continue;
         }
         tr.pass_live_dense_items = g.count * p.nseg;
@@ -1282,7 +1357,8 @@
             hipLaunchKernelGGL(kLiveKernels[g.nl - FDR_LIVE_MIN_NL], dim3(grid), dim3(512), live_lds_bytes(g.nl), s,
                                p1_q, (int)a.nq, (const _Float16 *)L.hb_t, (int)a.nt, (int)a.t_base, p.segs, kp, p.nq_pad,
                                R.partial, R.shared, ib, base, g.count, (const int *)(L.live_order + g.first),
-                               (const unsigned *)L.live_ids, ord);
+                               (const unsigned *)L.live_ids, ord, (const unsigned *)L.live_masks,
+                               reinterpret_cast<const unsigned *>(L.live_lists), (const int *)L.live_lens);
     });
 }
 
diff --git a/fedrann_amd/csrc/host_common.inc b/fedrann_amd/csrc/host_common.inc
--- a/fedrann_amd/csrc/host_common.inc
+++ b/fedrann_amd/csrc/host_common.inc
@@ -1,4 +1,9 @@
 #define FDR_EXPORT extern "C" __attribute__((visibility("default")))
+#ifdef __HIPCC__
+#define FDR_HOST_DEVICE __host__ __device__
+#else
+#define FDR_HOST_DEVICE
+#endif
 typedef unsigned long long u64;
 
 #ifndef FDR_W8_DEFAULT
diff --git a/fedrann_amd/csrc/knn_prefilter_live.inc b/fedrann_amd/csrc/knn_prefilter_live.inc
--- a/fedrann_amd/csrc/knn_prefilter_live.inc
+++ b/fedrann_amd/csrc/knn_prefilter_live.inc
@@ -11,6 +11,44 @@
 #pragma unroll
     for (int off = 32; off >= 1; off >>= 1) m |= __shfl_xor(m, off);
     if (lane == 0) masks[b] = m;
+}
+
+__global__ __launch_bounds__(64) void live_stage_masks_kernel(const u64 *__restrict__ keys_s, int nt, SegBounds segs,
+                                                              uint8_t *__restrict__ smask) {
+    const int seg = blockIdx.y, stage = blockIdx.x, lane = threadIdx.x;
+    const int t_begin = segs.b[seg], t_end = min(nt, segs.b[seg + 1]);
+    const int r0 = t_begin + stage * 128;
+    if (r0 >= t_end) return;
+    unsigned m = 0;
+#pragma unroll
+    for (int i = 0; i < 2; ++i) {
+        const int r = r0 + i * 64 + lane;
+        if (r < t_end) m |= (unsigned)keys_s[r] & 0xffu;
+    }
+#pragma unroll
+    for (int off = 32; off >= 1; off >>= 1) m |= __shfl_xor(m, off);
+    if (lane == 0) smask[live_stage_row(t_begin, seg) + stage] = (uint8_t)m;
+}
+
+__global__ __launch_bounds__(64) void live_stage_lists_kernel(const uint8_t *__restrict__ smask, int nt, SegBounds segs,
+                                                              int all, uint16_t *__restrict__ lists,
+                                                              int *__restrict__ lens) {
+    const int seg = blockIdx.y, lane = threadIdx.x;
+    const unsigned v = blockIdx.x;
+    const int t_begin = segs.b[seg], t_end = min(nt, segs.b[seg + 1]);
+    const int nstages = t_end > t_begin ? (t_end - t_begin + 127) >> 7 : 0;
+    const size_t row = (size_t)live_stage_row(t_begin, seg);
+    const uint8_t *sm = smask + row;
+    uint16_t *out = lists + row * 256 + (size_t)v * live_list_stride(nstages);
+    int count = 0;
+    for (int s0 = 0; s0 < nstages; s0 += 64) {
+        const int s = s0 + lane;
+        const bool keep = s < nstages && (s == 0 || all != 0 || (sm[s] & v) != 0u);
+        const unsigned long long kept = __ballot(keep);
+        if (keep) out[count + __popcll(kept & ((1ull << lane) - 1ull))] = (uint16_t)s;
+        count += __popcll(kept);
+    }
+    if (lane == 0) lens[seg * 256 + (int)v] = count;
 }
 
 __global__ __launch_bounds__(256) void to_half_blocked_kernel(const float *__restrict__ Ehat,
@@ -57,7 +95,8 @@
 __global__ __launch_bounds__(512, 4) void knn_prefilter_live_kernel(
     const _Float16 *__restrict__ Qh, int nq, const _Float16 *__restrict__ Tb, int nt, int t_base, SegBounds segs, int K,
     int nq_pad, u64 *__restrict__ partial, unsigned *__restrict__ tau_shared, int ib, int item_base, int nb,
-    const int *__restrict__ blocks, const unsigned *__restrict__ live_ids, OrderArgs ord) {
+    const int *__restrict__ blocks, const unsigned *__restrict__ live_ids, OrderArgs ord,
+    const unsigned *__restrict__ masks, const unsigned *__restrict__ lists, const int *__restrict__ lens) {
     static_assert(NL >= FDR_LIVE_MIN_NL && NL <= FDR_LIVE_MAX_NL, "instances NL = 2 .. 6");
     extern __shared__ __attribute__((aligned(16))) unsigned char smem[];
     constexpr int DP = 128, NW = 8, U = 4, LH = 16, QW = 32 * NW;
@@ -70,6 +109,7 @@
     const int seg = item / nb;
     const int qb = __builtin_amdgcn_readfirstlane(blocks[item - seg * nb]);
     const unsigned ids = __builtin_amdgcn_readfirstlane(live_ids[qb]);
+    const unsigned bmask = __builtin_amdgcn_readfirstlane(masks[qb]) & 0xffu;
 
     const int tid = threadIdx.x;
     const int lane = tid & 63;
@@ -123,6 +163,13 @@
     const int t_end = min(nt, segs.b[seg + 1]);
     const int nunits = (t_end - t_begin + 31) >> 5;
     const int nstages = (nunits + U - 1) / U;
+    const int nlist = nstages > 0 ? min(lens[seg * 256 + (int)bmask], nstages) : 0;
+    const unsigned *list = lists + (((size_t)live_stage_row(t_begin, seg) * 256 + (size_t)bmask * live_list_stride(nstages)) >> 1);
+    auto entry = [&](int i) -> int {
+        const int e = max(min(i, nlist - 1), 0);
+        const unsigned w = __builtin_amdgcn_readfirstlane(list[e >> 1]);
+        return min((int)((w >> (16 * (e & 1))) & 0xffffu), max(nstages - 1, 0));
+    };
 
     const char *seg_base = reinterpret_cast<const char *>(Tb) + (size_t)(t_begin >> 5) * TILE_BYTES;
     unsigned poff[PPW];
@@ -132,20 +179,21 @@
         const int tl = p / NL, s = p - tl * NL;
         poff[u] = (unsigned)(tl * TILE_BYTES) + ((ids >> (4 * s)) & 7u) * 1024u;
     }
-    unsigned soff = (unsigned)((lane & 31) * 32 + (lane >> 5) * 16);
-    auto issue_stage = [&](auto par_c) {
+    const unsigned soff = (unsigned)((lane & 31) * 32 + (lane >> 5) * 16);
+    auto issue_stage = [&](auto par_c, int sn) {
+        const unsigned stoff = (unsigned)sn * (unsigned)(U * TILE_BYTES);
         constexpr int par = decltype(par_c)::value;
         unsigned char *dst = smem + par * STAGE_BYTES;
         static_for(std::make_integer_sequence<int, PPW>{}, [&](auto u_c) {
             constexpr int u = decltype(u_c)::value;
             if (NW * (u + 1) <= NPIECE || wave < NPIECE - NW * u)
-                __builtin_amdgcn_global_load_lds((const __attribute__((address_space(1))) void *)(seg_base + (soff + poff[u])),
+                __builtin_amdgcn_global_load_lds((const __attribute__((address_space(1))) void *)(seg_base + (soff + (poff[u] + stoff))),
                                                  (__attribute__((address_space(3))) void *)(dst + (wave + NW * u) * 1024),
                                                  16, 0, 0);
         });
-        soff += (unsigned)(U * TILE_BYTES);
-    };
-    if (nstages > 0) issue_stage(std::integral_constant<int, 0>{});
+    };
+    int sprev = 0, scur = entry(0), snext = entry(1);
+    if (nlist > 0) issue_stage(std::integral_constant<int, 0>{}, scur);
     __syncthreads();
 
     unsigned q0 = PK_EMPTY, q1 = PK_EMPTY;
@@ -212,7 +260,8 @@
     auto stage_body = [&](auto par_c, int it) {
         constexpr int par = decltype(par_c)::value;
         STAMP(ts0);
-        if (it + 1 < nstages) issue_stage(std::integral_constant<int, par ^ 1>{});
+        const int safter = entry(it + 2);
+        if (it + 1 < nlist) issue_stage(std::integral_constant<int, par ^ 1>{}, snext);
         STAMP(ts1);
         STAMP_ADD(0, ts0, ts1);
         auto mfma_pair = [&](auto p_c) __attribute__((always_inline)) {
@@ -239,11 +288,11 @@
             score(acc, ts);
             if (ts + 1 < nunits) score(accB, ts + 1);
         };
-        if (late && it > 0 && U * it - 2 < nunits) score_pair(U * it - 2);
-        if (it < nstages) {
+        if (late && it > 0 && U * sprev + U - 2 < nunits) score_pair(U * sprev + U - 2);
+        if (it < nlist) {
             static_for(std::make_integer_sequence<int, NP>{}, [&](auto p_c) {
                 constexpr int p = decltype(p_c)::value;
-                const int tp = U * it + 2 * p;
+                const int tp = U * scur + 2 * p;
                 if (tp < nunits) {
                     mfma_pair(p_c);
                     if (!late || p < NP - 1) score_pair(tp);
@@ -270,8 +319,11 @@
 #else
         __syncthreads();
 #endif
-    };
-    const int niter = nstages + 1;
+        sprev = scur;
+        scur = snext;
+        snext = safter;
+    };
+    const int niter = nlist + 1;
     for (int it0 = 0; it0 < niter; it0 += 2) {
         stage_body(std::integral_constant<int, 0>{}, it0);
         if (it0 + 1 < niter) stage_body(std::integral_constant<int, 1>{}, it0 + 1);
@@ -301,7 +353,8 @@
 }
 
 typedef void (*LiveKernel)(const _Float16 *, int, const _Float16 *, int, int, SegBounds, int, int, u64 *, unsigned *, int,
-                           int, int, const int *, const unsigned *, OrderArgs);
+                           int, int, const int *, const unsigned *, OrderArgs, const unsigned *, const unsigned *,
+                           const int *);
 static constexpr LiveKernel kLiveKernels[FDR_LIVE_MAX_NL - FDR_LIVE_MIN_NL + 1] = {
     knn_prefilter_live_kernel<2>, knn_prefilter_live_kernel<3>, knn_prefilter_live_kernel<4>,
     knn_prefilter_live_kernel<5>, knn_prefilter_live_kernel<6>};
diff --git a/fedrann_amd/csrc/knn_workspace.inc b/fedrann_amd/csrc/knn_workspace.inc
--- a/fedrann_amd/csrc/knn_workspace.inc
+++ b/fedrann_amd/csrc/knn_workspace.inc
@@ -58,6 +58,11 @@
     if (live_mode == FDR_LIVE_OFF || shape != FDR_P128_W8U4) return false;
     return live_mode == FDR_LIVE_FORCE || (FDR_LIVE_AUTO_ON && pp.cohort > 0 && pp.queues == 2);
 }
+
+#define FDR_SKIP_AUTO_ON 1
+static FDR_HOST_DEVICE inline int live_stage_row(int t_begin, int seg) { return (t_begin >> 7) + 2 * seg; }
+static FDR_HOST_DEVICE inline int live_list_stride(int nstages) { return (nstages + 1) & ~1; }
+static size_t live_stage_rows(int64_t nt) { return (size_t)(nt >> 7) + 2 * FDR_MAX_SEG + 2; }
 
 static bool knn_prefilter_wanted(int knn_mode, int64_t nt, int k) {
     if (knn_mode == FDR_MODE_EXACT) return false;
@@ -106,6 +111,9 @@
     ws_half *hb_t;
     unsigned *live_masks, *live_ids;
     int *live_order;
+    uint8_t *live_smask;
+    uint16_t *live_lists;
+    int *live_lens;
     ws_half *live_hq;
     int *live_perm;
     unsigned *live_tau;
@@ -166,6 +174,9 @@
         L.live_masks = A.take<unsigned>(nqb);
         L.live_ids = A.take<unsigned>(nqb);
         L.live_order = A.take<int>(nqb);
+        L.live_smask = A.take<uint8_t>(live_stage_rows(nt));
+        L.live_lists = A.take<uint16_t>(live_stage_rows(nt) * 256);
+        L.live_lens = A.take<int>((size_t)FDR_MAX_SEG * 256);
         L.live_hq = A.take<ws_half>(nqb * 256 * dp);
         L.live_perm = A.take<int>(nqb * 256);
         L.live_tau = A.take<unsigned>(nqb * 256);
diff --git a/include/fedrann_hip.h b/include/fedrann_hip.h
--- a/include/fedrann_hip.h
+++ b/include/fedrann_hip.h
@@ -100,6 +100,11 @@
 #define FDR_LIVE_OFF 1
 #define FDR_LIVE_FORCE 2
 int fdr_set_live_chunks(fdr_ctx *ctx, int mode);
+#define FDR_SKIP_AUTO 0
+#define FDR_SKIP_OFF 1
+int fdr_set_live_skip(fdr_ctx *ctx, int mode);
+int fdr_last_live_stage_lists(fdr_ctx *ctx, int32_t segment, int32_t *first_row_out, int32_t *nstages_out, int32_t *lens,
+                              uint16_t *lists);
 int fdr_last_unique(fdr_ctx *ctx, int *unique_targets, int *unique_queries);
 int fdr_last_prefilter_launches(fdr_ctx *ctx, int *launches, int *queues);
 #define FDR_TRACE_NONE 0
@@ -135,6 +140,9 @@
     int32_t pass_live;
     int32_t pass_live_items[5];
     int32_t pass_live_dense_items;
+    int32_t skip_live;
+    int64_t skip_stages_walked;
+    int64_t skip_stages_skipped;
 } fdr_knn_trace;
 int fdr_last_knn_trace(fdr_ctx *ctx, fdr_knn_trace *out);
 int fdr_last_uncertified(fdr_ctx *ctx);
@@ -149,6 +157,7 @@
 int fdr_last_query_paths(fdr_ctx *ctx, uint8_t *paths, int64_t n_queries);
 #define FDR_CAPTURE_CANDIDATES 1
 #define FDR_CAPTURE_RANGE 2
+#define FDR_CAPTURE_LIVE_LISTS 4
 #define FDR_RANGE_CAP 1024
 int fdr_set_knn_capture(fdr_ctx *ctx, int what);
 int fdr_last_candidates(fdr_ctx *ctx, uint64_t *keys, int64_t n_queries, int32_t kp, int32_t *qbits_out);
```

Result: faster. 282.3 million, median of 6 (+2.1%).
